# lucaspk512/vrdone

Measured on AMD Instinct MI355X. Metric: subject-object pairs/sec forward (2048 pairs x 256 frames x 512-d), higher is better.
Workload: dtype f16x3: f32 products as 3 scaled-f16 MFMA products (~22-bit), f32 accumulate; reference-grade: distance to a float64 run of the reference <= 1.4 x the reference's own float32 error (tests/golden/mask_vrd_f64.npz)

## Files before the change

### include/vrdone_hip.h

```cpp
#ifndef VRDONE_HIP_H
#define VRDONE_HIP_H

#include <stdint.h>

#ifdef __cplusplus
extern "C" {
#endif

#define VRD_ABI_VERSION 36

#define VRD_DETERMINISTIC 1
#define VRD_ERR_SCRATCH (-3)
int vrd_scratch_required(int64_t* floats);

enum vrd_act { VRD_ACT_NONE = 0, VRD_ACT_RELU = 1, VRD_ACT_GELU = 2 };

enum vrd_pair_format { VRD_PAIR_NONE = 0, VRD_PAIR_BF16 = 1, VRD_PAIR_F16 = 2 };
#define VRD_F16_ACT_EXP 4

enum vrd_kernel_id {
    VRD_K_GEMM = 0, VRD_K_LAYERNORM = 1, VRD_K_DWCONV_LN = 2, VRD_K_LOCAL_ATTN = 3,
    VRD_K_ATTN_SMALL = 4, VRD_K_ATTN_FLASH = 5, VRD_K_POOL = 6, VRD_K_MASK_HEAD = 7,
    VRD_K_TRANSPOSE = 8, VRD_K_POSTPROC = 9, VRD_K_GEMM_X3 = 10, VRD_K_GEMM_X3_DMA = 11, VRD_K_GEMM_X3_BIG = 12,
    VRD_K_BACKWARD = 13,
    VRD_K_COUNT = 14
};

int vrd_abi_version(void);
const char* vrd_last_error(void);

int vrd_f16_range_flag(void** flag);

int vrd_prof_enable(int on);
int vrd_prof_reset(void);
int vrd_prof_read(int kernel_id, double* ms, int64_t* launches, double* flops, double* bytes);
int vrd_prof_read_skipped(int kernel_id, double* flops_skipped);
int vrd_prof_select(unsigned long long family_mask);

int vrd_bct_to_btc(const float* src, int B, int C_total, int T, int c0, int count,
                   float* dst, int64_t ld_dst, int out_pair , int T_src, const int32_t* src_batch,
                   void* stream);
typedef struct {
    const float* const* src;
    const int32_t* lens;
    int32_t P, C_in, T, V, Cc, S, E;
    float* vis;
    float* clip;
    float* so_box;
    float* ent;
    int32_t pair_wide;
} vrd_pack_args;
int vrd_pack_pairs(const vrd_pack_args* a, void* stream);

typedef struct {
    const float* vis;
    const float* clip;
    const float* boxes;
    const int64_t* s_row;
    const int64_t* o_row;
    const int32_t* lens;
    int32_t P, T, V, Cc, stride;
    float w, h;
    float* out_vis;
    float* out_clip;
    float* out_so_box;
    float* out_ent;
    int32_t pair_wide;
    const float* seq_wh;
} vrd_gather_args;
int vrd_gather_pairs(const vrd_gather_args* a, void* stream);

typedef struct {
    const float* streams;
    const float* snippets;
    const int64_t* stream_row;
    const int32_t* lens;
    int32_t P, T, D, L, piece, reach;
    float* out;
} vrd_assemble_args;
int vrd_assemble_pairs(const vrd_assemble_args* a, void* stream);

int vrd_btc_to_bct(const float* src, int64_t ld_src, int B, int C, int T, float* dst, void* stream);

typedef struct {
    const float* A;  int64_t lda;
    const float* W;
    const float* bias;
    float* C;  int64_t ldc;
    int64_t M;  int32_t N;  int32_t Cin;  int32_t taps;  int32_t T;
    int32_t act;
    const uint8_t* row_mask;
    const float* scale;
    const float* res;  int64_t ldres;  int32_t res_masked;
    const float* res2;  int64_t ldres2;
    const uint16_t* W_split;
    int32_t a_pair_width;
    int32_t c_pair;
    const int32_t* row_blocks;
    const int32_t* row_blocks_active;
    int32_t row_block_seg_len;
    int32_t split_fmt;
    const float* w_scale;
    const float* a_scale;
    int32_t products;
} vrd_gemm_args;
int vrd_gemm(const vrd_gemm_args* a, void* stream);
int vrd_gemm_batch(const vrd_gemm_args* a, int count, void* stream);

int vrd_row_blocks(const uint8_t* mask, int64_t rows, int seg_len, int32_t* order, int32_t* n_active, void* stream);

typedef struct {
    const float* x;
    int64_t ldx;
    int64_t rows;
    int Cin, taps, T, N;
    const float* w;
    const float* bias;
    const uint8_t* row_mask;
    const float* gamma;
    const float* beta;
    int relu;
    float* y;
    int64_t ldy;
    int out_pair;
} vrd_conv_ln_args;
int vrd_conv_ln(const vrd_conv_ln_args* a, void* stream);

int vrd_layernorm(const float* x, int64_t ldx, float* y, int64_t ldy, int64_t rows, int C,
                  const float* gamma, const float* beta, int relu,
                  const float* post_add, int64_t ld_add, int add_period, int out_pair , void* stream);

#define VRD_MAX_SEGS 32
typedef struct {
    int32_t count;
    int32_t n[VRD_MAX_SEGS];
    int32_t T[VRD_MAX_SEGS];
    int64_t row[VRD_MAX_SEGS];
} vrd_row_segs;

typedef struct {
    const float* x;  int64_t ldx;
    const float* x_up;  int64_t ldx_up;
    int32_t B, Tin, C, ksize, stride, group_in;
    const uint8_t* mask_out;
    int32_t n_out;
    const float* w[3];
    const float* bias[3];
    const float* gamma[3];
    const float* beta[3];
    int32_t relu[3];
    float* y[3];
    int64_t ldy[3];
    int32_t out_pair[3];
    const float* pre_gamma;
    const float* pre_beta;
    const float* packed[3];
    const vrd_row_segs* segs;
} vrd_dwconv_ln_args;
int vrd_dwconv_ln(const vrd_dwconv_ln_args* a, void* stream);

int vrd_local_attn(const float* q, const float* k, const float* v, int64_t ld,
                   const uint8_t* mask, const float* rel_pe, int B, int T, int C, int n_head, int half_win,
                   float* out, int64_t ldo, int out_pair, void* stream);
int vrd_local_attn_segs(const float* q, const float* k, const float* v, int64_t ld,
                        const uint8_t* mask, const float* rel_pe, const vrd_row_segs* segs, int C, int n_head, int half_win,
                        float* out, int64_t ldo, int out_pair, void* stream);

int vrd_attention(const float* q, int64_t ldq, const float* k, const float* v, int64_t ldkv,
                  const uint8_t* kv_mask, int B, int Tq, int Tk, int n_head, int head_dim,
                  float* out, int64_t ldo, int algo, int out_pair, void* stream);

int vrd_attention_pair(const float* q, int64_t ldq, const float* k, const float* v, int64_t ldkv,
                       const uint8_t* kv_mask, const uint8_t* q_mask, int B, int Tq, int Tk, int n_head, int head_dim,
                       float* out, int64_t ldo, int out_pair, int pair_fmt, void* stream, int products);

int vrd_maxpool_mask(const float* x, int64_t ldx, int B, int Tin, int C, const uint8_t* mask_in,
                     float* y, int64_t ldy, uint8_t* mask_out, void* stream);

int vrd_mask_head(const float* emb, int64_t ld_emb, const float* feat, int64_t ld_feat,
                  const uint8_t* out_mask, int B, int Q, int T, int Dp, float fill,
                  float* seg, void* stream);

int vrd_postprocess(const float* logits, const float* masks, const int32_t* valid_len,
                    int P, int Q, int K1, int T, int topk,
                    float* top_score, int32_t* top_cat, int32_t* seg_first, int32_t* seg_last,
                    void* stream);

typedef struct {
    const float* cand;
    const float* s_score;
    const float* o_score;
    const int32_t* so_offset;
    const int32_t* so_start;
    const int32_t* so_end;
    const int32_t* video_pairs;
    int32_t n_videos, max_video_pairs, Q, k, feat_stride, pred_min_frames, n_max_pair;
    int32_t* out_count;
    int32_t* out_index;
    float* out_score;
} vrd_select_args;
int vrd_select_triplets(const vrd_select_args* a, void* stream);


int vrd_gemm_wgrad(const float* G, int64_t ldg, const float* X, int64_t ldx, const uint8_t* row_mask, int64_t M, int N, int Cin,
                   int taps, int T, float* dW, float* scratch, int64_t scratch_floats, void* stream, int flags);

int vrd_gemm_wgrad_x3(const float* G, int64_t ldg, const float* X, int64_t ldx, const uint8_t* row_mask, int64_t M, int N, int Cin,
                      int taps, int T, float* dW, float* dbias, float* scratch, int64_t scratch_floats, const float* g_scale,
                      void* stream, int flags);

#define VRD_ABSMAX_SCALE_FLOATS 516
int vrd_absmax_scale(const float* x, int64_t ldx, int64_t rows, int cols, float* scale, void* stream);

int vrd_colsum(const float* a, int64_t lda, const float* b, int64_t ldb, int b_cstride, int b_coffset, int b_rstride, int shift,
               int T, const uint8_t* row_mask, const float* row_scale, int64_t rows, int C, float* out, float* scratch,
               int64_t scratch_floats, void* stream, int flags);

int vrd_dwconv_wgrad(const float* dD, int64_t lddd, const float* x, int64_t ldx, int ksize, int stride, int group_in, int T,
                     const uint8_t* row_mask, int64_t rows, int C, float* dw, float* dbias, float* scratch, int64_t scratch_floats,
                     void* stream, int flags);

int vrd_rowcol_scale(const float* v, int64_t ldv, int64_t rows, int C, const float* col_scale, const float* row_scale,
                     const uint8_t* row_mask, const float* res, int64_t ldres, int res_masked, const float* res2, int64_t ldres2,
                     float* out, int64_t ldo, void* stream);

int vrd_activation(const float* x, int64_t ldx, const float* dy, int64_t lddy, int64_t rows, int C, int act, float* out, int64_t ldo,
            void* stream);

int vrd_layernorm_bwd(const float* x, int64_t ldx, const float* dy, int64_t lddy, int64_t rows, int C, const float* gamma,
                      const float* beta, int relu, float* dx, int64_t lddx, float* dgamma, float* dbeta, float* scratch,
                      int64_t scratch_floats, void* stream, int flags);

typedef struct {
    const float* dD[3];  int64_t lddd[3];
    const float* w[3];
    int32_t n_out, B, Tin, C, ksize, stride, group_in;
    const uint8_t* mask_out;
    float* dx;  int64_t lddx;
    float* dx_up;  int64_t lddx_up;
} vrd_dwconv_bwd_args;
int vrd_dwconv_bwd(const vrd_dwconv_bwd_args* a, void* stream);

int vrd_local_attn_bwd(const float* q, const float* k, const float* v, int64_t ld, const float* dO, int64_t lddo,
                       const uint8_t* mask, const float* rel_pe, int B, int T, int C, int n_head, int half_win,
                       float* dq, float* dk, float* dv,
                       int64_t ldd, float* scratch, void* stream);

int vrd_attn_bwd_probs(const float* q, int64_t ldq, const float* k, const float* v, int64_t ldkv, const float* dO, int64_t lddo,
                       const uint8_t* kv_mask, int B, int Tq, int Tk, int n_head, int head_dim, float* P, float* dS, void* stream);

int vrd_attn_bwd_softmax(float* P, float* dS, const uint8_t* kv_mask, int B, int Tq, int Tk, int n_head, void* stream);

int vrd_attention_bwd(const float* q, int64_t ldq, const float* k, const float* v, int64_t ldkv, const float* out, const float* dO,
                      int64_t ldo, const uint8_t* kv_mask, int B, int Tq, int Tk, int n_head, int head_dim, float* dq, float* dk,
                      float* dv, const float* lse , float* scratch,
                      const float* o_scale, const float* v_scale, void* stream);
int vrd_attention_rows(const float* q, int64_t ldq, const float* k, const float* v, int64_t ldkv, const uint8_t* kv_mask, int B, int Tq,
                       int Tk, int n_head, int head_dim, int fmt, float* out, int64_t ldo, float* lse, void* stream);

typedef struct {
    const float* A;  int64_t a_z0, a_z1, a_row, a_col;
    const float* B;  int64_t b_z0, b_z1, b_row, b_col;
    float* C;  int64_t c_z0, c_z1, c_row, c_col;
    int32_t Z0, Z1, M, N, K;
    float alpha;
    int32_t accumulate;
} vrd_bmm_args;
int vrd_bmm(const vrd_bmm_args* a, void* stream);

int vrd_maxpool_bwd(const float* x, int64_t ldx, const float* dy, int64_t lddy, int B, int Tin, int C, const uint8_t* mask_in, float* dx,
                    int64_t lddx, void* stream);

int vrd_assign(const float* cost, int64_t ld, const int32_t* first, const int32_t* count, int P, int Q, int32_t* query_of, void* stream);

int vrd_ema_update(float* const* ema, const float* const* model, const int64_t* numel, const int32_t* chunk_tensor,
                   const int32_t* chunk_index, int n_chunks, float decay, float one_minus_decay, void* stream);

typedef struct {
    const float* logits[4];
    const float* masks[4];
    int32_t n_layers, B, Q, K1, T, G;
    const uint8_t* out_valid;
    const int64_t* tgt_ids;
    const float* tgt_masks;
    const int32_t* owner;
    const int32_t* segs;
    float scale_range, alpha, gamma;
    float w_class, w_mask, w_dice;
} vrd_criterion_args;

typedef struct {
    float* logits[4];
    float* masks[4];
} vrd_criterion_grads;

int vrd_criterion_costs(const vrd_criterion_args* a, float* cost, void* stream);
int vrd_criterion_losses(const vrd_criterion_args* a, const int32_t* query_of, const float* class_weight, float num_masks, float* out,
                         void* stream);
int vrd_criterion_backward(const vrd_criterion_args* a, const int32_t* query_of, const float* class_weight, float num_masks,
                           const float* fwd_out, const float* gout, const vrd_criterion_grads* grads, void* stream);

int vrd_split_weight(const float* src, int R, int Q, int taps, int64_t sr, int64_t st, int64_t sq, uint16_t* out, int fmt, float* scale,
                     void* stream);

typedef struct {
    const float* src;
    uint16_t* out;
    int32_t R, Q, taps, fmt;
    int64_t sr, st, sq;
    float* scale;
} vrd_split_job;
int vrd_split_weights(const vrd_split_job* jobs, int n_jobs, const int32_t* chunk_job, const int32_t* chunk_index, int n_chunks,
// ... 7 lines not shown
```

### vrdone_amd/_hip.py

```python
import ctypes as C
import os

_HERE = os.path.dirname(os.path.abspath(__file__))
LIB_PATH = os.environ.get("VRDONE_HIP_LIB") or os.path.join(_HERE, "csrc", "libvrdone_hip.so")

ACT_NONE, ACT_RELU, ACT_GELU = 0, 1, 2
PAIR_NONE, PAIR_BF16, PAIR_F16 = 0, 1, 2
F16_ACT_EXP = 4
ABSMAX_SCALE_FLOATS = 516
(K_GEMM, K_LAYERNORM, K_DWCONV_LN, K_LOCAL_ATTN, K_ATTN_SMALL, K_ATTN_FLASH, K_POOL, K_MASK_HEAD,
 K_TRANSPOSE, K_POSTPROC, K_GEMM_X3, K_GEMM_X3_DMA, K_GEMM_X3_BIG, K_BACKWARD, K_COUNT) = range(15)
KERNEL_NAMES = ["gemm_f32_mfma", "layernorm", "dwconv_ln", "local_attn", "attn_small", "attn_flash",
                "maxpool_mask", "mask_head", "transpose", "postprocess", "gemm_x3_mfma", "gemm_x3_dma",
                "gemm_x3_big", "backward"]
assert len(KERNEL_NAMES) == K_COUNT

c_f32p = C.c_void_p
c_u8p = C.c_void_p
c_i32p = C.c_void_p


class CriterionArgs(C.Structure):
    _fields_ = [("logits", C.c_void_p * 4), ("masks", C.c_void_p * 4),
                ("n_layers", C.c_int32), ("B", C.c_int32), ("Q", C.c_int32), ("K1", C.c_int32), ("T", C.c_int32), ("G", C.c_int32),
                ("out_valid", C.c_void_p), ("tgt_ids", C.c_void_p), ("tgt_masks", C.c_void_p), ("owner", C.c_void_p),
                ("segs", C.c_void_p), ("scale_range", C.c_float), ("alpha", C.c_float), ("gamma", C.c_float),
                ("w_class", C.c_float), ("w_mask", C.c_float), ("w_dice", C.c_float)]


class CriterionGrads(C.Structure):
    _fields_ = [("logits", C.c_void_p * 4), ("masks", C.c_void_p * 4)]


class GemmArgs(C.Structure):
    _fields_ = [("A", c_f32p), ("lda", C.c_int64), ("W", c_f32p), ("bias", c_f32p),
                ("C", c_f32p), ("ldc", C.c_int64),
                ("M", C.c_int64), ("N", C.c_int32), ("Cin", C.c_int32), ("taps", C.c_int32), ("T", C.c_int32),
                ("act", C.c_int32), ("row_mask", c_u8p), ("scale", c_f32p),
                ("res", c_f32p), ("ldres", C.c_int64), ("res_masked", C.c_int32),
                ("res2", c_f32p), ("ldres2", C.c_int64), ("W_split", C.c_void_p),
                ("a_pair_width", C.c_int32), ("c_pair", C.c_int32),
                ("row_blocks", C.c_void_p), ("row_blocks_active", C.c_void_p), ("row_block_seg_len", C.c_int32),
                ("split_fmt", C.c_int32), ("w_scale", c_f32p), ("a_scale", c_f32p), ("products", C.c_int32)]


MAX_SEGS = 32


class RowSegs(C.Structure):
    _fields_ = [("count", C.c_int32), ("n", C.c_int32 * MAX_SEGS), ("T", C.c_int32 * MAX_SEGS), ("row", C.c_int64 * MAX_SEGS)]

    _made = {}

    @classmethod
    def of(cls, segs):
        key = tuple(segs)
        s = cls._made.get(key)
        if s is None:
            assert 1 <= len(segs) <= MAX_SEGS
            if len(cls._made) > 4096:
                cls._made.clear()
            s = cls._made[key] = cls()
            s.count = len(segs)
            for i, (row, n, T) in enumerate(segs):
                s.row[i], s.n[i], s.T[i] = row, n, T
        return s


class DwconvLnArgs(C.Structure):
    _fields_ = [("x", c_f32p), ("ldx", C.c_int64), ("x_up", c_f32p), ("ldx_up", C.c_int64),
                ("B", C.c_int32), ("Tin", C.c_int32), ("C", C.c_int32), ("ksize", C.c_int32),
                ("stride", C.c_int32), ("group_in", C.c_int32),
                ("mask_out", c_u8p), ("n_out", C.c_int32),
                ("w", c_f32p * 3), ("bias", c_f32p * 3), ("gamma", c_f32p * 3), ("beta", c_f32p * 3),
                ("relu", C.c_int32 * 3), ("y", c_f32p * 3), ("ldy", C.c_int64 * 3), ("out_pair", C.c_int32 * 3),
                ("pre_gamma", c_f32p), ("pre_beta", c_f32p), ("packed", c_f32p * 3), ("segs", C.POINTER(RowSegs))]


class ConvLnArgs(C.Structure):
    _fields_ = [("x", c_f32p), ("ldx", C.c_int64), ("rows", C.c_int64),
                ("Cin", C.c_int32), ("taps", C.c_int32), ("T", C.c_int32), ("N", C.c_int32),
                ("w", c_f32p), ("bias", c_f32p), ("row_mask", c_u8p), ("gamma", c_f32p), ("beta", c_f32p),
                ("relu", C.c_int32), ("y", c_f32p), ("ldy", C.c_int64), ("out_pair", C.c_int32)]


class PackArgs(C.Structure):
    _fields_ = [("src", C.c_void_p), ("lens", C.c_void_p),
                ("P", C.c_int32), ("C_in", C.c_int32), ("T", C.c_int32), ("V", C.c_int32), ("Cc", C.c_int32),
                ("S", C.c_int32), ("E", C.c_int32),
                ("vis", c_f32p), ("clip", c_f32p), ("so_box", c_f32p), ("ent", c_f32p), ("pair_wide", C.c_int32)]


class DwconvBwdArgs(C.Structure):
    _fields_ = [("dD", c_f32p * 3), ("lddd", C.c_int64 * 3), ("w", c_f32p * 3),
                ("n_out", C.c_int32), ("B", C.c_int32), ("Tin", C.c_int32), ("C", C.c_int32), ("ksize", C.c_int32),
                ("stride", C.c_int32), ("group_in", C.c_int32),
                ("mask_out", c_u8p), ("dx", c_f32p), ("lddx", C.c_int64), ("dx_up", c_f32p), ("lddx_up", C.c_int64)]


class BmmArgs(C.Structure):
    _fields_ = [("A", c_f32p), ("a_z0", C.c_int64), ("a_z1", C.c_int64), ("a_row", C.c_int64), ("a_col", C.c_int64),
                ("B", c_f32p), ("b_z0", C.c_int64), ("b_z1", C.c_int64), ("b_row", C.c_int64), ("b_col", C.c_int64),
                ("C", c_f32p), ("c_z0", C.c_int64), ("c_z1", C.c_int64), ("c_row", C.c_int64), ("c_col", C.c_int64),
                ("Z0", C.c_int32), ("Z1", C.c_int32), ("M", C.c_int32), ("N", C.c_int32), ("K", C.c_int32),
                ("alpha", C.c_float), ("accumulate", C.c_int32)]


class SplitJob(C.Structure):
    _fields_ = [("src", c_f32p), ("out", C.c_void_p), ("R", C.c_int32), ("Q", C.c_int32), ("taps", C.c_int32), ("fmt", C.c_int32),
                ("sr", C.c_int64), ("st", C.c_int64), ("sq", C.c_int64), ("scale", c_f32p)]


class GatherArgs(C.Structure):
    _fields_ = [("vis", c_f32p), ("clip", c_f32p), ("boxes", c_f32p), ("s_row", C.c_void_p), ("o_row", C.c_void_p),
                ("lens", C.c_void_p), ("P", C.c_int32), ("T", C.c_int32), ("V", C.c_int32), ("Cc", C.c_int32),
                ("stride", C.c_int32), ("w", C.c_float), ("h", C.c_float),
                ("out_vis", c_f32p), ("out_clip", c_f32p), ("out_so_box", c_f32p), ("out_ent", c_f32p),
                ("pair_wide", C.c_int32), ("seq_wh", c_f32p)]


class SelectArgs(C.Structure):
    _fields_ = [("cand", c_f32p), ("s_score", c_f32p), ("o_score", c_f32p), ("so_offset", c_i32p), ("so_start", c_i32p),
                ("so_end", c_i32p), ("video_pairs", c_i32p),
                ("n_videos", C.c_int32), ("max_video_pairs", C.c_int32), ("Q", C.c_int32), ("k", C.c_int32),
                ("feat_stride", C.c_int32), ("pred_min_frames", C.c_int32), ("n_max_pair", C.c_int32),
                ("out_count", c_i32p), ("out_index", c_i32p), ("out_score", c_f32p)]


class AssembleArgs(C.Structure):
    _fields_ = [("streams", c_f32p), ("snippets", c_f32p), ("stream_row", C.c_void_p), ("lens", C.c_void_p),
                ("P", C.c_int32), ("T", C.c_int32), ("D", C.c_int32), ("L", C.c_int32), ("piece", C.c_int32), ("reach", C.c_int32),
                ("out", c_f32p)]


_SIGNATURES = {
    "vrd_abi_version": (C.c_int, []),
    "vrd_last_error": (C.c_char_p, []),
    "vrd_f16_range_flag": (C.c_int, [C.POINTER(C.c_void_p)]),
    "vrd_prof_enable": (C.c_int, [C.c_int]),
    "vrd_prof_reset": (C.c_int, []),
    "vrd_prof_read": (C.c_int, [C.c_int, C.POINTER(C.c_double), C.POINTER(C.c_int64), C.POINTER(C.c_double),
                                C.POINTER(C.c_double)]),
    "vrd_prof_read_skipped": (C.c_int, [C.c_int, C.POINTER(C.c_double)]),
    "vrd_prof_select": (C.c_int, [C.c_uint64]),
    "vrd_bct_to_btc": (C.c_int, [c_f32p, C.c_int, C.c_int, C.c_int, C.c_int, C.c_int, c_f32p, C.c_int64, C.c_int, C.c_int, c_i32p,
                                 C.c_void_p]),
    "vrd_btc_to_bct": (C.c_int, [c_f32p, C.c_int64, C.c_int, C.c_int, C.c_int, c_f32p, C.c_void_p]),
    "vrd_pack_pairs": (C.c_int, [C.POINTER(PackArgs), C.c_void_p]),
    "vrd_gather_pairs": (C.c_int, [C.POINTER(GatherArgs), C.c_void_p]),
    "vrd_assemble_pairs": (C.c_int, [C.POINTER(AssembleArgs), C.c_void_p]),
    "vrd_split_weight": (C.c_int, [c_f32p, C.c_int, C.c_int, C.c_int, C.c_int64, C.c_int64, C.c_int64, C.c_void_p, C.c_int, c_f32p,
                                   C.c_void_p]),
    "vrd_split_weights": (C.c_int, [C.c_void_p, C.c_int, C.c_void_p, C.c_void_p, C.c_int, C.c_void_p]),
    "vrd_gemm": (C.c_int, [C.POINTER(GemmArgs), C.c_void_p]),
    "vrd_gemm_batch": (C.c_int, [C.POINTER(GemmArgs), C.c_int, C.c_void_p]),
    "vrd_row_blocks": (C.c_int, [c_u8p, C.c_int64, C.c_int, C.c_void_p, C.c_void_p, C.c_void_p]),
    "vrd_conv_ln": (C.c_int, [C.POINTER(ConvLnArgs), C.c_void_p]),
    "vrd_layernorm": (C.c_int, [c_f32p, C.c_int64, c_f32p, C.c_int64, C.c_int64, C.c_int, c_f32p, c_f32p, C.c_int,
                                c_f32p, C.c_int64, C.c_int, C.c_int, C.c_void_p]),
    "vrd_dwconv_ln": (C.c_int, [C.POINTER(DwconvLnArgs), C.c_void_p]),
    "vrd_local_attn": (C.c_int, [c_f32p, c_f32p, c_f32p, C.c_int64, c_u8p, c_f32p, C.c_int, C.c_int, C.c_int, C.c_int,
                                 C.c_int, c_f32p, C.c_int64, C.c_int, C.c_void_p]),
    "vrd_local_attn_segs": (C.c_int, [c_f32p, c_f32p, c_f32p, C.c_int64, c_u8p, c_f32p, C.POINTER(RowSegs), C.c_int, C.c_int,
                                      C.c_int, c_f32p, C.c_int64, C.c_int, C.c_void_p]),
    "vrd_attention": (C.c_int, [c_f32p, C.c_int64, c_f32p, c_f32p, C.c_int64, c_u8p, C.c_int, C.c_int, C.c_int,
                                C.c_int, C.c_int, c_f32p, C.c_int64, C.c_int, C.c_int, C.c_void_p]),
    "vrd_attention_pair": (C.c_int, [c_f32p, C.c_int64, c_f32p, c_f32p, C.c_int64, c_u8p, c_u8p, C.c_int, C.c_int, C.c_int,
                                     C.c_int, C.c_int, c_f32p, C.c_int64, C.c_int, C.c_int, C.c_void_p, C.c_int]),
    "vrd_maxpool_mask": (C.c_int, [c_f32p, C.c_int64, C.c_int, C.c_int, C.c_int, c_u8p, c_f32p, C.c_int64, c_u8p,
                                   C.c_void_p]),
    "vrd_mask_head": (C.c_int, [c_f32p, C.c_int64, c_f32p, C.c_int64, c_u8p, C.c_int, C.c_int, C.c_int, C.c_int,
                                C.c_float, c_f32p, C.c_void_p]),
    "vrd_postprocess": (C.c_int, [c_f32p, c_f32p, c_i32p, C.c_int, C.c_int, C.c_int, C.c_int, C.c_int, c_f32p, c_i32p,
                                  c_i32p, c_i32p, C.c_void_p]),
    "vrd_select_triplets": (C.c_int, [C.POINTER(SelectArgs), C.c_void_p]),
    "vrd_gemm_wgrad": (C.c_int, [c_f32p, C.c_int64, c_f32p, C.c_int64, c_u8p, C.c_int64, C.c_int, C.c_int, C.c_int, C.c_int,
                                 c_f32p, c_f32p, C.c_int64, C.c_void_p, C.c_int]),
    "vrd_gemm_wgrad_x3": (C.c_int, [c_f32p, C.c_int64, c_f32p, C.c_int64, c_u8p, C.c_int64, C.c_int, C.c_int, C.c_int, C.c_int,
                                    c_f32p, c_f32p, c_f32p, C.c_int64, c_f32p, C.c_void_p, C.c_int]),
    "vrd_scratch_required": (C.c_int, [C.POINTER(C.c_int64)]),
    "vrd_absmax_scale": (C.c_int, [c_f32p, C.c_int64, C.c_int64, C.c_int, c_f32p, C.c_void_p]),
    "vrd_dwconv_wgrad": (C.c_int, [c_f32p, C.c_int64, c_f32p, C.c_int64, C.c_int, C.c_int, C.c_int, C.c_int, c_u8p, C.c_int64,
                                   C.c_int, c_f32p, c_f32p, c_f32p, C.c_int64, C.c_void_p, C.c_int]),
    "vrd_colsum": (C.c_int, [c_f32p, C.c_int64, c_f32p, C.c_int64, C.c_int, C.c_int, C.c_int, C.c_int, C.c_int, c_u8p, c_f32p,
                             C.c_int64, C.c_int, c_f32p, c_f32p, C.c_int64, C.c_void_p, C.c_int]),
    "vrd_rowcol_scale": (C.c_int, [c_f32p, C.c_int64, C.c_int64, C.c_int, c_f32p, c_f32p, c_u8p, c_f32p, C.c_int64, C.c_int,
                                   c_f32p, C.c_int64, c_f32p, C.c_int64, C.c_void_p]),
    "vrd_activation": (C.c_int, [c_f32p, C.c_int64, c_f32p, C.c_int64, C.c_int64, C.c_int, C.c_int, c_f32p, C.c_int64, C.c_void_p]),
    "vrd_layernorm_bwd": (C.c_int, [c_f32p, C.c_int64, c_f32p, C.c_int64, C.c_int64, C.c_int, c_f32p, c_f32p, C.c_int, c_f32p,
                                    C.c_int64, c_f32p, c_f32p, c_f32p, C.c_int64, C.c_void_p, C.c_int]),
    "vrd_dwconv_bwd": (C.c_int, [C.POINTER(DwconvBwdArgs), C.c_void_p]),
    "vrd_local_attn_bwd": (C.c_int, [c_f32p, c_f32p, c_f32p, C.c_int64, c_f32p, C.c_int64, c_u8p, c_f32p, C.c_int, C.c_int,
                                     C.c_int, C.c_int, C.c_int, c_f32p, c_f32p, c_f32p, C.c_int64, c_f32p, C.c_void_p]),
    "vrd_attn_bwd_probs": (C.c_int, [c_f32p, C.c_int64, c_f32p, c_f32p, C.c_int64, c_f32p, C.c_int64, c_u8p, C.c_int, C.c_int,
                                     C.c_int, C.c_int, C.c_int, c_f32p, c_f32p, C.c_void_p]),
    "vrd_bmm": (C.c_int, [C.POINTER(BmmArgs), C.c_void_p]),
    "vrd_attention_bwd": (C.c_int, [c_f32p, C.c_int64, c_f32p, c_f32p, C.c_int64, c_f32p, c_f32p, C.c_int64, c_u8p, C.c_int, C.c_int,
                                    C.c_int, C.c_int, C.c_int, c_f32p, c_f32p, c_f32p, c_f32p, c_f32p, c_f32p, c_f32p, C.c_void_p]),
    "vrd_attention_rows": (C.c_int, [c_f32p, C.c_int64, c_f32p, c_f32p, C.c_int64, c_u8p, C.c_int, C.c_int, C.c_int, C.c_int, C.c_int,
                                     C.c_int, c_f32p, C.c_int64, c_f32p, C.c_void_p]),
    "vrd_assign": (C.c_int, [c_f32p, C.c_int64, c_i32p, c_i32p, C.c_int, C.c_int, c_i32p, C.c_void_p]),
    "vrd_ema_update": (C.c_int, [C.c_void_p, C.c_void_p, C.c_void_p, c_i32p, c_i32p, C.c_int, C.c_float, C.c_float, C.c_void_p]),
    "vrd_attn_bwd_softmax": (C.c_int, [c_f32p, c_f32p, c_u8p, C.c_int, C.c_int, C.c_int, C.c_int, C.c_void_p]),
    "vrd_criterion_costs": (C.c_int, [C.c_void_p, c_f32p, C.c_void_p]),
    "vrd_criterion_losses": (C.c_int, [C.c_void_p, c_i32p, c_f32p, C.c_float, c_f32p, C.c_void_p]),
    "vrd_criterion_backward": (C.c_int, [C.c_void_p, c_i32p, c_f32p, C.c_float, c_f32p, c_f32p, C.c_void_p, C.c_void_p]),
    "vrd_maxpool_bwd": (C.c_int, [c_f32p, C.c_int64, c_f32p, C.c_int64, C.c_int, C.c_int, C.c_int, c_u8p, c_f32p, C.c_int64,
                                  C.c_void_p]),
}

ABI_VERSION = 36

DETERMINISTIC = 1
ERR_SCRATCH = -3


class HipLibraryError(RuntimeError):
    pass


_FLAGS_DEFAULT = ("vrd_gemm_wgrad_x3", "vrd_colsum", "vrd_dwconv_wgrad", "vrd_layernorm_bwd")


def _flags_default(fn):
    n = len(fn.argtypes)

    def call(*args):
        return fn(*args, 0) if len(args) == n - 1 else fn(*args)
    call.__name__, call.argtypes, call.restype = fn.__name__, fn.argtypes, fn.restype
    return call


def _load():
    if not os.path.exists(LIB_PATH):
        raise HipLibraryError(
            f"{LIB_PATH} is missing: the HIP extension was not built "
            "(run `make -C vrdone_amd/csrc`); there is no CPU fallback for this path")
    import torch
    lib = C.CDLL(LIB_PATH)
    for name, (res, args) in _SIGNATURES.items():
        fn = getattr(lib, name)
        fn.restype = res
        fn.argtypes = args
    for name in _FLAGS_DEFAULT:
        setattr(lib, name, _flags_default(getattr(lib, name)))
    got = lib.vrd_abi_version()
    if got != ABI_VERSION:
        raise HipLibraryError(f"libvrdone_hip.so ABI {got} != expected {ABI_VERSION}: rebuild it")
    return lib


lib = _load()


def check(rc, what):
    if rc != 0:
        raise RuntimeError(f"{what} failed ({rc}): {lib.vrd_last_error().decode()}")


RANGE_TAGS = {1: "boundary tensors (bct_to_btc / pack_pairs / gather_pairs)", 2: "layernorm", 4: "dwconv_ln", 8: "gemm outputs",
              16: "f32 rows split inside a gemm", 32: "attention outputs", 64: "other"}


def prof_enable(on=True):
    check(lib.vrd_prof_enable(1 if on else 0), "vrd_prof_enable")


def prof_select(families=None):
    mask = (1 << 64) - 1 if families is None else sum(1 << KERNEL_NAMES.index(f) for f in families)
    check(lib.vrd_prof_select(mask), "vrd_prof_select")


def prof_reset():
    check(lib.vrd_prof_reset(), "vrd_prof_reset")


def prof_read():
    out = {}
    for kid, name in enumerate(KERNEL_NAMES):
        ms, n, fl, by, sk = C.c_double(), C.c_int64(), C.c_double(), C.c_double(), C.c_double()
        check(lib.vrd_prof_read(kid, C.byref(ms), C.byref(n), C.byref(fl), C.byref(by)), "vrd_prof_read")
        check(lib.vrd_prof_read_skipped(kid, C.byref(sk)), "vrd_prof_read_skipped")
        out[name] = {"ms": ms.value, "launches": n.value, "flops": fl.value, "bytes": by.value, "flops_skipped": sk.value}
    return out
```

### vrdone_amd/csrc/vrd_rowops.hip

```cpp
#include "vrd_common.h"
#include <cmath>

namespace {

constexpr float LN_EPS = 1e-5f;

__device__ __forceinline__ float4 ld4(const float* p) { return *reinterpret_cast<const float4*>(p); }
__device__ __forceinline__ void st4(float* p, float4 v) { *reinterpret_cast<float4*>(p) = v; }
__device__ __forceinline__ float4 f4add(float4 a, float4 b) { return make_float4(a.x + b.x, a.y + b.y, a.z + b.z, a.w + b.w); }

__global__ __launch_bounds__(256) void bct_to_btc_kernel(const float* __restrict__ src, int C_total, int T, int c0,
                                                         int count, float* __restrict__ dst, int64_t ld_dst, int pair, int T_src,
                                                         const int32_t* __restrict__ src_batch, unsigned* rflag) {
    __shared__ float tile[64][65];
    vrd::RangeTrack rt;
    const int b = blockIdx.z, ct = blockIdx.y * 64, tt = blockIdx.x * 64;
    const int tx = threadIdx.x & 63, ty = threadIdx.x >> 6;
    const float* s = src + ((int64_t)(src_batch ? src_batch[b] : b) * C_total + c0) * T_src;
    for (int c = ty; c < 64; c += 4)
        tile[c][tx] = (ct + c < count && tt + tx < T) ? s[(int64_t)(ct + c) * T_src + tt + tx] : 0.f;
    __syncthreads();
    for (int t = ty; t < 64; t += 4)
        if (tt + t < T && ct + tx < count) {
            float* row = dst + ((int64_t)b * T + tt + t) * ld_dst;
// ... 197 lines not shown
    for (int i = 0; i < NV; ++i) {
        v[i].x -= mean; v[i].y -= mean; v[i].z -= mean; v[i].w -= mean;
        ss += (v[i].x * v[i].x + v[i].y * v[i].y) + (v[i].z * v[i].z + v[i].w * v[i].w);
    }
    const float inv = 1.0f / sqrtf(vrd::wave_sum(ss) * inv_c + LN_EPS);
#pragma unroll
    for (int i = 0; i < NV; ++i) {
        const float4 g = ld4(gamma + lane_chan<NV, WIDE>(i, lane)), bb = ld4(beta + lane_chan<NV, WIDE>(i, lane));
        v[i].x = fmaf(v[i].x * inv, g.x, bb.x);
        v[i].y = fmaf(v[i].y * inv, g.y, bb.y);
        v[i].z = fmaf(v[i].z * inv, g.z, bb.z);
        v[i].w = fmaf(v[i].w * inv, g.w, bb.w);
        if (relu) {
            v[i].x = fmaxf(v[i].x, 0.f); v[i].y = fmaxf(v[i].y, 0.f);
            v[i].z = fmaxf(v[i].z, 0.f); v[i].w = fmaxf(v[i].w, 0.f);
        }
    }
}

template <int NV>
__global__ __launch_bounds__(256) void layernorm_kernel(const float* __restrict__ x, int64_t ldx, float* __restrict__ y,
                                                        int64_t ldy, int64_t rows, const float* __restrict__ gamma,
                                                        const float* __restrict__ beta, int relu,
                                                        const float* __restrict__ post_add, int64_t ld_add, int period,
                                                        int pair, unsigned* rflag) {
    vrd::RangeTrack rt;
    const int lane = threadIdx.x & 63;
    int64_t row = (int64_t)blockIdx.x * 4 + __builtin_amdgcn_readfirstlane(threadIdx.x >> 6);
    const int64_t stride = (int64_t)gridDim.x * 4;
    if (row >= rows) return;
    float4 v[NV], vn[NV];
#pragma unroll
    for (int i = 0; i < NV; ++i) v[i] = ld4(x + row * ldx + i * 256 + lane * 4);
    for (;;) {
        const int64_t nxt = row + stride;
        if (nxt < rows) {
#pragma unroll
            for (int i = 0; i < NV; ++i) vn[i] = ld4(x + nxt * ldx + i * 256 + lane * 4);
        }
        ln_rows<NV>(v, gamma, beta, lane, relu != 0);
        if (post_add) {
            const float* a = post_add + (row % period) * ld_add;
#pragma unroll
            for (int i = 0; i < NV; ++i) v[i] = f4add(v[i], ld4(a + i * 256 + lane * 4));
        }
#pragma unroll
        for (int i = 0; i < NV; ++i) {
            if (pair) vrd::store_pair4(y + row * ldy, i * 256 + lane * 4, 256 * NV, v[i], pair, &rt);
            else st4(y + row * ldy + i * 256 + lane * 4, v[i]);
        }
        if (nxt >= rows) break;
        row = nxt;
#pragma unroll
        for (int i = 0; i < NV; ++i) v[i] = vn[i];
    }
    rt.report(rflag, vrd::RANGE_LAYERNORM);
}

constexpr int CL_MAXK = 32;
template <int NV>
__global__ __launch_bounds__(256) void conv_ln_kernel(vrd_conv_ln_args p, unsigned* rflag) {
    vrd::RangeTrack rt;
    constexpr int N = 256 * NV;
    constexpr bool WIDE = NV == 2;
    extern __shared__ __attribute__((aligned(16))) float cl_lds[];
    const int K = p.Cin * p.taps;
    for (int idx = threadIdx.x; idx < N * K; idx += 256) {
        const int n = idx / K, rem = idx - n * K, ci = rem / p.taps, tap = rem - ci * p.taps;
        cl_lds[(tap * p.Cin + ci) * N + n] = p.w[idx];
    }
    for (int n = threadIdx.x; n < N; n += 256) cl_lds[K * N + n] = p.bias ? p.bias[n] : 0.f;
    __syncthreads();
    const int lane = threadIdx.x & 63;
    constexpr int RG = 4;
    int64_t grp = (int64_t)blockIdx.x * 4 + __builtin_amdgcn_readfirstlane(threadIdx.x >> 6);
    const int64_t stride = (int64_t)gridDim.x * 4;
    const int half = p.taps / 2;
    const int lrow = lane / p.Cin, lci = lane - lrow * p.Cin;
    auto load_in = [&](int64_t g) {
        const int64_t r = g * RG - half + lrow;
        float val = 0.f;
        if (lrow < RG + 2 * half && r >= 0 && r < p.rows) val = p.x[r * p.ldx + lci];
        return val;
    };
    float xin = grp * RG < p.rows ? load_in(grp) : 0.f;
    for (; grp * RG < p.rows; grp += stride) {
        const int64_t row0 = grp * RG;
        const float xcur = xin;
        if ((grp + stride) * RG < p.rows) xin = load_in(grp + stride);
        float4 v[RG][NV];
        int t[RG];
#pragma unroll
        for (int j = 0; j < RG; ++j) {
            t[j] = (int)((row0 + j) % p.T);
#pragma unroll
            for (int i = 0; i < NV; ++i) v[j][i] = *reinterpret_cast<const float4*>(cl_lds + K * N + lane_chan<NV, WIDE>(i, lane));
        }
        for (int tap = 0; tap < p.taps; ++tap) {
            for (int ci = 0; ci < p.Cin; ++ci) {
                const float* wk = cl_lds + (tap * p.Cin + ci) * N;
                float4 w[NV];
#pragma unroll
                for (int i = 0; i < NV; ++i) w[i] = *reinterpret_cast<const float4*>(wk + lane_chan<NV, WIDE>(i, lane));
#pragma unroll
                for (int j = 0; j < RG; ++j) {
                    const int tt = t[j] + tap - half;
                    const bool ok = tt >= 0 && tt < p.T && row0 + j < p.rows;
                    const float xl = __builtin_bit_cast(float, __builtin_amdgcn_readlane(__builtin_bit_cast(int, xcur), (j + tap) * p.Cin + ci));
                    const float xv = ok ? xl : 0.f;
#pragma unroll
                    for (int i = 0; i < NV; ++i) {
                        v[j][i].x = fmaf(w[i].x, xv, v[j][i].x); v[j][i].y = fmaf(w[i].y, xv, v[j][i].y);
                        v[j][i].z = fmaf(w[i].z, xv, v[j][i].z); v[j][i].w = fmaf(w[i].w, xv, v[j][i].w);
                    }
                }
            }
        }
#pragma unroll
        for (int j = 0; j < RG; ++j) {
            const int64_t row = row0 + j;
            if (row >= p.rows) break;
            if (p.row_mask) {
                const float mk = (float)vrd::uniform_load(p.row_mask + row);
#pragma unroll
                for (int i = 0; i < NV; ++i) v[j][i].x *= mk, v[j][i].y *= mk, v[j][i].z *= mk, v[j][i].w *= mk;
            }
            if (p.gamma) {
                ln_rows<NV, WIDE>(v[j], p.gamma, p.beta, lane, p.relu != 0);
            } else if (p.relu) {
#pragma unroll
                for (int i = 0; i < NV; ++i) {
                    v[j][i].x = fmaxf(v[j][i].x, 0.f); v[j][i].y = fmaxf(v[j][i].y, 0.f);
                    v[j][i].z = fmaxf(v[j][i].z, 0.f); v[j][i].w = fmaxf(v[j][i].w, 0.f);
                }
            }
            float* yr = p.y + row * p.ldy;
            if (WIDE && p.out_pair) {
                vrd::store_pair8(yr, lane * 8, v[j][0], v[j][NV - 1], p.out_pair, &rt);
            } else {
#pragma unroll
                for (int i = 0; i < NV; ++i) {
                    const int c = lane_chan<NV, WIDE>(i, lane);
                    if (p.out_pair) vrd::store_pair4(yr, c, N, v[j][i], p.out_pair, &rt);
                    else st4(yr + c, v[j][i]);
                }
            }
        }
    }
    rt.report(rflag, vrd::RANGE_LAYERNORM);
}

constexpr int DW_RW = 16;

template <int NV, int KS, int GIN>
__global__ __launch_bounds__(256) void dwconv_ln_kernel(vrd_dwconv_ln_args p, int Tout_u, int strips_per_seq, int strips_per_wave, int rw, unsigned* rflag,
                                                        vrd::SegTable sg) {
    vrd::RangeTrack rt;
    constexpr int C = 256 * NV, NT = GIN * KS, SETF = (NT + 3) * C;
    constexpr bool WIDE = NV == 2 && GIN == 1;
    extern __shared__ __attribute__((aligned(16))) float dw_lds[];
    const int lane = threadIdx.x & 63, wave = __builtin_amdgcn_readfirstlane(threadIdx.x >> 6);
    for (int o = 0; o < p.n_out; ++o) {
        float* const ls = dw_lds + o * SETF;
        if (p.packed[o]) {
            for (int idx = threadIdx.x * 4; idx < SETF; idx += 1024) st4(ls + idx, ld4(p.packed[o] + idx));
            continue;
        }
        for (int idx = threadIdx.x; idx < C * NT; idx += 256) ls[(idx % NT) * C + idx / NT] = p.w[o][idx];
        for (int c = threadIdx.x; c < C; c += 256) {
            ls[NT * C + c] = p.bias[o] ? p.bias[o][c] : 0.f;
            ls[(NT + 1) * C + c] = p.gamma[o] ? p.gamma[o][c] : 1.f;
            ls[(NT + 2) * C + c] = p.gamma[o] ? p.beta[o][c] : 0.f;
        }
    }
    const float* const pre = dw_lds + p.n_out * SETF;
    if (p.pre_gamma)
        for (int c = threadIdx.x; c < C; c += 256) {
            dw_lds[p.n_out * SETF + c] = p.pre_gamma[c];
            dw_lds[p.n_out * SETF + C + c] = p.pre_beta[c];
        }
    __syncthreads();
    const int nwg = gridDim.x, bid = blockIdx.x;
    const int xcd = bid & 7, qq = nwg >> 3, rem = nwg & 7;
    const int lid = (xcd < rem ? xcd * (qq + 1) : rem * (qq + 1) + (xcd - rem) * qq) + (bid >> 3);
    for (int si = 0; si < strips_per_wave; ++si) {
    const int64_t ws = ((int64_t)lid * 4 + wave) * strips_per_wave + si;
    int Tin, Tout, to0;
    int64_t xrow0, urow0, orow0;
    if (sg.count) {
        int g, b, strip;
        if (!vrd::seg_find(sg, ws, g, b, strip)) break;
        Tin = sg.T[g], Tout = Tin / p.stride, to0 = strip * rw;
        xrow0 = sg.row[g] + (int64_t)b * Tin;
        urow0 = sg.row[g] / 2 + (int64_t)b * (Tin / 2);
        orow0 = sg.row[g] / p.stride + (int64_t)b * Tout;
    } else {
        const int b = (int)(ws / strips_per_seq);
        if (b >= p.B) break;
        Tin = p.Tin, Tout = Tout_u, to0 = (int)(ws - (int64_t)b * strips_per_seq) * rw;
        xrow0 = (int64_t)b * Tin, urow0 = (int64_t)b * (Tin / 2), orow0 = (int64_t)b * Tout;
    }
    const int to1 = min(to0 + rw, Tout);

    struct Row {
        float4 v[NV][GIN];
    };
    auto load_row = [&](int ti) {
        Row r;
        const bool ok = ti >= 0 && ti < Tin;
#pragma unroll
        for (int i = 0; i < NV; ++i)
#pragma unroll
            for (int g = 0; g < GIN; ++g) {
                float4 v = make_float4(0.f, 0.f, 0.f, 0.f);
                if (ok) {
                    const int64_t coff = (int64_t)GIN * lane_chan<NV, WIDE>(i, lane) + 4 * g;
                    v = ld4(p.x + (xrow0 + ti) * p.ldx + coff);
                    if (p.x_up) v = f4add(v, ld4(p.x_up + (urow0 + (ti >> 1)) * p.ldx_up + coff));
                }
                r.v[i][g] = v;
            }
        if (GIN == 1 && p.pre_gamma && ok) {
            float4 t[NV];
#pragma unroll
            for (int i = 0; i < NV; ++i) t[i] = r.v[i][0];
            ln_rows<NV, WIDE>(t, pre, pre + C, lane, false);
#pragma unroll
            for (int i = 0; i < NV; ++i) r.v[i][0] = t[i];
        }
        return r;
    };
    if (p.mask_out) {
        const int64_t r0 = orow0 + to0;
        const bool mine = lane < to1 - to0 && p.mask_out[r0 + lane] != 0;
        if (!__any(mine)) {
#pragma unroll
            for (int o = 0; o < 3; ++o) {
                if (o >= p.n_out) break;
                const float* const lb = dw_lds + o * SETF + (NT + 2) * C;
                float4 val[NV];
#pragma unroll
                for (int i = 0; i < NV; ++i) {
                    val[i] = *reinterpret_cast<const float4*>(lb + lane_chan<NV, WIDE>(i, lane));
                    if (p.relu[o]) {
                        val[i].x = fmaxf(val[i].x, 0.f); val[i].y = fmaxf(val[i].y, 0.f);
                        val[i].z = fmaxf(val[i].z, 0.f); val[i].w = fmaxf(val[i].w, 0.f);
                    }
                }
                for (int to = to0; to < to1; ++to) {
                    const int64_t row = orow0 + to;
                    if (WIDE && p.out_pair[o]) {
                        vrd::store_pair8(p.y[o] + row * p.ldy[o], lane * 8, val[0], val[NV - 1], p.out_pair[o], &rt);
                    } else {
#pragma unroll
                        for (int i = 0; i < NV; ++i) {
                            const int c = lane_chan<NV, WIDE>(i, lane);
                            if (p.out_pair[o]) vrd::store_pair4(p.y[o] + row * p.ldy[o], c, 256 * NV, val[i], p.out_pair[o], &rt);
                            else st4(p.y[o] + row * p.ldy[o] + c, val[i]);
                        }
                    }
                }
            }
            continue;
        }
    }
    Row win[KS];
#pragma unroll
    for (int k = 0; k < KS; ++k) win[k] = load_row(p.stride * to0 + k - KS / 2);
    for (int to = to0; to < to1; ++to) {
        Row nxt[2];
        const int tn = p.stride * (to + 1) - KS / 2;
        const bool more = to + 1 < to1;
        if (KS == 1) {
            if (more) nxt[0] = load_row(tn);
        } else if (p.stride == 1) {
            if (more) nxt[0] = load_row(tn + 2);
        } else {
            if (more) {
                nxt[0] = load_row(tn + 1);
                nxt[1] = load_row(tn + 2);
            }
        }
        const int64_t row = orow0 + to;
        const float mk = p.mask_out ? (float)p.mask_out[row] : 1.f;
#pragma unroll
        for (int o = 0; o < 3; ++o) {
            if (o >= p.n_out) break;
            const float* const ls = dw_lds + o * SETF;
            float4 acc[NV];
#pragma unroll
            for (int i = 0; i < NV; ++i) {
                const int c = lane_chan<NV, WIDE>(i, lane);
                float4 r = *reinterpret_cast<const float4*>(ls + NT * C + c);
#pragma unroll
                for (int k = 0; k < KS; ++k) {
                    if (GIN == 1) {
                        const float4 w = *reinterpret_cast<const float4*>(ls + k * C + c);
                        const float4 v = win[k].v[i][0];
                        r.x += w.x * v.x; r.y += w.y * v.y; r.z += w.z * v.z; r.w += w.w * v.w;
                    } else {
                        const float4 w0 = *reinterpret_cast<const float4*>(ls + (0 * KS + k) * C + c);
                        const float4 w1 = *reinterpret_cast<const float4*>(ls + (1 * KS + k) * C + c);
                        const float4 v0 = win[k].v[i][0], v1 = win[k].v[i][GIN - 1];
                        r.x += w0.x * v0.x + w1.x * v0.y;
                        r.y += w0.y * v0.z + w1.y * v0.w;
                        r.z += w0.z * v1.x + w1.z * v1.y;
                        r.w += w0.w * v1.z + w1.w * v1.w;
                    }
                }
                acc[i] = make_float4(r.x * mk, r.y * mk, r.z * mk, r.w * mk);
            }
            if (p.gamma[o]) {
                ln_rows<NV, WIDE>(acc, ls + (NT + 1) * C, ls + (NT + 2) * C, lane, p.relu[o] != 0);
            } else if (p.relu[o]) {
#pragma unroll
                for (int i = 0; i < NV; ++i) {
                    acc[i].x = fmaxf(acc[i].x, 0.f); acc[i].y = fmaxf(acc[i].y, 0.f);
                    acc[i].z = fmaxf(acc[i].z, 0.f); acc[i].w = fmaxf(acc[i].w, 0.f);
                }
            }
            if (WIDE && p.out_pair[o]) {
                vrd::store_pair8(p.y[o] + row * p.ldy[o], lane * 8, acc[0], acc[NV - 1], p.out_pair[o], &rt);
            } else {
#pragma unroll
                for (int i = 0; i < NV; ++i) {
                    const int c = lane_chan<NV, WIDE>(i, lane);
                    if (p.out_pair[o]) vrd::store_pair4(p.y[o] + row * p.ldy[o], c, 256 * NV, acc[i], p.out_pair[o], &rt);
                    else st4(p.y[o] + row * p.ldy[o] + c, acc[i]);
                }
            }
        }
        if (more) {
            if (KS == 1) {
                win[0] = nxt[0];
            } else if (p.stride == 1) {
                win[0] = win[1];
                win[KS > 1 ? 1 : 0] = win[KS - 1];
                win[KS - 1] = nxt[0];
            } else {
                win[0] = win[KS - 1];
                win[KS > 1 ? 1 : 0] = nxt[0];
                win[KS - 1] = nxt[1];
            }
        }
    }
    }
    rt.report(rflag, vrd::RANGE_DWCONV_LN);
}

__global__ __launch_bounds__(256) void maxpool_mask_kernel(const float* __restrict__ x, int64_t ldx, int B, int Tin, int C,
                                                           const uint8_t* __restrict__ mask_in, float* __restrict__ y,
                                                           int64_t ldy, uint8_t* __restrict__ mask_out) {
    const int c4 = C / 4;
    const int64_t idx = (int64_t)blockIdx.x * 256 + threadIdx.x;
    const int Tout = Tin / 2;
    if (idx >= (int64_t)B * Tout * c4) return;
    const int c = (int)(idx % c4) * 4;
    const int64_t row = idx / c4;
    const int b = (int)(row / Tout), to = (int)(row - (int64_t)b * Tout);
    const float* base = x + ((int64_t)b * Tin + 2 * to) * ldx + c;
    float4 m = ld4(base);
    const float4 r = ld4(base + ldx);
    m.x = fmaxf(m.x, r.x); m.y = fmaxf(m.y, r.y); m.z = fmaxf(m.z, r.z); m.w = fmaxf(m.w, r.w);
    if (to > 0) {
        const float4 l = ld4(base - ldx);
        m.x = fmaxf(m.x, l.x); m.y = fmaxf(m.y, l.y); m.z = fmaxf(m.z, l.z); m.w = fmaxf(m.w, l.w);
    }
    const uint8_t mk = mask_in[(int64_t)b * Tin + 2 * to];
    const float f = (float)mk;
    st4(y + row * ldy + c, make_float4(m.x * f, m.y * f, m.z * f, m.w * f));
    if (c == 0 && mask_out) mask_out[row] = mk;
}

constexpr int MH_D = 256, MH_TT = 32, MH_QMAX = 16;

__global__ __launch_bounds__(256) void mask_head_kernel(const float* __restrict__ emb, int64_t ld_emb,
                                                        const float* __restrict__ feat, int64_t ld_feat,
                                                        const uint8_t* __restrict__ out_mask, int Q, int T, float fill,
                                                        float* __restrict__ seg) {
    __shared__ float fs[MH_TT][MH_D + 1];
    __shared__ float es[MH_QMAX][MH_D];
    const int b = blockIdx.y, t0 = blockIdx.x * MH_TT, tid = threadIdx.x;
    for (int i = tid; i < MH_TT * (MH_D / 4); i += 256) {
        const int r = i / (MH_D / 4), c = (i % (MH_D / 4)) * 4;
        float4 v = make_float4(0.f, 0.f, 0.f, 0.f);
        if (t0 + r < T) v = ld4(feat + ((int64_t)b * T + t0 + r) * ld_feat + c);
        fs[r][c] = v.x; fs[r][c + 1] = v.y; fs[r][c + 2] = v.z; fs[r][c + 3] = v.w;
    }
    for (int i = tid; i < Q * (MH_D / 4); i += 256) {
        const int r = i / (MH_D / 4), c = (i % (MH_D / 4)) * 4;
        st4(&es[r][c], ld4(emb + ((int64_t)b * Q + r) * ld_emb + c));
    }
    __syncthreads();
    const int tt = tid & 31, qg = tid >> 5;
    if (t0 + tt >= T) return;
    const bool on = out_mask[(int64_t)b * T + t0 + tt] != 0;
    for (int q = qg; q < Q; q += 8) {
        float s = 0.f;
#pragma unroll 8
        for (int c = 0; c < MH_D; ++c) s = fmaf(es[q][c], fs[tt][c], s);
        seg[((int64_t)b * Q + q) * T + t0 + tt] = on ? s : fill;
    }
}

inline bool aligned16(const void* ptr) { return (reinterpret_cast<uintptr_t>(ptr) & 15u) == 0; }

constexpr int RB_THREADS = 1024;
__global__ __launch_bounds__(RB_THREADS) void row_blocks_kernel(const uint8_t* __restrict__ mask, int nblocks, int seg_len, int S,
                                                                int32_t* __restrict__ order, int32_t* __restrict__ n_active) {
    __shared__ int counts[RB_THREADS];
    const int tid = threadIdx.x;
    const int per = (nblocks + RB_THREADS - 1) / RB_THREADS;
    const int b0 = min(tid * per, nblocks), b1 = min(b0 + per, nblocks);
    auto active = [&](int b) {
        const uint4* q = reinterpret_cast<const uint4*>(mask + (int64_t)b * 32);
        const uint4 lo = q[0], hi = q[1];
        return ((lo.x | lo.y | lo.z | lo.w | hi.x | hi.y | hi.z | hi.w) != 0u) ? 1 : 0;
    };
    int mine = 0;
    for (int b = b0; b < b1; ++b) mine += active(b);
    counts[tid] = mine;
    __syncthreads();
    for (int d = 1; d < RB_THREADS; d <<= 1) {
        const int v = tid >= d ? counts[tid - d] : 0;
        __syncthreads();
        counts[tid] += v;
        __syncthreads();
    }
    const int total = counts[RB_THREADS - 1];
    auto start = [&](int s) { return min(s * seg_len, nblocks); };
    auto first = [&](int s) { return (int)(((int64_t)total * start(s)) / nblocks); };
    auto pads_before = [&](int s) { return start(s) - first(s); };
    int a = counts[tid] - mine;
    int i = b0 - a;
    int sa = 0, sp = 0;
    for (int b = b0; b < b1; ++b) {
        if (active(b)) {
            while (sa + 1 < S && first(sa + 1) <= a) ++sa;
            order[start(sa) + (a - first(sa))] = b;
            ++a;
        } else {
            while (sp + 1 < S && pads_before(sp + 1) <= i) ++sp;
            order[start(sp) + (first(sp + 1) - first(sp)) + (i - pads_before(sp))] = b;
            ++i;
        }
    }
    if (tid < S) n_active[tid] = first(tid + 1) - first(tid);
}

}

extern "C" {

int vrd_bct_to_btc(const float* src, int B, int C_total, int T, int c0, int count, float* dst, int64_t ld_dst,
                   int out_pair, int T_src, const int32_t* src_batch, void* stream) {
    VRD_CHECK_ARG(src && dst, "vrd_bct_to_btc: null pointer");
    if (T_src == 0) T_src = T;
    VRD_CHECK_ARG(T_src >= T, "vrd_bct_to_btc: T_src (%d) < T (%d)", T_src, T);
    VRD_CHECK_ARG(B > 0 && T > 0 && count > 0 && c0 >= 0 && c0 + count <= C_total && ld_dst >= count,
                  "vrd_bct_to_btc: bad slab c0=%d count=%d C=%d ld=%lld", c0, count, C_total, (long long)ld_dst);
    VRD_CHECK_ARG(B <= 65535, "vrd_bct_to_btc: B too large for one launch (%d)", B);
    hipStream_t s = static_cast<hipStream_t>(stream);
    vrd::ProfScope prof(VRD_K_TRANSPOSE, s, 0.0, 8.0 * B * (double)count * T);
    dim3 grid((T + 63) / 64, (count + 63) / 64, B);
    VRD_CHECK_ARG(!out_pair || (count % 32 == 0 && ld_dst % 4 == 0 && aligned16(dst)), "vrd_bct_to_btc: pair rows need count %% 32 == 0");
    const bool vec = T % 4 == 0 && T_src % 4 == 0 && count % 4 == 0 && ld_dst % 4 == 0 && aligned16(dst) && aligned16(src);
    if (vec) hipLaunchKernelGGL(bct_to_btc_vec_kernel, grid, dim3(256), 0, s, src, C_total, T, c0, count, dst, ld_dst, out_pair, T_src, src_batch, out_pair == VRD_PAIR_F16 ? vrd::range_flag() : nullptr);
    else hipLaunchKernelGGL(bct_to_btc_kernel, grid, dim3(256), 0, s, src, C_total, T, c0, count, dst, ld_dst, out_pair, T_src, src_batch, out_pair == VRD_PAIR_F16 ? vrd::range_flag() : nullptr);
    VRD_LAUNCH_CHECK();
    return 0;
}

int vrd_pack_pairs(const vrd_pack_args* a, void* stream) {
    VRD_CHECK_ARG(a && a->src && a->lens && a->vis && a->so_box && a->ent, "vrd_pack_pairs: null pointer");
    VRD_CHECK_ARG(a->P > 0 && a->T > 0 && a->V > 0 && a->S > 0 && a->E > 0 && a->Cc >= 0, "vrd_pack_pairs: bad sizes");
    VRD_CHECK_ARG(a->C_in == 2 * a->V + 2 * a->Cc + a->S + 2 * a->E, "vrd_pack_pairs: C_in %d does not match the slab widths", a->C_in);
    VRD_CHECK_ARG(a->Cc == 0 || a->clip, "vrd_pack_pairs: clip buffer missing");
    VRD_CHECK_ARG(!a->pair_wide || (a->V % 32 == 0 && a->Cc % 32 == 0), "vrd_pack_pairs: pair rows need widths %% 32 == 0");
    hipStream_t s = static_cast<hipStream_t>(stream);
    const int64_t rows = (int64_t)a->P * a->T;
    vrd::ProfScope prof(VRD_K_TRANSPOSE, s, 0.0, 8.0 * (double)rows * a->C_in);
    hipLaunchKernelGGL(pack_pairs_kernel, dim3((unsigned)((rows + 3) / 4)), dim3(256), 0, s, *a, a->pair_wide == VRD_PAIR_F16 ? vrd::range_flag() : nullptr);
    VRD_LAUNCH_CHECK();
    return 0;
}

int vrd_gather_pairs(const vrd_gather_args* a, void* stream) {
    VRD_CHECK_ARG(a && a->vis && a->boxes && a->s_row && a->o_row && a->lens && a->out_so_box && a->out_ent,
                  "vrd_gather_pairs: null pointer");
    VRD_CHECK_ARG(a->P > 0 && a->T > 0 && a->V > 0 && a->Cc >= 0 && a->stride >= 1 && a->w > 0.f && a->h > 0.f, "vrd_gather_pairs: bad sizes");
    VRD_CHECK_ARG(a->Cc == 0 || !a->out_vis || (a->clip && a->out_clip), "vrd_gather_pairs: clip buffers missing");
    VRD_CHECK_ARG(!a->pair_wide || (a->V % 32 == 0 && a->Cc % 32 == 0), "vrd_gather_pairs: pair rows need widths %% 32 == 0");
    VRD_CHECK_ARG(aligned16(a->boxes), "vrd_gather_pairs: boxes must be 16-byte aligned");
    hipStream_t s = static_cast<hipStream_t>(stream);
    const int64_t rows = (int64_t)a->P * a->T;
    vrd::ProfScope prof(VRD_K_TRANSPOSE, s, 0.0, 8.0 * (double)rows * ((a->out_vis ? 2 * a->V + 2 * a->Cc : 0) + 21));
    hipLaunchKernelGGL(gather_pairs_kernel, dim3((unsigned)((rows + 3) / 4)), dim3(256), 0, s, *a, a->pair_wide == VRD_PAIR_F16 ? vrd::range_flag() : nullptr);
    VRD_LAUNCH_CHECK();
    return 0;
}

int vrd_assemble_pairs(const vrd_assemble_args* a, void* stream) {
    VRD_CHECK_ARG(a && a->streams && a->snippets && a->stream_row && a->lens && a->out, "vrd_assemble_pairs: null pointer");
    VRD_CHECK_ARG(a->P > 0 && a->T > 0 && a->D > 0 && a->D % 4 == 0, "vrd_assemble_pairs: bad sizes");
    VRD_CHECK_ARG(a->reach >= 0 && a->piece >= 2 * a->reach && a->piece >= 1 && a->L > a->piece && a->T >= a->L,
                  "vrd_assemble_pairs: pieces of %d frames in buffers of %d (T = %d) cannot cover a reach of %d", a->piece, a->L, a->T, a->reach);
    VRD_CHECK_ARG(aligned16(a->streams) && aligned16(a->snippets) && aligned16(a->out), "vrd_assemble_pairs: rows must be 16-byte aligned");
    hipStream_t s = static_cast<hipStream_t>(stream);
    const int64_t rows = 2 * (int64_t)a->P * a->T;
    VRD_CHECK_ARG((rows + 3) / 4 < ((int64_t)1 << 31), "vrd_assemble_pairs: grid too large");
    vrd::ProfScope prof(VRD_K_TRANSPOSE, s, 0.0, 8.0 * (double)rows * a->D);
    hipLaunchKernelGGL(assemble_pairs_kernel, dim3((unsigned)((rows + 3) / 4)), dim3(256), 0, s, *a);
    VRD_LAUNCH_CHECK();
    return 0;
}

int vrd_row_blocks(const uint8_t* mask, int64_t rows, int seg_len, int32_t* order, int32_t* n_active, void* stream) {
    VRD_CHECK_ARG(mask && order && n_active, "vrd_row_blocks: null pointer");
    VRD_CHECK_ARG(rows > 0 && rows % 32 == 0 && rows / 32 < (1 << 30), "vrd_row_blocks: rows %lld must be a positive multiple of 32", (long long)rows);
    const int nblocks = (int)(rows / 32);
    VRD_CHECK_ARG(seg_len >= 1 && (nblocks + seg_len - 1) / seg_len <= 64, "vrd_row_blocks: segment length %d gives more than 64 segments", seg_len);
    VRD_CHECK_ARG(aligned16(mask), "vrd_row_blocks: mask must be 16-byte aligned");
    hipStream_t s = static_cast<hipStream_t>(stream);
    vrd::ProfScope prof(VRD_K_TRANSPOSE, s, 0.0, (double)rows + 4.0 * nblocks);
    hipLaunchKernelGGL(row_blocks_kernel, dim3(1), dim3(RB_THREADS), 0, s, mask, nblocks, seg_len, (nblocks + seg_len - 1) / seg_len, order, n_active);
    VRD_LAUNCH_CHECK();
    return 0;
}

int vrd_btc_to_bct(const float* src, int64_t ld_src, int B, int C, int T, float* dst, void* stream) {
    VRD_CHECK_ARG(src && dst, "vrd_btc_to_bct: null pointer");
    VRD_CHECK_ARG(B > 0 && B <= 65535 && T > 0 && C > 0 && ld_src >= C, "vrd_btc_to_bct: bad shape");
    hipStream_t s = static_cast<hipStream_t>(stream);
    vrd::ProfScope prof(VRD_K_TRANSPOSE, s, 0.0, 8.0 * B * (double)C * T);
    dim3 grid((T + 63) / 64, (C + 63) / 64, B);
    hipLaunchKernelGGL(btc_to_bct_kernel, grid, dim3(256), 0, s, src, ld_src, C, T, dst);
    VRD_LAUNCH_CHECK();
    return 0;
}

int vrd_layernorm(const float* x, int64_t ldx, float* y, int64_t ldy, int64_t rows, int C, const float* gamma,
                  const float* beta, int relu, const float* post_add, int64_t ld_add, int add_period, int out_pair,
                  void* stream) {
    VRD_CHECK_ARG(x && y && gamma && beta, "vrd_layernorm: null pointer");
    VRD_CHECK_ARG(C == 256 || C == 512, "vrd_layernorm: C must be 256 or 512 (got %d)", C);
    VRD_CHECK_ARG(ldx >= C && ldy >= C && ldx % 4 == 0 && ldy % 4 == 0 && aligned16(x) && aligned16(y) &&
                      aligned16(gamma) && aligned16(beta),
                  "vrd_layernorm: rows must be 16-byte aligned");
    VRD_CHECK_ARG(!post_add || (add_period > 0 && ld_add % 4 == 0 && aligned16(post_add)), "vrd_layernorm: bad post_add");
    if (rows <= 0) return 0;
    hipStream_t s = static_cast<hipStream_t>(stream);
    vrd::ProfScope prof(VRD_K_LAYERNORM, s, 0.0, 8.0 * (double)rows * C);
    unsigned* const rflag = out_pair == VRD_PAIR_F16 ? vrd::range_flag() : nullptr;
    static const int64_t max_blocks = [] { const char* e = getenv("VRD_LN_BLOCKS"); return e ? atoll(e) : 8192; }();
    const int64_t want = (rows + 3) / 4;
    dim3 grid((unsigned)(max_blocks > 0 && want > max_blocks ? max_blocks : want));
    if (C == 256)
        hipLaunchKernelGGL(layernorm_kernel<1>, grid, dim3(256), 0, s, x, ldx, y, ldy, rows, gamma, beta, relu, post_add, ld_add, add_period, out_pair, rflag);
    else
        hipLaunchKernelGGL(layernorm_kernel<2>, grid, dim3(256), 0, s, x, ldx, y, ldy, rows, gamma, beta, relu, post_add, ld_add, add_period, out_pair, rflag);
    VRD_LAUNCH_CHECK();
    return 0;
}

int vrd_conv_ln(const vrd_conv_ln_args* a, void* stream) {
    VRD_CHECK_ARG(a && a->x && a->w && a->y, "vrd_conv_ln: null pointer");
    VRD_CHECK_ARG(a->N == 256 || a->N == 512, "vrd_conv_ln: N must be 256 or 512 (got %d)", a->N);
    VRD_CHECK_ARG((a->taps == 1 || a->taps == 3) && a->Cin > 0 && a->Cin * a->taps <= CL_MAXK && (4 + a->taps - 1) * a->Cin <= 64,
                  "vrd_conv_ln: taps in {1, 3}, taps * Cin <= %d and (3 + taps) * Cin <= 64 (got %d x %d)", CL_MAXK, a->taps, a->Cin);
    VRD_CHECK_ARG(a->rows >= 0 && a->T > 0 && a->rows % a->T == 0 && a->ldx >= a->Cin, "vrd_conv_ln: bad rows / T / ldx");
    VRD_CHECK_ARG((a->gamma == nullptr) == (a->beta == nullptr), "vrd_conv_ln: gamma and beta go together");
    VRD_CHECK_ARG(a->ldy >= a->N && a->ldy % 4 == 0 && aligned16(a->y) && aligned16(a->gamma) && aligned16(a->beta),
                  "vrd_conv_ln: output rows and LayerNorm parameters must be 16-byte aligned");
    VRD_CHECK_ARG(!a->out_pair || (a->ldy % 32 == 0 && (a->out_pair == VRD_PAIR_BF16 || a->out_pair == VRD_PAIR_F16)),
                  "vrd_conv_ln: pair output needs rows that start on a 128-byte block");
    if (a->rows == 0) return 0;
    hipStream_t s = static_cast<hipStream_t>(stream);
    const int K = a->Cin * a->taps;
    vrd::ProfScope prof(VRD_K_LAYERNORM, s, 2.0 * (double)a->rows * a->N * K, 4.0 * (double)a->rows * (a->N + a->Cin));
    unsigned* const rflag = a->out_pair == VRD_PAIR_F16 ? vrd::range_flag() : nullptr;
    const size_t lds = (size_t)(K + 1) * a->N * sizeof(float);
    const int64_t want = (a->rows + 15) / 16;
    dim3 grid((unsigned)(want > 4096 ? 4096 : want));
    if (a->N == 256) {
        if (lds > 48 * 1024)
            if (int rc = vrd::reserve_lds(reinterpret_cast<const void*>(conv_ln_kernel<1>), lds, "vrd_conv_ln")) return rc;
        hipLaunchKernelGGL(conv_ln_kernel<1>, grid, dim3(256), lds, s, *a, rflag);
    } else {
        if (lds > 48 * 1024)
            if (int rc = vrd::reserve_lds(reinterpret_cast<const void*>(conv_ln_kernel<2>), lds, "vrd_conv_ln")) return rc;
        hipLaunchKernelGGL(conv_ln_kernel<2>, grid, dim3(256), lds, s, *a, rflag);
    }
    VRD_LAUNCH_CHECK();
    return 0;
}

int vrd_dwconv_ln(const vrd_dwconv_ln_args* a, void* stream) {
    VRD_CHECK_ARG(a && a->x, "vrd_dwconv_ln: null args");
    VRD_CHECK_ARG(a->C == 256 || a->C == 512, "vrd_dwconv_ln: C must be 256 or 512 (got %d)", a->C);
    VRD_CHECK_ARG(a->ksize == 1 || a->ksize == 3, "vrd_dwconv_ln: ksize must be 1 or 3");
    VRD_CHECK_ARG(a->stride == 1 || a->stride == 2, "vrd_dwconv_ln: stride must be 1 or 2");
    VRD_CHECK_ARG(a->group_in == 1 || (a->group_in == 2 && a->C == 256 && a->ksize == 3),
                  "vrd_dwconv_ln: group_in=2 is only built for C=256, ksize=3");
    VRD_CHECK_ARG(a->segs || (a->B > 0 && a->Tin > 0 && a->Tin % a->stride == 0), "vrd_dwconv_ln: Tin %% stride != 0");
    VRD_CHECK_ARG(a->n_out >= 1 && a->n_out <= 3, "vrd_dwconv_ln: n_out must be 1..3");
    VRD_CHECK_ARG((a->pre_gamma == nullptr) == (a->pre_beta == nullptr) && (!a->pre_gamma || (a->group_in == 1 && !a->x_up)),
                  "vrd_dwconv_ln: input LayerNorm needs gamma and beta, group_in == 1 and no x_up");
    VRD_CHECK_ARG(a->ldx >= (int64_t)a->C * a->group_in && a->ldx % 4 == 0 && aligned16(a->x), "vrd_dwconv_ln: bad x layout");
    VRD_CHECK_ARG(!a->x_up || (a->Tin % 2 == 0 && a->ldx_up % 4 == 0 && aligned16(a->x_up)), "vrd_dwconv_ln: bad x_up layout");
    for (int o = 0; o < a->n_out; ++o) {
        VRD_CHECK_ARG((a->w[o] || a->packed[o]) && a->y[o] && aligned16(a->w[o]) && aligned16(a->packed[o]) && aligned16(a->y[o]) &&
                          a->ldy[o] % 4 == 0 && a->ldy[o] >= a->C,
                      "vrd_dwconv_ln: bad output set %d", o);
        VRD_CHECK_ARG((a->gamma[o] == nullptr) == (a->beta[o] == nullptr), "vrd_dwconv_ln: gamma/beta mismatch");
    }
    vrd::SegTable sg;
    sg.count = 0;
    int64_t rows_in = (int64_t)a->B * a->Tin;
    int Tmax = a->Tin;
    if (a->segs) {
        const int even = (a->x_up || a->stride == 2) ? 2 : 1;
        VRD_CHECK_ARG(vrd::seg_table(sg, a->segs, even, 16) >= 0, "vrd_dwconv_ln: bad row groups (1..%d groups, T %% %d == 0)", VRD_MAX_SEGS, even);
        rows_in = 0, Tmax = 0;
        for (int g = 0; g < sg.count; ++g) {
            VRD_CHECK_ARG(sg.row[g] % even == 0, "vrd_dwconv_ln: a group's first row must be even with stride 2 / x_up");
            rows_in += (int64_t)sg.n[g] * sg.T[g];
            Tmax = sg.T[g] > Tmax ? sg.T[g] : Tmax;
        }
    }
    const int Tout = Tmax / a->stride;
    const int64_t rows = rows_in / a->stride;
    hipStream_t s = static_cast<hipStream_t>(stream);
    vrd::ProfScope prof(VRD_K_DWCONV_LN, s, 0.0,
                        4.0 * ((double)rows_in * a->C * a->group_in * (a->x_up ? 1.5 : 1.0) + (double)rows * a->C * a->n_out));
    const size_t lds = ((size_t)a->n_out * (a->group_in * a->ksize + 3) + (a->pre_gamma ? 2 : 0)) * a->C * sizeof(float);
    static const int rw_env = [] { const char* e = getenv("VRD_DW_RW"); return e ? atoi(e) : 0; }();
    int rw = DW_RW;
    {
        const int64_t wgs_per_cu = lds ? (int64_t)(160 * 1024 / lds) : 8;
        const int64_t resident = 256 * (wgs_per_cu < 1 ? 1 : wgs_per_cu > 4 ? 4 : wgs_per_cu) * 4;
        auto strips_at = [&](int r) -> int64_t {
            return a->segs ? vrd::seg_table(sg, a->segs, a->stride, r) : (int64_t)a->B * ((Tout + r - 1) / r);
        };
        if (strips_at(DW_RW) < 6 * resident) {
            double best = 1e30;
            for (int r = 8; r <= 32; ++r) {
                const int64_t n = strips_at(r);
                const double cost = (double)((n + resident - 1) / resident) * (r + 3);
                if (cost < best - 1e-9) best = cost, rw = r;
            }
        }
        if (rw_env >= 1 && rw_env <= 64) rw = rw_env;
    }
    const int strips = (Tout + rw - 1) / rw;
    static const int spw_env = [] { const char* e = getenv("VRD_DW_SPW"); return e ? atoi(e) : 0; }();
    const int64_t total_strips = a->segs ? vrd::seg_table(sg, a->segs, a->stride, rw) : (int64_t)a->B * strips;
    const int spw = spw_env > 0 ? spw_env : 1;
    dim3 grid((unsigned)((total_strips + 4 * spw - 1) / (4 * spw))), block(256);
    bool any_f16 = false;
    for (int o = 0; o < a->n_out; ++o) any_f16 |= a->out_pair[o] == VRD_PAIR_F16;
    unsigned* const rflag = any_f16 ? vrd::range_flag() : nullptr;
#define VRD_DW(NV, KS, GIN) hipLaunchKernelGGL((dwconv_ln_kernel<NV, KS, GIN>), grid, block, lds, s, *a, Tout, strips, spw, rw, rflag, sg)
    if (a->group_in == 2) VRD_DW(1, 3, 2);
    else if (a->C == 256 && a->ksize == 3) VRD_DW(1, 3, 1);
    else if (a->C == 256) VRD_DW(1, 1, 1);
    else if (a->ksize == 3) VRD_DW(2, 3, 1);
    else VRD_DW(2, 1, 1);
#undef VRD_DW
    VRD_LAUNCH_CHECK();
    return 0;
}

int vrd_maxpool_mask(const float* x, int64_t ldx, int B, int Tin, int C, const uint8_t* mask_in, float* y, int64_t ldy,
                     uint8_t* mask_out, void* stream) {
    VRD_CHECK_ARG(x && y && mask_in, "vrd_maxpool_mask: null pointer");
    VRD_CHECK_ARG(B > 0 && Tin > 0 && Tin % 2 == 0 && C % 4 == 0, "vrd_maxpool_mask: Tin must be even, C %% 4 == 0");
    VRD_CHECK_ARG(ldx % 4 == 0 && ldy % 4 == 0 && ldx >= C && ldy >= C && aligned16(x) && aligned16(y), "vrd_maxpool_mask: bad layout");
    hipStream_t s = static_cast<hipStream_t>(stream);
    const int64_t n = (int64_t)B * (Tin / 2) * (C / 4);
    vrd::ProfScope prof(VRD_K_POOL, s, 0.0, 4.0 * (double)B * Tin * C * 1.5);
    hipLaunchKernelGGL(maxpool_mask_kernel, dim3((unsigned)((n + 255) / 256)), dim3(256), 0, s, x, ldx, B, Tin, C, mask_in, y, ldy, mask_out);
    VRD_LAUNCH_CHECK();
    return 0;
}

int vrd_mask_head(const float* emb, int64_t ld_emb, const float* feat, int64_t ld_feat, const uint8_t* out_mask, int B,
                  int Q, int T, int Dp, float fill, float* seg, void* stream) {
    VRD_CHECK_ARG(emb && feat && out_mask && seg, "vrd_mask_head: null pointer");
    VRD_CHECK_ARG(Dp == MH_D, "vrd_mask_head: mask dim must be %d (got %d)", MH_D, Dp);
    VRD_CHECK_ARG(Q >= 1 && Q <= MH_QMAX, "vrd_mask_head: num queries must be 1..%d (got %d)", MH_QMAX, Q);
    VRD_CHECK_ARG(B > 0 && B <= 65535 && T > 0, "vrd_mask_head: bad B/T");
    VRD_CHECK_ARG(ld_emb % 4 == 0 && ld_feat % 4 == 0 && aligned16(emb) && aligned16(feat), "vrd_mask_head: bad layout");
    hipStream_t s = static_cast<hipStream_t>(stream);
    vrd::ProfScope prof(VRD_K_MASK_HEAD, s, 2.0 * B * (double)Q * T * Dp, 4.0 * B * ((double)T * Dp + (double)Q * Dp + (double)Q * T));
    hipLaunchKernelGGL(mask_head_kernel, dim3((T + MH_TT - 1) / MH_TT, B), dim3(256), 0, s, emb, ld_emb, feat, ld_feat, out_mask, Q, T, fill, seg);
    VRD_LAUNCH_CHECK();
    return 0;
}

}
```

### vrdone_amd/csrc/vrd_runtime.hip

```cpp
#include "vrd_common.h"
#include <atomic>
#include <mutex>
#include <vector>
#include <utility>
#include <cstring>

namespace vrd {

static thread_local char g_err[512] = "";
static std::mutex g_mu;
static bool g_prof_on = false;
static unsigned long long g_prof_mask = ~0ull;

struct ProfRec {
    int id;
    hipEvent_t e0, e1;
    double flops, bytes;
};
static std::vector<ProfRec> g_recs;
static std::vector<hipEvent_t> g_free_events;
static double g_ms[VRD_K_COUNT], g_flops[VRD_K_COUNT], g_bytes[VRD_K_COUNT];
static int64_t g_launches[VRD_K_COUNT];
static double g_skipped[VRD_K_COUNT];
double take_big_skipped_flops();
double take_f32_skipped_flops();

void set_error(const char* fmt, ...) {
    va_list ap;
    va_start(ap, fmt);
    vsnprintf(g_err, sizeof(g_err), fmt, ap);
    va_end(ap);
}

int reserve_lds(const void* kernel, size_t bytes, const char* what) {
    int dev = 0;
    if (hipGetDevice(&dev) != hipSuccess) dev = 0;
    std::lock_guard<std::mutex> lk(g_mu);
    static std::vector<std::pair<const void*, int>> done;
    for (const auto& d : done)
        if (d.first == kernel && d.second == dev) return 0;
    hipError_t e = hipFuncSetAttribute(kernel, hipFuncAttributeMaxDynamicSharedMemorySize, (int)bytes);
    if (e != hipSuccess) {
        set_error("%s: cannot reserve %zu B of LDS on device %d: %s", what, bytes, dev, hipGetErrorString(e));
        return -2;
    }
    done.emplace_back(kernel, dev);
    return 0;
}

int device_cu_count() {
    int dev = 0;
    if (hipGetDevice(&dev) != hipSuccess) dev = 0;
    std::lock_guard<std::mutex> lk(g_mu);
    static std::vector<int> cus;
    if (dev >= (int)cus.size()) cus.resize(dev + 1, 0);
    if (cus[dev] == 0) {
        int n = 0;
        if (hipDeviceGetAttribute(&n, hipDeviceAttributeMultiprocessorCount, dev) != hipSuccess || n <= 0) n = 256;
        cus[dev] = n;
    }
    return cus[dev];
}

unsigned* range_flag() {
    constexpr int MAX_DEV = 64;
    static std::atomic<unsigned*> flags[MAX_DEV];
    static std::atomic<bool> failed[MAX_DEV];
    int dev = 0;
    if (hipGetDevice(&dev) != hipSuccess) dev = 0;
    if (dev < 0 || dev >= MAX_DEV) return nullptr;
    if (unsigned* q = flags[dev].load(std::memory_order_acquire)) return q;
    if (failed[dev].load(std::memory_order_relaxed)) return nullptr;
    std::lock_guard<std::mutex> lk(g_mu);
    if (unsigned* q = flags[dev].load(std::memory_order_acquire)) return q;
    unsigned* q = nullptr;
    if (hipMalloc(&q, 64) != hipSuccess) {
        failed[dev].store(true);
        return nullptr;
    }
    if (hipMemset(q, 0, 64) != hipSuccess) {
        (void)hipFree(q);
        failed[dev].store(true);
        return nullptr;
    }
    flags[dev].store(q, std::memory_order_release);
    return q;
}

static hipEvent_t get_event() {
    if (!g_free_events.empty()) {
        hipEvent_t e = g_free_events.back();
        g_free_events.pop_back();
        return e;
    }
    hipEvent_t e;
    if (hipEventCreate(&e) != hipSuccess) return nullptr;
    return e;
}

ProfScope::ProfScope(int kernel_id, hipStream_t s, double flops, double bytes)
    : id(kernel_id), stream(s), slot(nullptr) {
    if (!g_prof_on || !((g_prof_mask >> kernel_id) & 1ull)) return;
    std::lock_guard<std::mutex> lk(g_mu);
    ProfRec r;
    r.id = kernel_id;
    r.e0 = get_event();
    r.e1 = get_event();
    r.flops = flops;
    r.bytes = bytes;
    if (!r.e0 || !r.e1) return;
    (void)hipEventRecord(r.e0, s);
    g_recs.push_back(r);
    slot = reinterpret_cast<void*>(g_recs.size());
}

ProfScope::~ProfScope() {
    if (!slot) return;
    std::lock_guard<std::mutex> lk(g_mu);
    size_t idx = reinterpret_cast<size_t>(slot) - 1;
    if (idx < g_recs.size()) (void)hipEventRecord(g_recs[idx].e1, stream);
}

static void drain() {
    for (auto& r : g_recs) {
        float ms = 0.f;
        if (hipEventSynchronize(r.e1) == hipSuccess && hipEventElapsedTime(&ms, r.e0, r.e1) == hipSuccess) {
            g_ms[r.id] += ms;
            g_flops[r.id] += r.flops;
            g_bytes[r.id] += r.bytes;
            g_launches[r.id] += 1;
        }
        g_free_events.push_back(r.e0);
        g_free_events.push_back(r.e1);
    }
    g_recs.clear();
    g_skipped[VRD_K_GEMM_X3_BIG] += take_big_skipped_flops();
    g_skipped[VRD_K_GEMM] += take_f32_skipped_flops();
}

}

extern "C" {

int vrd_abi_version(void) { return VRD_ABI_VERSION; }
const char* vrd_last_error(void) { return vrd::g_err; }

int vrd_f16_range_flag(void** flag) {
    VRD_CHECK_ARG(flag, "vrd_f16_range_flag: null pointer");
    *flag = vrd::range_flag();
    if (!*flag) {
        vrd::set_error("vrd_f16_range_flag: cannot allocate the flag word");
        return -2;
    }
    return 0;
}

int vrd_prof_enable(int on) {
    std::lock_guard<std::mutex> lk(vrd::g_mu);
    vrd::g_prof_on = on != 0;
    return 0;
}

int vrd_prof_select(unsigned long long family_mask) {
    std::lock_guard<std::mutex> lk(vrd::g_mu);
    vrd::g_prof_mask = family_mask;
    return 0;
}

int vrd_prof_reset(void) {
    std::lock_guard<std::mutex> lk(vrd::g_mu);
    vrd::drain();
    memset(vrd::g_ms, 0, sizeof(vrd::g_ms));
    memset(vrd::g_flops, 0, sizeof(vrd::g_flops));
    memset(vrd::g_bytes, 0, sizeof(vrd::g_bytes));
    memset(vrd::g_launches, 0, sizeof(vrd::g_launches));
    memset(vrd::g_skipped, 0, sizeof(vrd::g_skipped));
    return 0;
}

int vrd_prof_read_skipped(int kernel_id, double* flops_skipped) {
    VRD_CHECK_ARG(kernel_id >= 0 && kernel_id < VRD_K_COUNT && flops_skipped, "vrd_prof_read_skipped: bad arguments");
    std::lock_guard<std::mutex> lk(vrd::g_mu);
    vrd::drain();
    *flops_skipped = vrd::g_skipped[kernel_id];
    return 0;
}

int vrd_prof_read(int kernel_id, double* ms, int64_t* launches, double* flops, double* bytes) {
    VRD_CHECK_ARG(kernel_id >= 0 && kernel_id < VRD_K_COUNT, "vrd_prof_read: bad kernel id %d", kernel_id);
    std::lock_guard<std::mutex> lk(vrd::g_mu);
    vrd::drain();
    if (ms) *ms = vrd::g_ms[kernel_id];
    if (launches) *launches = vrd::g_launches[kernel_id];
    if (flops) *flops = vrd::g_flops[kernel_id];
    if (bytes) *bytes = vrd::g_bytes[kernel_id];
    return 0;
}

}
```

### vrdone_amd/models/backbones.py

```python
import torch
from torch import nn

from .blocks import ConvMLP, LayerNorm, MaskedConv1D, TransformerBlock, _from_cl, _mask2d, _ops, get_sinusoid_encoding
from .local_transformer import MaskedConvTransformerDecoderLayer


class MaskConvTransformerBackbone(nn.Module):
    def __init__(self, n_visual, n_bbox_entity, n_bbox_so, n_embd, n_head, n_embd_ks, fuse_ks, n_fuse_head,
                 fuse_path_drop, fuse_qx_stride, fuse_kv_stride, max_len, arch=(2, 2, 3), mha_win_size=[-1] * 4,
                 scale_factor=2, with_ln=False, attn_pdrop=0.0, proj_pdrop=0.0, path_pdrop=0.0, use_abs_pe=False,
                 use_rel_pe=False, use_local=True):
        super().__init__()
        assert len(arch) == 3 and len(mha_win_size) == 1 + arch[-1]
        assert with_ln, "built for embd_with_ln=True"
        assert scale_factor == 2 and n_embd_ks == 3
        self.n_visual, self.n_bbox_entity, self.n_bbox_so = n_visual, n_bbox_entity, n_bbox_so
        self.n_clip = 0
        self.arch, self.mha_win_size, self.max_len = arch, mha_win_size, max_len
        self.relu = nn.ReLU(inplace=True)
        self.scale_factor, self.use_abs_pe, self.use_rel_pe = scale_factor, use_abs_pe, use_rel_pe

        if use_abs_pe:
            self.register_buffer("pos_embd", get_sinusoid_encoding(max_len, n_embd) / (n_embd ** 0.5), persistent=False)
        self.visual_embd, self.visual_embd_norm = self._embedding(n_visual, n_embd, n_embd_ks, arch[0])
        self.bbox_entity_embd = MaskedConv1D(n_bbox_entity, n_embd, n_embd_ks, stride=1, padding=n_embd_ks // 2)
        self.bbox_entity_norm = LayerNorm(n_embd)
        self.visual_bbox_fuse = ConvMLP(n_embd * 2, n_embd, n_embd, kernel_size=fuse_ks, num_layers=2)

        self.stem = nn.ModuleList()
        self.s_attn = nn.ModuleList()
        self.o_attn = nn.ModuleList()
        for _ in range(arch[1]):
            self.stem.append(TransformerBlock(n_embd, n_head, n_ds_strides=(1, 1), attn_pdrop=attn_pdrop,
                                              proj_pdrop=proj_pdrop, path_pdrop=path_pdrop,
                                              mha_win_size=mha_win_size[0], use_rel_pe=use_rel_pe))
            for mutual in (self.s_attn, self.o_attn):
                mutual.append(MaskedConvTransformerDecoderLayer(
                    n_embd=n_embd, n_head=n_fuse_head, path_pdrop=fuse_path_drop, n_qx_stride=fuse_qx_stride,
                    n_kv_stride=fuse_kv_stride, with_ffn=False, use_local=use_local,
                    win_size=mha_win_size[0] if use_local else None))
        self.s_fuse_norm = LayerNorm(n_embd)
        self.o_fuse_norm = LayerNorm(n_embd)
        self.so_fuse = ConvMLP(n_embd * 2, n_embd, n_embd, kernel_size=fuse_ks, num_layers=2)
        self.bbox_so_embd = MaskedConv1D(n_bbox_so, n_embd, n_embd_ks, stride=1, padding=n_embd_ks // 2)
        self.so_visual_bbox_fuse = ConvMLP(n_embd * 2, n_embd, n_embd, kernel_size=fuse_ks, num_layers=2)

        self.branch = nn.ModuleList(
            TransformerBlock(n_embd, n_head, n_ds_strides=(scale_factor, scale_factor), attn_pdrop=attn_pdrop,
                             proj_pdrop=proj_pdrop, path_pdrop=path_pdrop, mha_win_size=mha_win_size[1 + i],
                             use_rel_pe=use_rel_pe)
            for i in range(arch[2]))
        self._zero_biases()

    @staticmethod
    def _embedding(n_in, n_embd, ks, depth):
        convs, norms = nn.ModuleList(), nn.ModuleList()
        for i in range(depth):
            convs.append(MaskedConv1D(n_in if i == 0 else n_embd, n_embd, ks, stride=1, padding=ks // 2, bias=False))
            norms.append(LayerNorm(n_embd))
        return convs, norms

    def _zero_biases(self):
        for m in self.modules():
            if isinstance(m, (nn.Linear, nn.Conv1d)) and m.bias is not None:
                nn.init.zeros_(m.bias)

    def in_channels(self):
        return 2 * self.n_visual + 2 * self.n_clip + self.n_bbox_so + 2 * self.n_bbox_entity

    def _unpack(self, x, frames=None, index=None):
        ops = _ops()
        B, _, T = x.shape
        if index is not None:
            B = index.numel()
        if frames is not None:
            T = frames
        V, Cc, S, E = self.n_visual, self.n_clip, self.n_bbox_so, self.n_bbox_entity
        pair = ops.pair_mode()

        def stacked(c0, width, as_pair):
            h = torch.empty(2, B, T, width, device=x.device, dtype=torch.float32)
            ops.bct_to_btc(x, c0, width, h[0], pair=as_pair, frames=frames, index=index)
            ops.bct_to_btc(x, c0 + width, width, h[1], pair=as_pair, frames=frames, index=index)
            h = h.view(2 * B, T, width)
            return ops.Pair(h, width) if as_pair else h

        o0 = 2 * V + 2 * Cc
        so_box = torch.empty(B, T, S, device=x.device, dtype=torch.float32)
        ops.bct_to_btc(x, o0, S, so_box, frames=frames, index=index)
        return (stacked(0, V, pair), stacked(2 * V, Cc, pair) if Cc else None, so_box, stacked(o0 + S, E, False))

    @staticmethod
    def _embed(h, convs, norms, mask2, out, post_add=None):
        ops = _ops()
        last = len(convs) - 1
        if last == 0 and post_add is None and ops.conv_ln_ok(h, convs[0].conv.weight, convs[0].conv.bias, norms[0].weight, norms[0].bias):
            c, nm = convs[0].conv, norms[0]
            return ops.conv_ln(h, c.weight, c.bias, row_mask=mask2, gamma=nm.weight.reshape(-1), beta=nm.bias.reshape(-1), relu=True,
                               out=out, pair=ops.pair_mode())
        for i, (conv, norm) in enumerate(zip(convs, norms)):
            h = ops.conv_gemm(h, conv.conv.weight, conv.conv.bias, row_mask=mask2)
            h = norm.cl(h, relu=True, out=out if i == last else None, pair=ops.pair_mode(), post_add=post_add if i == last else None)
        return h

    def cl(self, x, mask):
        assert x.shape[1] == self.in_channels(), f"expected {self.in_channels()} input channels, got {x.shape[1]}"
        return self.cl_parts(*self._unpack(x.contiguous()), mask)

    def cl_parts(self, vis, clip, so_box, ent, mask):
        return self.pair_stage(self.entity_stage(vis, clip, ent, torch.cat([mask, mask], dim=0)), so_box, mask)

    def entity_reach(self):
        win = self.mha_win_size[0]
        if self.use_abs_pe:
            return None
        if win <= 1 or any(c.kernel_size[0] != 1 for c in self.visual_bbox_fuse.layers):
            return None
        return self.arch[0] + 1 + win // 2

    def _position_rows(self, mask2):
        n, T = mask2.shape
        pe = self.pos_embd
        if self.training:
            assert T <= self.max_len, "Reached max length."
        elif T >= self.max_len:
            pe = torch.nn.functional.interpolate(pe, T, mode='linear', align_corners=False)
        rows = pe[0, :, :T].t()
        return (rows[None] * mask2[..., None].to(rows.dtype)).reshape(n * T, -1).contiguous()

    def entity_stage(self, vis, clip, ent, mask2):
        ops = _ops()
        n, T = mask2.shape
        Cc = self.n_clip
        D = self.s_fuse_norm.num_channels
        new = lambda *shape: torch.empty(*shape, device=mask2.device, dtype=torch.float32)

        pair = ops.pair_mode()
        cat = (lambda t: ops.Pair(t, D)) if pair else (lambda t: t)

        fuse_in = new(n, T, 2 * D)
        pe = self._position_rows(mask2) if self.use_abs_pe else None
        if Cc:
            vc = new(n, T, 2 * D)
            a = self._embed(vis, self.visual_embd, self.visual_embd_norm, mask2, vc[..., :D])
            b = self._embed(clip, self.clip_embd, self.clip_embd_norm, mask2, vc[..., D:])
            a = self.visual_clip_fuse.cl(cat(ops.join(vc, (a, b))), row_mask=mask2, out=fuse_in[..., :D], out_pair=pair, res=pe)
        else:
            a = self._embed(vis, self.visual_embd, self.visual_embd_norm, mask2, fuse_in[..., :D], post_add=pe)
        b = self._embed(ent, [self.bbox_entity_embd], [self.bbox_entity_norm], mask2, fuse_in[..., D:])
        so = self.visual_bbox_fuse.cl(cat(ops.join(fuse_in, (a, b))), row_mask=mask2)
        so, _ = self.stem[0].cl(so, mask2)
        return so

    def pair_stage(self, so, so_box, mask):
        ops = _ops()
        B, T = mask.shape
        D = self.s_fuse_norm.num_channels
        dev = mask.device
        mask2 = torch.cat([mask, mask], dim=0)
        new = lambda *shape: torch.empty(*shape, device=dev, dtype=torch.float32)
        pair = ops.pair_mode()
        cat = (lambda t: ops.Pair(t, D)) if pair else (lambda t: t)

        for i, (s_attn, o_attn) in enumerate(zip(self.s_attn, self.o_attn)):
            if i:
                so, _ = self.stem[i].cl(so, mask2)
            s, o = so[:B], so[B:]
            nxt = new(2 * B, T, D)
            s2, _ = s_attn.cl(s, o, mask, mask, stream_add=s, out=nxt[:B])
            o2, _ = o_attn.cl(o, s, mask, mask, stream_add=o, out=nxt[B:])
            so = ops.join(nxt, (s2, o2), dim=0)

        so_in = new(B, T, 2 * D)
        a = self.s_fuse_norm.cl(so[:B], out=so_in[..., :D], pair=pair)
        b = self.o_fuse_norm.cl(so[B:], out=so_in[..., D:], pair=pair)
        pair_box = new(B, T, 2 * D)
        a = self.so_fuse.cl(cat(ops.join(so_in, (a, b))), row_mask=mask, out=pair_box[..., :D], out_pair=pair)
        conv = self.bbox_so_embd.conv
        if ops.conv_ln_ok(so_box, conv.weight, conv.bias):
            b = ops.conv_ln(so_box, conv.weight, conv.bias, row_mask=mask, out=pair_box[..., D:], pair=pair)
        else:
            b = ops.conv_gemm(so_box, conv.weight, conv.bias, row_mask=mask, out=pair_box[..., D:], out_pair=pair)
        e = self.so_visual_bbox_fuse.cl(cat(ops.join(pair_box, (a, b))), row_mask=mask)

        feats, masks = [e], [mask]
        for blk in self.branch:
            e, mask = blk.cl(e, mask)
            feats.append(e)
            masks.append(mask)
        return feats, masks

    def forward(self, x, mask):
        feats, masks = self.cl(x, _mask2d(mask))
        return tuple(_from_cl(f) for f in feats), tuple(m[:, None, :] for m in masks)


class MaskConvTransformerBackboneWithCLIP(MaskConvTransformerBackbone):

    def __init__(self, n_visual, n_clip, n_bbox_entity, n_bbox_so, n_embd, n_head, n_embd_ks, fuse_ks, n_fuse_head,
                 fuse_path_drop, fuse_qx_stride, fuse_kv_stride, max_len, arch=(2, 2, 3), mha_win_size=[-1] * 4,
                 scale_factor=2, with_ln=False, attn_pdrop=0.0, proj_pdrop=0.0, path_pdrop=0.0, use_abs_pe=False,
                 use_rel_pe=False, use_local=True):
        super().__init__(n_visual=n_visual, n_bbox_entity=n_bbox_entity, n_bbox_so=n_bbox_so, n_embd=n_embd,
                         n_head=n_head, n_embd_ks=n_embd_ks, fuse_ks=fuse_ks, n_fuse_head=n_fuse_head,
                         fuse_path_drop=fuse_path_drop, fuse_qx_stride=fuse_qx_stride, fuse_kv_stride=fuse_kv_stride,
                         max_len=max_len, arch=arch, mha_win_size=mha_win_size, scale_factor=scale_factor,
                         with_ln=with_ln, attn_pdrop=attn_pdrop, proj_pdrop=proj_pdrop, path_pdrop=path_pdrop,
                         use_abs_pe=use_abs_pe, use_rel_pe=use_rel_pe, use_local=use_local)
        self.n_clip = n_clip
        self.clip_embd, self.clip_embd_norm = self._embedding(n_clip, n_embd, n_embd_ks, arch[0])
        self.visual_clip_fuse = ConvMLP(n_embd * 2, n_embd, n_embd, kernel_size=fuse_ks, num_layers=2)
        self._zero_biases()
```

### vrdone_amd/models/blocks.py

```python
import math

import torch
from torch import nn

from .transformer import _get_activation_fn


def _ops():
    from .. import ops
    return ops


def _mask2d(mask):
    return mask.reshape(mask.shape[0], mask.shape[-1]).contiguous()


def _from_cl(x_cl):
    return _ops().btc_to_bct(x_cl)


def _to_cl(x):
    return _ops().to_channels_last(x)


class MaskedConv1D(nn.Module):

    def __init__(self, in_channels, out_channels, kernel_size, stride=1, padding=0, dilation=1, groups=1,
                 bias=True, padding_mode='zeros'):
        super().__init__()
        assert kernel_size % 2 == 1 and kernel_size // 2 == padding
        self.stride = stride
        self.conv = nn.Conv1d(in_channels, out_channels, kernel_size, stride, padding, dilation, groups, bias,
                              padding_mode)
        if bias:
            nn.init.zeros_(self.conv.bias)

    def cl(self, x, mask, out=None):
        ops = _ops()
        conv = self.conv
        assert x.shape[1] % self.stride == 0
        m_out = mask if self.stride == 1 else mask[:, ::self.stride].contiguous()
        if conv.groups == 1:
            assert self.stride == 1, "dense strided conv is not on the path"
            y = ops.conv_gemm(x, conv.weight, conv.bias, row_mask=m_out, out=out)
        else:
            assert conv.groups == conv.out_channels, "only depthwise / 2-in-per-group convs are on the path"
            y, = ops.dwconv_ln(x, [dict(weight=conv.weight, bias=conv.bias, out=out)], mask_out=m_out,
                               stride=self.stride)
        return y, m_out

    def forward(self, x, mask, downsample=True):
        assert downsample or self.stride == 1
        y, m = self.cl(_to_cl(x), _mask2d(mask))
        return _from_cl(y), m[:, None, :]


class LayerNorm(nn.Module):

    def __init__(self, num_channels, eps=1e-5, affine=True, device=None, dtype=None):
        super().__init__()
        assert affine and eps == 1e-5, "the fused kernels implement the affine, eps=1e-5 form used on the path"
        self.num_channels, self.eps, self.affine = num_channels, eps, affine
        kw = {'device': device, 'dtype': dtype}
        self.weight = nn.Parameter(torch.ones(1, num_channels, 1, **kw))
        self.bias = nn.Parameter(torch.zeros(1, num_channels, 1, **kw))

    def cl(self, x, relu=False, post_add=None, out=None, pair=False):
        return _ops().layernorm(x, self.weight, self.bias, relu=relu, post_add=post_add, out=out, pair=pair)

    def forward(self, x):
        assert x.dim() == 3 and x.shape[1] == self.num_channels
        return _from_cl(self.cl(_to_cl(x)))


def get_sinusoid_encoding(n_position, d_hid):
    import numpy as np
    pos = np.arange(n_position, dtype=np.float64)[:, None]
    j = np.arange(d_hid)[None, :]
    angle = pos / np.power(10000.0, 2 * (j // 2) / d_hid)
    return torch.tensor(np.where(j % 2 == 0, np.sin(angle), np.cos(angle)), dtype=torch.float32).unsqueeze(0).transpose(1, 2)


class ConvMLP(nn.Module):

    def __init__(self, input_dim, hidden_dim, output_dim, num_layers, kernel_size=1, act_layer='gelu', drop=0.0,
                 with_bias=True):
        super().__init__()
        assert kernel_size == 1 and act_layer == 'gelu' and drop == 0.0
        self.num_layers = num_layers
        dims = [input_dim] + [hidden_dim] * (num_layers - 1) + [output_dim]
        self.layers = nn.ModuleList(nn.Conv1d(a, b, 1, bias=with_bias) for a, b in zip(dims[:-1], dims[1:]))
        for layer in self.layers:
            if layer.bias is not None:
                nn.init.zeros_(layer.bias)

    def cl(self, x, row_mask=None, out=None, out_pair=False, res=None):
        ops = _ops()
        last = self.num_layers - 1
        for i, layer in enumerate(self.layers):
            if i < last:
                x = ops.conv_gemm(x, layer.weight, layer.bias, act=ops.ACT_GELU, out_pair=ops.pair_mode(), skip_rows=row_mask)
            else:
                x = ops.conv_gemm(x, layer.weight, layer.bias, row_mask=row_mask, out=out, out_pair=out_pair, res=res)
        return x

    def forward(self, x):
        return _from_cl(self.cl(_to_cl(x)))


class _FactorPool:
    POOL = 4096

    def __init__(self):
        self.pools = {}

    def reset(self):
        self.pools.clear()

    def take(self, n, keep_prob, device):
        capturing = torch.cuda.is_current_stream_capturing()
        key = (device, keep_prob)
        ent = self.pools.get(key)
        if ent is None or ent[2] != capturing or ent[1] + n > ent[0].numel():
            size = max(self.POOL, n)
            ent = self.pools[key] = [torch.floor(keep_prob + torch.rand(size, device=device)) / keep_prob, 0, capturing]
        out = ent[0][ent[1]:ent[1] + n]
        ent[1] += n
        return out


_factor_pool = _FactorPool()


class AffineDropPath(nn.Module):

    def __init__(self, num_dim, drop_prob=0.0, init_scale_value=1e-4):
        super().__init__()
        self.scale = nn.Parameter(init_scale_value * torch.ones(1, num_dim, 1))
        self.drop_prob = drop_prob
        self.keep = None

    def row_factors(self, n_samples, rows_per_sample, device):
        if not self.training or self.drop_prob == 0.0 or not torch.is_grad_enabled():
            return None
        keep_prob = 1.0 - self.drop_prob
        if self.keep is not None:
            assert self.keep.numel() >= n_samples
            factors = self.keep[:n_samples].to(device=device, dtype=torch.float32) / keep_prob
        else:
            factors = _factor_pool.take(n_samples, keep_prob, torch.device(device))
        return factors[:, None].expand(n_samples, rows_per_sample).contiguous().view(-1)

    def forward(self, x):
        y = x * self.scale
        rf = self.row_factors(x.shape[0], 1, x.device)
        return y if rf is None else y * rf.view(-1, 1, 1)


class Scale(nn.Module):

    def __init__(self, init_value=1.0):
        super().__init__()
        self.scale = nn.Parameter(torch.tensor(init_value, dtype=torch.float32))

    def forward(self, x):
        return x * self.scale


class _ConvAttention(nn.Module):

    def _build(self, n_embd, n_head, q_kernel, kv_kernel, stride):
        assert n_embd % n_head == 0
        self.n_embd, self.n_head = n_embd, n_head
        self.n_channels = n_embd // n_head
        self.scale = 1.0 / math.sqrt(self.n_channels)
        for name, ks in (("query", q_kernel), ("key", kv_kernel), ("value", kv_kernel)):
            setattr(self, f"{name}_conv", MaskedConv1D(n_embd, n_embd, ks, stride=stride, padding=ks // 2,
                                                        groups=n_embd, bias=False))
            setattr(self, f"{name}_norm", LayerNorm(n_embd))
        self.key = nn.Conv1d(n_embd, n_embd, 1)
        self.query = nn.Conv1d(n_embd, n_embd, 1)
        self.value = nn.Conv1d(n_embd, n_embd, 1)
        self.attn_drop, self.proj_drop = nn.Dropout(0.0), nn.Dropout(0.0)
        self.proj = nn.Conv1d(n_embd, n_embd, 1)

    def _branch_set(self, name):
        conv, norm = getattr(self, f"{name}_conv"), getattr(self, f"{name}_norm")
        return dict(weight=conv.conv.weight, gamma=norm.weight, beta=norm.bias, pair=_ops().pair_mode())

    def _groups(self, q_in, k_in, v_in, q_mask, kv_mask, pre_ln=None, pre_ln_on="qkv"):
        specs = [("query", q_in, q_mask, "q"), ("key", k_in, kv_mask, "k"), ("value", v_in, kv_mask, "v")]
        groups = []
        for name, x, m, tag in specs:
            ks = getattr(self, f"{name}_conv").conv.kernel_size
            use_ln = pre_ln is not None and tag in pre_ln_on
            for g in groups:
                if g[0] is x and g[1] is m and g[2] == use_ln and g[3] == ks:
                    g[4].append(name)
                    break
            else:
                groups.append((x, m, use_ln, ks, [name]))
        return groups

    def _prep(self, q_in, k_in, v_in, q_mask, kv_mask, stride=1, pre_ln=None, pre_ln_on="qkv"):
        ops = _ops()
        outs = {}
        for x, m, use_ln, _, names in self._groups(q_in, k_in, v_in, q_mask, kv_mask, pre_ln, pre_ln_on):
            res = ops.dwconv_ln(x, [self._branch_set(n) for n in names], mask_out=m, stride=stride,
                                pre_ln=pre_ln if use_ln else None)
            outs.update(zip(names, res))
        return outs["query"], outs["key"], outs["value"]

    def _project(self, q, k, v, out_pair=False, q_mask=None, kv_mask=None):
        ops = _ops()
        return tuple(ops.conv_gemm_batch([
            ((q, self.query.weight, self.query.bias), dict(out_pair=out_pair, skip_rows=q_mask)),
            ((k, self.key.weight, self.key.bias), dict(out_pair=out_pair, skip_rows=kv_mask)),
            ((v, self.value.weight, self.value.bias), dict(out_pair=out_pair, skip_rows=kv_mask))]))


def make_rel_pe(n_embd, n_head, window_size):
    rel_pe = nn.Parameter(torch.zeros(1, 1, n_head, window_size))
    nn.init.trunc_normal_(rel_pe, std=(2.0 / n_embd) ** 0.5)
    return rel_pe


class LocalMaskedMHCA(_ConvAttention):

    def __init__(self, n_embd, n_head, window_size, n_qx_stride=1, n_kv_stride=1, attn_pdrop=0.0, proj_pdrop=0.0,
                 use_rel_pe=False):
        super().__init__()
        assert window_size > 1 and window_size % 2 == 1
        assert n_qx_stride == n_kv_stride and n_kv_stride in (1, 2)
        assert attn_pdrop == 0.0 and proj_pdrop == 0.0
        self.window_size, self.window_overlap = window_size, window_size // 2
        self.use_rel_pe = use_rel_pe
        self.n_qx_stride, self.n_kv_stride = n_qx_stride, n_kv_stride
        ks = n_kv_stride + 1 if n_kv_stride > 1 else 3
        self._build(n_embd, n_head, ks, ks, n_kv_stride)
        self.rel_pe = make_rel_pe(n_embd, n_head, window_size) if use_rel_pe else None

    def cl(self, x, mask, mask_out=None, pre_ln=None, **epilogue):
        ops = _ops()
        s = self.n_kv_stride
        if mask_out is None:
            mask_out = mask if s == 1 else mask[:, ::s].contiguous()
        q, k, v = self._prep(x, x, x, mask_out, mask_out, stride=s, pre_ln=pre_ln)
        q, k, v = self._project(q, k, v, q_mask=mask_out, kv_mask=mask_out)
        att = ops.local_attention(q, k, v, mask_out, self.n_head, self.window_overlap, pair=ops.pair_mode(),
                                  rel_pe=self.rel_pe)
        return ops.conv_gemm(att, self.proj.weight, self.proj.bias, row_mask=mask_out, **epilogue), mask_out

    def forward(self, x, mask):
        assert (x.shape[-1] // self.n_kv_stride) % (2 * self.window_overlap) == 0
        y, m = self.cl(_to_cl(x), _mask2d(mask))
        return _from_cl(y), m[:, None, :]


class MaskedMHCA(_ConvAttention):

    def __init__(self, n_embd, n_head, n_qx_stride=1, n_kv_stride=1, attn_pdrop=0.0, proj_pdrop=0.0):
        super().__init__()
        assert n_qx_stride == n_kv_stride and n_kv_stride in (1, 2), "built for equal query / key-value strides 1 or 2"
        assert attn_pdrop == 0.0 and proj_pdrop == 0.0
        self.n_qx_stride, self.n_kv_stride = n_qx_stride, n_kv_stride
        ks = n_kv_stride + 1 if n_kv_stride > 1 else 3
        self._build(n_embd, n_head, ks, ks, n_kv_stride)

    def cl(self, x, mask, mask_out=None, pre_ln=None, **epilogue):
        ops = _ops()
        s = self.n_kv_stride
        if mask_out is None:
            mask_out = mask if s == 1 else mask[:, ::s].contiguous()
        q, k, v = self._prep(x, x, x, mask_out, mask_out, stride=s, pre_ln=pre_ln)
        qkv_pair = ops.flash_pair_ok(self.n_head, self.n_embd, q.shape[1])
        q, k, v = self._project(q, k, v, out_pair=qkv_pair, q_mask=mask_out, kv_mask=mask_out)
        att = ops.attention(q, k, v, mask_out, self.n_head, pair=ops.pair_mode(), q_mask=mask_out)
        return ops.conv_gemm(att, self.proj.weight, self.proj.bias, row_mask=mask_out, **epilogue), mask_out

    def forward(self, x, mask):
        y, m = self.cl(_to_cl(x), _mask2d(mask))
        return _from_cl(y), m[:, None, :]


class MaskedMHA(nn.Module):

    def __init__(self, n_embd, n_head, attn_pdrop=0.0, proj_pdrop=0.0):
        super().__init__()
        assert n_embd % n_head == 0 and attn_pdrop == 0.0 and proj_pdrop == 0.0
        self.n_embd, self.n_head = n_embd, n_head
        self.n_channels = n_embd // n_head
        self.scale = 1.0 / math.sqrt(self.n_channels)
        self.key = nn.Conv1d(n_embd, n_embd, 1)
        self.query = nn.Conv1d(n_embd, n_embd, 1)
        self.value = nn.Conv1d(n_embd, n_embd, 1)
        self.attn_drop, self.proj_drop = nn.Dropout(0.0), nn.Dropout(0.0)
        self.proj = nn.Conv1d(n_embd, n_embd, 1)

    def cl_qkv(self, q_in, k_in, v_in, q_mask, kv_mask, **epilogue):
        ops = _ops()
        q = ops.conv_gemm(q_in, self.query.weight, self.query.bias)
        k = ops.conv_gemm(k_in, self.key.weight, self.key.bias)
        v = ops.conv_gemm(v_in, self.value.weight, self.value.bias)
        att = ops.attention(q, k, v, kv_mask, self.n_head)
        return ops.conv_gemm(att, self.proj.weight, self.proj.bias, row_mask=q_mask, **epilogue), q_mask

    def forward(self, x, mask):
        m = _mask2d(mask)
        xc = _to_cl(x)
        y, _ = self.cl_qkv(xc, xc, xc, m, m)
        return _from_cl(y), mask


class TransformerBlock(nn.Module):

    def __init__(self, n_embd, n_head, n_ds_strides=(1, 1), n_out=None, n_hidden=None, act_layer=nn.GELU,
                 attn_pdrop=0.0, proj_pdrop=0.0, path_pdrop=0.0, mha_win_size=-1, use_rel_pe=False):
        super().__init__()
        assert len(n_ds_strides) == 2 and act_layer is nn.GELU
        self.ln1 = LayerNorm(n_embd)
        self.ln2 = LayerNorm(n_embd)
        if mha_win_size > 1:
            self.attn = LocalMaskedMHCA(n_embd, n_head, window_size=mha_win_size, n_qx_stride=n_ds_strides[0],
                                        n_kv_stride=n_ds_strides[1], attn_pdrop=attn_pdrop, proj_pdrop=proj_pdrop,
                                        use_rel_pe=use_rel_pe)
        else:
            self.attn = MaskedMHCA(n_embd, n_head, n_qx_stride=n_ds_strides[0], n_kv_stride=n_ds_strides[1],
                                   attn_pdrop=attn_pdrop, proj_pdrop=proj_pdrop)
        s = n_ds_strides[0]
        self.pool_skip = nn.MaxPool1d(s + 1, stride=s, padding=(s + 1) // 2) if s > 1 else nn.Identity()
        n_hidden = n_hidden or 4 * n_embd
        n_out = n_out or n_embd
        assert n_out == n_embd
        self.mlp = nn.Sequential(nn.Conv1d(n_embd, n_hidden, 1), act_layer(), nn.Dropout(proj_pdrop, inplace=True),
                                 nn.Conv1d(n_hidden, n_out, 1), nn.Dropout(proj_pdrop, inplace=True))
        if path_pdrop > 0.0:
            self.drop_path_attn = AffineDropPath(n_embd, drop_prob=path_pdrop)
            self.drop_path_mlp = AffineDropPath(n_out, drop_prob=path_pdrop)
        else:
            self.drop_path_attn = nn.Identity()
            self.drop_path_mlp = nn.Identity()

    @staticmethod
    def _scale(dp):
        return dp.scale if isinstance(dp, AffineDropPath) else None

    @staticmethod
    def _drop(dp, mask):
        return dp.row_factors(mask.shape[0], mask.shape[1], mask.device) if isinstance(dp, AffineDropPath) else None

    def cl(self, x, mask, out=None):
        ops = _ops()
        if self.attn.n_kv_stride > 1:
            skip, m_out = ops.maxpool_mask(x, mask)
        else:
            skip, m_out = x, mask
        y, _ = self.attn.cl(x, mask, m_out, pre_ln=(self.ln1.weight, self.ln1.bias),
                            scale=self._scale(self.drop_path_attn), row_scale=self._drop(self.drop_path_attn, m_out),
                            res=skip, res_masked=True)
        h = self.ln2.cl(y, pair=ops.pair_mode())
        h = ops.conv_gemm(h, self.mlp[0].weight, self.mlp[0].bias, act=ops.ACT_GELU, out_pair=ops.pair_mode(), skip_rows=m_out)
        y = ops.conv_gemm(h, self.mlp[3].weight, self.mlp[3].bias, row_mask=m_out, scale=self._scale(self.drop_path_mlp),
# ... 8 lines not shown
```

### vrdone_amd/models/fpns.py

```python
from torch import nn

from .blocks import LayerNorm, MaskedConv1D, _from_cl, _mask2d, _ops, _to_cl


class FPN1D_Fuse(nn.Module):
    def __init__(self, in_channels, out_channel, scale_factor=2.0, start_level=0, end_level=-1, with_ln=True,
                 norm_first=False):
        super().__init__()
        assert isinstance(in_channels, (list, tuple))
        assert with_ln and norm_first and start_level == 0 and int(scale_factor) == 2, \
            "built for the shipped configs: fpn_with_ln, fpn_norm_first, start level 0, scale factor 2"
        self.in_channels, self.out_channel, self.scale_factor = in_channels, out_channel, scale_factor
        self.start_level = start_level
        self.end_level = len(in_channels) if end_level == -1 else end_level
        assert self.start_level < self.end_level <= len(in_channels)

        self.input_norms = nn.ModuleList()
        self.lateral_convs = nn.ModuleList()
        self.fpn_convs = nn.ModuleList()
        self.lateral_norms = nn.ModuleList()
        self.fpn_norms = nn.ModuleList()
        for i in range(self.start_level, self.end_level):
            top = i == self.end_level - 1
            self.input_norms.append(LayerNorm(in_channels[i]))
            self.lateral_convs.append(None if top else MaskedConv1D(in_channels[i], out_channel, 1, bias=False))
            self.lateral_norms.append(None if top else LayerNorm(out_channel))
            self.fpn_convs.append(MaskedConv1D(in_channels[i] if top else out_channel, out_channel, 3, padding=1,
                                               bias=False, groups=out_channel))
            self.fpn_norms.append(LayerNorm(out_channel))
        self.mask_features = MaskedConv1D(out_channel, out_channel, 3, padding=1, groups=out_channel)

    def cl(self, feats, masks):
        ops = _ops()
        y = None
        for l in range(len(self.lateral_convs) - 1, -1, -1):
            x = self.input_norms[l].cl(feats[l], pair=ops.pair_mode() and self.lateral_convs[l] is not None)
            fpn = dict(weight=self.fpn_convs[l].conv.weight, gamma=self.fpn_norms[l].weight, beta=self.fpn_norms[l].bias)
            if self.lateral_convs[l] is None:
                y, = ops.dwconv_ln(x, [fpn], mask_out=masks[l])
            else:
                c = ops.conv_gemm(x, self.lateral_convs[l].conv.weight, None, row_mask=masks[l])
                c = self.lateral_norms[l].cl(c)
                y, = ops.dwconv_ln(c, [fpn], mask_out=masks[l], x_up=y)
        mf = self.mask_features.conv
        out, = ops.dwconv_ln(y, [dict(weight=mf.weight, bias=mf.bias)], mask_out=masks[0])
        return out, masks[0]

    def forward(self, inputs, fpn_masks):
        assert len(inputs) == len(self.in_channels) == len(fpn_masks)
        out, m = self.cl([_to_cl(x) for x in inputs], [_mask2d(m) for m in fpn_masks])
        return _from_cl(out), m[:, None, :]
```

### vrdone_amd/models/local_transformer.py

```python
from typing import Optional

import torch
from torch import nn, Tensor

from .blocks import (make_rel_pe, AffineDropPath, LayerNorm, MaskedMHA, _ConvAttention, _from_cl, _mask2d, _ops,
                     _to_cl)
from .transformer import _get_clones


class MaskedMHA_QKV(MaskedMHA):

    def forward(self, q, k, v, _qx_mask, _kv_mask, _attn_mask=None):
        assert _attn_mask is None
        y, _ = self.cl_qkv(_to_cl(q), _to_cl(k), _to_cl(v), _mask2d(_qx_mask), _mask2d(_kv_mask))
        return _from_cl(y), _qx_mask


def _qkv_kernel(stride):
    return stride + 1 if (stride > 1 or stride == 0) else 3


class MaskedMHCA_QKV(_ConvAttention):
    _half_win = None

    def __init__(self, n_embd, n_head, n_qx_stride=0, n_kv_stride=1, attn_pdrop=0.0, proj_pdrop=0.0):
        super().__init__()
        assert n_qx_stride in (0, 1) and n_kv_stride in (0, 1) and attn_pdrop == 0.0 and proj_pdrop == 0.0
        self.n_qx_stride, self.n_kv_stride = n_qx_stride, n_kv_stride
        self._build(n_embd, n_head, _qkv_kernel(n_qx_stride), _qkv_kernel(n_kv_stride), 1)

    def cl_qkv(self, q_in, k_in, v_in, q_mask, kv_mask, pre_ln=None, pre_ln_on="", **epilogue):
        ops = _ops()
        q, k, v = self._prep(q_in, k_in, v_in, q_mask, kv_mask, pre_ln=pre_ln, pre_ln_on=pre_ln_on)
        qkv_pair = self._half_win is None and ops.flash_pair_ok(self.n_head, self.n_embd, q.shape[1])
        q, k, v = self._project(q, k, v, out_pair=qkv_pair, q_mask=q_mask, kv_mask=kv_mask)
        if self._half_win is None:
            att = ops.attention(q, k, v, kv_mask, self.n_head, pair=ops.pair_mode(), q_mask=q_mask)
        else:
            assert q.shape[1] == k.shape[1]
            att = ops.local_attention(q, k, v, kv_mask, self.n_head, self._half_win, pair=ops.pair_mode(),
                                      rel_pe=getattr(self, "rel_pe", None))
        return ops.conv_gemm(att, self.proj.weight, self.proj.bias, row_mask=q_mask, **epilogue), q_mask

    def forward(self, q, k, v, _qx_mask, _kv_mask, _attn_mask=None):
        assert _attn_mask is None
        qc = _to_cl(q)
        kc = qc if k is q else _to_cl(k)
        vc = kc if v is k else (qc if v is q else _to_cl(v))
        qm = _mask2d(_qx_mask)
        km = qm if _kv_mask is _qx_mask else _mask2d(_kv_mask)
        y, _ = self.cl_qkv(qc, kc, vc, qm, km)
        return _from_cl(y), _qx_mask


class LocalMaskedMHCA_QKV(MaskedMHCA_QKV):

    def __init__(self, n_embd, n_head, window_size, n_qx_stride=0, n_kv_stride=1, attn_pdrop=0.0, proj_pdrop=0.0,
                 use_rel_pe=False):
        super().__init__(n_embd, n_head, n_qx_stride, n_kv_stride, attn_pdrop, proj_pdrop)
        assert window_size > 1 and window_size % 2 == 1
        self.window_size, self.window_overlap = window_size, window_size // 2
        self.use_rel_pe = use_rel_pe
        self._half_win = self.window_overlap
        self.rel_pe = make_rel_pe(n_embd, n_head, window_size) if use_rel_pe else None


class MaskedConvTransformerDecoderLayer(nn.Module):

    def __init__(self, n_embd, n_head, n_hidden=None, act_layer=nn.GELU, attn_pdrop=0.0, proj_pdrop=0.0,
                 path_pdrop=0.0, n_qx_stride=0, n_kv_stride=1, with_ffn=True, use_local=False, win_size=None,
                 use_rel_pe=False):
        super().__init__()
        assert n_qx_stride >= 0 and n_kv_stride >= 0 and act_layer is nn.GELU
        self.with_ffn = with_ffn
        self.ln1 = LayerNorm(n_embd)
        self.ln2 = LayerNorm(n_embd)
        if use_local:
            assert win_size is not None and n_qx_stride != 0 and n_kv_stride != 0, \
                "local decoder layers are built for the conv (stride 1) form only"
            self.self_attn = LocalMaskedMHCA_QKV(n_embd, n_head, window_size=win_size, n_qx_stride=n_qx_stride,
                                                 n_kv_stride=n_kv_stride, use_rel_pe=use_rel_pe)
            self.multihead_attn = LocalMaskedMHCA_QKV(n_embd, n_head, window_size=win_size, n_qx_stride=n_qx_stride,
                                                      n_kv_stride=n_kv_stride, use_rel_pe=use_rel_pe)
        else:
            if n_qx_stride == 0:
                self.self_attn = MaskedMHA_QKV(n_embd, n_head)
            else:
                self.self_attn = MaskedMHCA_QKV(n_embd, n_head, n_qx_stride=n_qx_stride, n_kv_stride=n_qx_stride)
            if n_kv_stride == 0:
                assert n_qx_stride == 0
                self.multihead_attn = MaskedMHA_QKV(n_embd, n_head)
            else:
                self.multihead_attn = MaskedMHCA_QKV(n_embd, n_head, n_qx_stride=n_qx_stride, n_kv_stride=n_kv_stride)
        if path_pdrop > 0.0:
            self.drop_path_attn1 = AffineDropPath(n_embd, drop_prob=path_pdrop)
            self.drop_path_attn2 = AffineDropPath(n_embd, drop_prob=path_pdrop)
        else:
            self.drop_path_attn1 = nn.Identity()
            self.drop_path_attn2 = nn.Identity()
        if with_ffn:
            self.ln3 = LayerNorm(n_embd)
            n_hidden = n_hidden or 4 * n_embd
            self.mlp = nn.Sequential(nn.Conv1d(n_embd, n_hidden, 1), act_layer(), nn.Dropout(proj_pdrop, inplace=True),
                                     nn.Conv1d(n_hidden, n_embd, 1), nn.Dropout(proj_pdrop, inplace=True))
            self.drop_path_mlp = AffineDropPath(n_embd, drop_prob=path_pdrop) if path_pdrop > 0.0 else nn.Identity()

    @staticmethod
    def _scale(dp):
        return dp.scale if isinstance(dp, AffineDropPath) else None

    @staticmethod
    def _drop(dp, tgt):
        return dp.row_factors(tgt.shape[0], tgt.shape[1], tgt.device) if isinstance(dp, AffineDropPath) else None

    def cl(self, tgt, memory, tgt_mask, memory_mask, query_pos=None, stream_add=None, out=None):
        ops = _ops()
        fuse1 = query_pos is None and isinstance(self.self_attn, MaskedMHCA_QKV)
        fuse2 = query_pos is None and isinstance(self.multihead_attn, MaskedMHCA_QKV)
        last = not self.with_ffn
        if fuse1:
            tgt, _ = self.self_attn.cl_qkv(tgt, tgt, tgt, tgt_mask, tgt_mask, pre_ln=(self.ln1.weight, self.ln1.bias),
                                           pre_ln_on="qk", scale=self._scale(self.drop_path_attn1),
                                           row_scale=self._drop(self.drop_path_attn1, tgt), res=tgt, res_masked=True)
        else:
            t2 = self.ln1.cl(tgt, post_add=query_pos)
            tgt, _ = self.self_attn.cl_qkv(t2, t2, tgt, tgt_mask, tgt_mask, scale=self._scale(self.drop_path_attn1),
                                           row_scale=self._drop(self.drop_path_attn1, tgt), res=tgt, res_masked=True)
        kw = dict(scale=self._scale(self.drop_path_attn2), row_scale=self._drop(self.drop_path_attn2, tgt), res=tgt,
                  res_masked=True, res2=stream_add if last else None, out=out if last else None)
        if fuse2:
            tgt, _ = self.multihead_attn.cl_qkv(tgt, memory, memory, tgt_mask, memory_mask,
                                                pre_ln=(self.ln2.weight, self.ln2.bias), pre_ln_on="q", **kw)
        else:
            t2 = self.ln2.cl(tgt, post_add=query_pos)
            tgt, _ = self.multihead_attn.cl_qkv(t2, memory, memory, tgt_mask, memory_mask, **kw)
        if self.with_ffn:
            assert stream_add is None
            t2 = self.ln3.cl(tgt)
            h = ops.conv_gemm(t2, self.mlp[0].weight, self.mlp[0].bias, act=ops.ACT_GELU)
            tgt = ops.conv_gemm(h, self.mlp[3].weight, self.mlp[3].bias, row_mask=tgt_mask, scale=self._scale(self.drop_path_mlp),
                                row_scale=self._drop(self.drop_path_mlp, tgt), res=tgt, out=out)
        return tgt, tgt_mask

    def forward(self, tgt, memory, tgt_mask: Optional[Tensor] = None, memory_mask: Optional[Tensor] = None,
                pos: Optional[Tensor] = None, query_pos: Optional[Tensor] = None, cross_first: bool = False,
                attn_mask: Optional[Tensor] = None):
        assert pos is None and not cross_first and attn_mask is None, "only the call form used on the path is built"
        qp = None
        if query_pos is not None:
            qp = query_pos[0].t().contiguous()
        tm = _mask2d(tgt_mask)
        mm = tm if memory_mask is tgt_mask else _mask2d(memory_mask)
        y, _ = self.cl(_to_cl(tgt), _to_cl(memory), tm, mm, query_pos=qp)
        return _from_cl(y), tgt_mask


class MaskedConvTransformerDecoder(nn.Module):

    def __init__(self, n_embd, n_head, n_hidden, attn_pdrop=0.0, proj_pdrop=0.0, path_pdrop=0.1, n_qx_stride=0,
                 n_kv_stride=1, num_layers=4, norm=None, return_intermediate=False, use_local=False, win_size=None,
                 use_rel_pe=False):
        super().__init__()
        layer = MaskedConvTransformerDecoderLayer(n_embd, n_head, n_hidden, attn_pdrop=attn_pdrop,
                                                  proj_pdrop=proj_pdrop, path_pdrop=path_pdrop,
                                                  n_qx_stride=n_qx_stride, n_kv_stride=n_kv_stride,
                                                  use_local=use_local, win_size=win_size, use_rel_pe=use_rel_pe)
        self.layers = _get_clones(layer, num_layers)
        self.num_layers = num_layers
        self.norm = norm
        self.return_intermediate = return_intermediate

    def cl(self, tgt, memory, memory_mask, query_pos, all_layers):
        outs = []
        for i, layer in enumerate(self.layers):
            tgt, _ = layer.cl(tgt, memory, None, memory_mask, query_pos=query_pos)
            if all_layers or i == self.num_layers - 1:
                outs.append(self.norm.cl(tgt))
        return outs


class MaskedConvTransformerDecoderOnly(nn.Module):

    def __init__(self, n_embd, n_head, n_hidden, attn_pdrop=0.0, proj_pdrop=0.0, path_pdrop=0.1, n_qx_stride=0,
                 n_kv_stride=1, num_layers=4, return_intermediate=False, use_local=False, win_size=None,
                 use_rel_pe=False):
        super().__init__()
        self.decoder = MaskedConvTransformerDecoder(n_embd, n_head, n_hidden, attn_pdrop=attn_pdrop,
                                                    proj_pdrop=proj_pdrop, path_pdrop=path_pdrop,
                                                    n_qx_stride=n_qx_stride, n_kv_stride=n_kv_stride,
                                                    num_layers=num_layers, norm=LayerNorm(n_embd),
                                                    return_intermediate=return_intermediate, use_local=use_local,
                                                    win_size=win_size, use_rel_pe=use_rel_pe)
        self.n_embd, self.n_head = n_embd, n_head
        for m in self.modules():
            if isinstance(m, (nn.Linear, nn.Conv1d)) and m.bias is not None:
                nn.init.zeros_(m.bias)

    def cl(self, src, src_mask, query_embed, all_layers):
        B = src.shape[0]
        tgt = torch.zeros(B, query_embed.shape[0], query_embed.shape[1], device=src.device, dtype=torch.float32)
        return self.decoder.cl(tgt, src, src_mask, query_embed, all_layers)
```

### vrdone_amd/models/ragged.py

```python
import torch

from .blocks import _ConvAttention, _ops


_MAX_SEGS = 32


class Layout:

    def __init__(self, buckets):
        self.segs, self.flat, off = [], [], 0
        self._tails = {}
        for n, T, flat in buckets:
            self.segs.append((off, n, T))
            self.flat.append(bool(flat))
            off += n * T
        assert self.flat == sorted(self.flat, reverse=True), "buckets that take the flat k = 3 convs come first"
        self.rows = off
        self.rows_flat = sum(n * T for (_, n, T), f in zip(self.segs, self.flat) if f)

    def twice(self):
        return self.segs + [(self.rows + off, n, T) for off, n, T in self.segs]

    def tail_rows(self, halves, device):
        key = (halves, str(device))
        if key not in self._tails:
            idx = [torch.arange(h * self.rows + off + T - 1, h * self.rows + off + n * T, T, dtype=torch.int64, device=device)
                   for h in range(halves) for (off, n, T), f in zip(self.segs, self.flat) if f]
            self._tails[key] = (torch.cat(idx) if len(idx) > 1 else idx[0]) if idx else None
        return self._tails[key]


def _part(x, off, n, T):
    if x is None:
        return None
    ops = _ops()
    if isinstance(x, ops.Pair):
        return ops.Pair(_part(x.t, off, n, T), x.width, x.fmt)
    return x[0, off:off + n * T].unflatten(0, (n, T))


def _mpart(m, off, n, T):
    return None if m is None else m[0, off:off + n * T].view(n, T)


def _merged(segs):
    if len(segs) > 1 and all(T == segs[0][2] for _, _, T in segs):
        return [(segs[0][0], sum(n for _, n, _ in segs), segs[0][2])]
    return segs


def _raw(x):
    return x.t if isinstance(x, _ops().Pair) else x


def _zero_rows(x, rows):
    _raw(x)[0].index_fill_(0, rows, 0.0)


def _dwconv_rows(x, sets, mask_out, segs, *, stride=1, x_up=None, pre_ln=None):
    ops = _ops()
    Cout = sets[0]["weight"].shape[0]
    rows_out = sum(n * (T // stride) for _, n, T in segs)
    bufs = [torch.empty(1, rows_out, Cout, device=x.device, dtype=torch.float32) for _ in sets]
    segs = _merged(segs)
    if len(segs) == 1:
        off, n, T = segs[0]
        oo, To = off // stride, T // stride
        ops.dwconv_ln(_part(x, off, n, T), [dict(st, out=_part(b, oo, n, To)) for st, b in zip(sets, bufs)],
                      mask_out=_mpart(mask_out, oo, n, To), stride=stride, x_up=_part(x_up, off // 2, n, T // 2), pre_ln=pre_ln)
    else:
        for g0 in range(0, len(segs), _MAX_SEGS):
            part = segs[g0:g0 + _MAX_SEGS]
            r0, r1 = part[0][0], part[-1][0] + part[-1][1] * part[-1][2]
            rel = [(off - r0, n, T) for off, n, T in part]
            ops.dwconv_ln(x[:, r0:r1], [dict(st, out=b[:, r0 // stride:r1 // stride]) for st, b in zip(sets, bufs)],
                          mask_out=None if mask_out is None else mask_out[:, r0 // stride:r1 // stride], stride=stride,
                          x_up=None if x_up is None else x_up[:, r0 // 2:r1 // 2], pre_ln=pre_ln, segs=rel)
    return [ops.Pair(b, Cout) if ops._fmt(st.get("pair")) else b for st, b in zip(sets, bufs)]


def _attention_rows(q, k, v, kv_mask, q_mask, n_head, qsegs, ksegs, *, half_win=None, rel_pe=None, pair=False, plain=False):
    ops = _ops()
    Cc = q.shape[-1]
    out = torch.empty(1, sum(n * T for _, n, T in qsegs), Cc, device=_raw(q).device, dtype=torch.float32)
    r = None
    if len(qsegs) > 1 and len(_merged(qsegs)) == 1 and len(_merged(ksegs)) == 1:
        qsegs, ksegs = _merged(qsegs), _merged(ksegs)
    if half_win is not None and 1 < len(qsegs) <= _MAX_SEGS:
        assert list(qsegs) == list(ksegs)
        r = ops.local_attention(q, k, v, kv_mask, n_head, half_win, pair=pair, rel_pe=rel_pe, out=out, segs=list(qsegs))
        return ops.Pair(out, Cc, r.fmt) if isinstance(r, ops.Pair) else out
    dev = _raw(q).device
    lanes = _lanes(dev) if half_win is None and len(qsegs) > 2 else None
    if lanes:
        main = torch.cuda.current_stream(dev)
        ready = torch.cuda.Event()
        ready.record(main)
        for lane in lanes:
            lane.wait_event(ready)
    for i, ((qo, n, Tq), (ko, nk, Tk)) in enumerate(zip(qsegs, ksegs)):
        assert n == nk
        o = _part(out, qo, n, Tq)
        if lanes and i % (len(lanes) + 1):
            with torch.cuda.stream(lanes[i % (len(lanes) + 1) - 1]):
                r = _attention_one(q, k, v, kv_mask, q_mask, n_head, (qo, n, Tq), (ko, nk, Tk), o, pair, plain)
            continue
        if half_win is not None:
            assert Tq == Tk
            r = ops.local_attention(_part(q, qo, n, Tq), _part(k, ko, n, Tk), _part(v, ko, n, Tk), _mpart(kv_mask, ko, n, Tk),
                                    n_head, half_win, pair=pair, rel_pe=rel_pe, out=o)
        elif plain:
            r = ops.attention(_part(q, qo, n, Tq), _part(k, ko, n, Tk), _part(v, ko, n, Tk), _mpart(kv_mask, ko, n, Tk), n_head, out=o)
        else:
            r = ops.attention(_part(q, qo, n, Tq), _part(k, ko, n, Tk), _part(v, ko, n, Tk), _mpart(kv_mask, ko, n, Tk), n_head,
                              pair=pair, q_mask=_mpart(q_mask, qo, n, Tq), out=o)
    if lanes:
        for lane in lanes:
            main.wait_stream(lane)
    return ops.Pair(out, Cc, r.fmt) if isinstance(r, ops.Pair) else out


def _attention_one(q, k, v, kv_mask, q_mask, n_head, qseg, kseg, o, pair, plain):
    ops = _ops()
    (qo, n, Tq), (ko, _, Tk) = qseg, kseg
    if plain:
        return ops.attention(_part(q, qo, n, Tq), _part(k, ko, n, Tk), _part(v, ko, n, Tk), _mpart(kv_mask, ko, n, Tk), n_head, out=o)
    return ops.attention(_part(q, qo, n, Tq), _part(k, ko, n, Tk), _part(v, ko, n, Tk), _mpart(kv_mask, ko, n, Tk), n_head,
                         pair=pair, q_mask=_mpart(q_mask, qo, n, Tq), out=o)


ATTN_LANES = int(__import__("os").environ.get("VRDONE_ROWS_ATTN_STREAMS", "2"))
_side_streams = {}


def _lanes(dev):
    if ATTN_LANES <= 1 or torch.cuda.is_current_stream_capturing():
        return None
    key = (dev.index if dev.index is not None else torch.cuda.current_device(), ATTN_LANES)
    if key not in _side_streams:
        _side_streams[key] = [torch.cuda.Stream(device=dev) for _ in range(ATTN_LANES - 1)]
    return _side_streams[key]


def _attn_rows(mod, q_in, k_in, v_in, q_mask, kv_mask, qsegs, ksegs, *, stride=1, pre_ln=None, pre_ln_on="", **epilogue):
    ops = _ops()
    if stride > 1:
        qsegs_o = ksegs_o = [(off // stride, n, T // stride) for off, n, T in qsegs]
    else:
        qsegs_o, ksegs_o = qsegs, ksegs
    if isinstance(mod, _ConvAttention):
        outs = {}
        for x, m, use_ln, _, names in mod._groups(q_in, k_in, v_in, q_mask, kv_mask, pre_ln, pre_ln_on):
            res = _dwconv_rows(x, [mod._branch_set(nm) for nm in names], m, qsegs if x is q_in else ksegs, stride=stride,
                               pre_ln=pre_ln if use_ln else None)
            outs.update(zip(names, res))
        q, k, v = outs["query"], outs["key"], outs["value"]
        half_win = getattr(mod, "_half_win", None)
        if half_win is None and hasattr(mod, "window_overlap"):
            half_win = mod.window_overlap
        qkv_pair = half_win is None and ops.flash_pair_ok(mod.n_head, mod.n_embd, min(T for _, _, T in qsegs_o))
        q, k, v = mod._project(q, k, v, out_pair=qkv_pair, q_mask=q_mask, kv_mask=kv_mask)
        att = _attention_rows(q, k, v, kv_mask, q_mask, mod.n_head, qsegs_o, ksegs_o, half_win=half_win,
                              rel_pe=getattr(mod, "rel_pe", None), pair=ops.pair_mode())
    else:
        q = ops.conv_gemm(q_in, mod.query.weight, mod.query.bias)
        k = ops.conv_gemm(k_in, mod.key.weight, mod.key.bias)
        v = ops.conv_gemm(v_in, mod.value.weight, mod.value.bias)
        att = _attention_rows(q, k, v, kv_mask, None, mod.n_head, qsegs_o, ksegs_o, plain=True)
    return ops.conv_gemm(att, mod.proj.weight, mod.proj.bias, row_mask=q_mask, **epilogue)


def _block(blk, x, mask, segs, out=None):
    ops = _ops()
    s = blk.attn.n_kv_stride
    if s > 1:
        assert s == 2
        rows_o = sum(n * (T // 2) for _, n, T in segs)
        skip = torch.empty(1, rows_o, x.shape[-1], device=x.device, dtype=torch.float32)
        m_out = torch.empty(1, rows_o, device=x.device, dtype=torch.bool)
        for off, n, T in segs:
            ops.maxpool_mask(_part(x, off, n, T), _mpart(mask, off, n, T), out=(_part(skip, off // 2, n, T // 2), _mpart(m_out, off // 2, n, T // 2)))
        segs_o = [(off // 2, n, T // 2) for off, n, T in segs]
    else:
        skip, m_out, segs_o = x, mask, segs
    y = _attn_rows(blk.attn, x, x, x, m_out, m_out, segs, segs, stride=s, pre_ln=(blk.ln1.weight, blk.ln1.bias), pre_ln_on="qkv",
                   scale=blk._scale(blk.drop_path_attn), res=skip, res_masked=True)
    h = blk.ln2.cl(y, pair=ops.pair_mode())
    h = ops.conv_gemm(h, blk.mlp[0].weight, blk.mlp[0].bias, act=ops.ACT_GELU, out_pair=ops.pair_mode(), skip_rows=m_out)
    y = ops.conv_gemm(h, blk.mlp[3].weight, blk.mlp[3].bias, row_mask=m_out, scale=blk._scale(blk.drop_path_mlp), res=y, out=out)
    return y, m_out, segs_o


def _decoder_layer(layer, tgt, memory, tgt_mask, memory_mask, qsegs, ksegs, *, query_pos=None, stream_add=None, out=None):
    ops = _ops()
    from .local_transformer import MaskedMHCA_QKV
    fuse1 = query_pos is None and isinstance(layer.self_attn, MaskedMHCA_QKV)
    fuse2 = query_pos is None and isinstance(layer.multihead_attn, MaskedMHCA_QKV)
    last = not layer.with_ffn
    kw1 = dict(scale=layer._scale(layer.drop_path_attn1), res=tgt, res_masked=True)
    if fuse1:
        tgt = _attn_rows(layer.self_attn, tgt, tgt, tgt, tgt_mask, tgt_mask, qsegs, qsegs, pre_ln=(layer.ln1.weight, layer.ln1.bias),
                         pre_ln_on="qk", **kw1)
    else:
        t2 = layer.ln1.cl(tgt, post_add=query_pos)
        tgt = _attn_rows(layer.self_attn, t2, t2, tgt, tgt_mask, tgt_mask, qsegs, qsegs, **kw1)
    kw = dict(scale=layer._scale(layer.drop_path_attn2), res=tgt, res_masked=True, res2=stream_add if last else None,
              out=out if last else None)
    if fuse2:
        tgt = _attn_rows(layer.multihead_attn, tgt, memory, memory, tgt_mask, memory_mask, qsegs, ksegs,
                         pre_ln=(layer.ln2.weight, layer.ln2.bias), pre_ln_on="q", **kw)
    else:
        t2 = layer.ln2.cl(tgt, post_add=query_pos)
        tgt = _attn_rows(layer.multihead_attn, t2, memory, memory, tgt_mask, memory_mask, qsegs, ksegs, **kw)
    if layer.with_ffn:
        assert stream_add is None
        t2 = layer.ln3.cl(tgt)
        h = ops.conv_gemm(t2, layer.mlp[0].weight, layer.mlp[0].bias, act=ops.ACT_GELU)
        tgt = ops.conv_gemm(h, layer.mlp[3].weight, layer.mlp[3].bias, row_mask=tgt_mask, scale=layer._scale(layer.drop_path_mlp),
                            res=tgt, out=out)
    return tgt


def _rows_of(x, sl):
    ops = _ops()
    return ops.Pair(x.t[:, sl], x.width, x.fmt) if isinstance(x, ops.Pair) else x[:, sl]


def _conv3_rows(h, conv, row_mask, lay, halves, tails, out=None, out_pair=False, norm=None):
    ops = _ops()
    assert conv.kernel_size[0] == 3
    N = conv.weight.shape[0]
    if out is None:
        out = torch.empty(1, halves * lay.rows, N, device=_raw(h).device, dtype=torch.float32)
    if tails is not None:
        _zero_rows(h, tails)
    small = ops.conv_ln_ok(h, conv.weight, conv.bias, *((norm.weight, norm.bias) if norm is not None else ()))
    assert small or norm is None

    def one(x, m, o):
        if small:
            ops.conv_ln(x, conv.weight, conv.bias, row_mask=m, out=o, pair=out_pair, relu=norm is not None,
                        gamma=None if norm is None else norm.weight.reshape(-1), beta=None if norm is None else norm.bias.reshape(-1))
        else:
            ops.conv_gemm(x, conv.weight, conv.bias, row_mask=m, out=o, out_pair=out_pair)
    for hf in range(halves):
        base = hf * lay.rows
        if lay.rows_flat:
            sl = slice(base, base + lay.rows_flat)
            one(_rows_of(h, sl), row_mask[:, sl], out[:, sl])
        for (off, n, T), flat in zip(lay.segs, lay.flat):
            if not flat:
                one(_part(h, base + off, n, T), _mpart(row_mask, base + off, n, T), _part(out, base + off, n, T))
    return ops.Pair(out, N) if out_pair else out


def _embed(h, convs, norms, mask2, out, lay, tails2):
    ops = _ops()
    last = len(convs) - 1
    if last == 0 and ops.conv_ln_ok(h, convs[0].conv.weight, convs[0].conv.bias, norms[0].weight, norms[0].bias):
        return _conv3_rows(h, convs[0].conv, mask2, lay, 2, tails2, out=out, out_pair=bool(ops.pair_mode()), norm=norms[0])
    for i, (conv, norm) in enumerate(zip(convs, norms)):
        h = _conv3_rows(h, conv.conv, mask2, lay, 2, tails2)
        h = norm.cl(h, relu=True, out=out if i == last else None, pair=ops.pair_mode())
    return h


def unpack_rows(bb, x, plan, lay):
    ops = _ops()
    R = lay.rows
    V, Cc, S, E = bb.n_visual, bb.n_clip, bb.n_bbox_so, bb.n_bbox_entity
    pair = ops.pair_mode()
    new = lambda rows, width: torch.empty(1, rows, width, device=x.device, dtype=torch.float32)

    def stacked(c0, width, as_pair):
        h = new(2 * R, width)
        for (off, n, T), bucket in zip(lay.segs, plan):
            t2, idx = bucket[0], bucket[1]
            ops.bct_to_btc(x, c0, width, _part(h, off, n, T), pair=as_pair, frames=t2, index=idx)
            ops.bct_to_btc(x, c0 + width, width, _part(h, R + off, n, T), pair=as_pair, frames=t2, index=idx)
        return ops.Pair(h, width) if as_pair else h

    o0 = 2 * V + 2 * Cc
    so_box = new(R, S)
    for (off, n, T), bucket in zip(lay.segs, plan):
        ops.bct_to_btc(x, o0, S, _part(so_box, off, n, T), frames=bucket[0], index=bucket[1])
    return stacked(0, V, pair), (stacked(2 * V, Cc, pair) if Cc else None), so_box, stacked(o0 + S, E, False)


def entity_rows(bb, vis, clip, ent, mask2, lay):
    ops = _ops()
    assert not bb.use_abs_pe, "absolute position rows are laid out per padded length: such models run bucket by bucket"
    dev = mask2.device
    R = lay.rows
    D = bb.s_fuse_norm.num_channels
    pair = ops.pair_mode()
    new = lambda rows, width: torch.empty(1, rows, width, device=dev, dtype=torch.float32)
    cat = (lambda t: ops.Pair(t, D)) if pair else (lambda t: t)
    tails2 = lay.tail_rows(2, dev)
    fuse_in = new(2 * R, 2 * D)
    if bb.n_clip:
        vc = new(2 * R, 2 * D)
        _embed(vis, bb.visual_embd, bb.visual_embd_norm, mask2, vc[..., :D], lay, tails2)
        _embed(clip, bb.clip_embd, bb.clip_embd_norm, mask2, vc[..., D:], lay, tails2)
        bb.visual_clip_fuse.cl(cat(vc), row_mask=mask2, out=fuse_in[..., :D], out_pair=pair)
    else:
        _embed(vis, bb.visual_embd, bb.visual_embd_norm, mask2, fuse_in[..., :D], lay, tails2)
    _embed(ent, [bb.bbox_entity_embd], [bb.bbox_entity_norm], mask2, fuse_in[..., D:], lay, tails2)
    so = bb.visual_bbox_fuse.cl(cat(fuse_in), row_mask=mask2)
    so, _, _ = _block(bb.stem[0], so, mask2, lay.twice())
    return so


def pair_rows(bb, so, so_box, mask, lay):
    ops = _ops()
    dev = mask.device
    R = lay.rows
    D = bb.s_fuse_norm.num_channels
    pair = ops.pair_mode()
    segs, segs2 = lay.segs, lay.twice()
    new = lambda rows, width: torch.empty(1, rows, width, device=dev, dtype=torch.float32)
    cat = (lambda t: ops.Pair(t, D)) if pair else (lambda t: t)
    mask2 = torch.cat([mask, mask], dim=1)
    for i, (s_attn, o_attn) in enumerate(zip(bb.s_attn, bb.o_attn)):
        if i:
            so, _, _ = _block(bb.stem[i], so, mask2, segs2)
        s, o = so[:, :R], so[:, R:]
        nxt = new(2 * R, D)
        _decoder_layer(s_attn, s, o, mask, mask, segs, segs, stream_add=s, out=nxt[:, :R])
        _decoder_layer(o_attn, o, s, mask, mask, segs, segs, stream_add=o, out=nxt[:, R:])
        so = nxt
    so_in = new(R, 2 * D)
    bb.s_fuse_norm.cl(so[:, :R], out=so_in[..., :D], pair=pair)
    bb.o_fuse_norm.cl(so[:, R:], out=so_in[..., D:], pair=pair)
    pair_box = new(R, 2 * D)
    bb.so_fuse.cl(cat(so_in), row_mask=mask, out=pair_box[..., :D], out_pair=pair)
    _conv3_rows(so_box, bb.bbox_so_embd.conv, mask, lay, 1, lay.tail_rows(1, dev), out=pair_box[..., D:], out_pair=pair)
    e = bb.so_visual_bbox_fuse.cl(cat(pair_box), row_mask=mask)

    feats, masks, lays = [e], [mask], [segs]
    for blk in bb.branch:
        e, mask, segs = _block(blk, e, mask, segs)
        feats.append(e)
        masks.append(mask)
        lays.append(segs)
    return feats, masks, lays


def backbone_rows(bb, x, plan, lay, mask):
    vis, clip, so_box, ent = unpack_rows(bb, x, plan, lay)
    so = entity_rows(bb, vis, clip, ent, torch.cat([mask, mask], dim=1), lay)
    return pair_rows(bb, so, so_box, mask, lay)


def neck_rows(neck, feats, masks, lays):
    ops = _ops()
    y = None
    for l in range(len(neck.lateral_convs) - 1, -1, -1):
        x = neck.input_norms[l].cl(feats[l], pair=ops.pair_mode() and neck.lateral_convs[l] is not None)
        fpn = dict(weight=neck.fpn_convs[l].conv.weight, gamma=neck.fpn_norms[l].weight, beta=neck.fpn_norms[l].bias)
        if neck.lateral_convs[l] is None:
            y, = _dwconv_rows(x, [fpn], masks[l], lays[l])
        else:
            c = ops.conv_gemm(x, neck.lateral_convs[l].conv.weight, None, row_mask=masks[l])
            c = neck.lateral_norms[l].cl(c)
            y, = _dwconv_rows(c, [fpn], masks[l], lays[l], x_up=y)
    mf = neck.mask_features.conv
    out, = _dwconv_rows(y, [dict(weight=mf.weight, bias=mf.bias)], masks[0], lays[0])
    return out


def predictor_rows(pred, x, mask_features, mask, output_mask, ksegs, segs0, with_aux, fill=-10.0):
    ops = _ops()
    if with_aux is None:
        with_aux = pred.aux_loss
    src = pred.input_norm.cl(x, pair=ops.pair_mode() and pred.input_proj is not None)
    if pred.input_proj is not None:
        src = ops.conv_gemm(src, pred.input_proj.weight, pred.input_proj.bias, row_mask=mask)
    qe = pred.query_embed.weight
    Q, Cq = qe.shape
    B = sum(n for _, n, _ in ksegs)
    qsegs, p = [], 0
    for _, n, _ in ksegs:
        qsegs.append((p * Q, n, Q))
        p += n
    dec = pred.transformer.decoder
    tgt = torch.zeros(1, B * Q, Cq, device=_raw(src).device, dtype=torch.float32)
    hs = []
    all_layers = with_aux and pred.aux_loss
    for i, layer in enumerate(dec.layers):
        tgt = _decoder_layer(layer, tgt, src, None, mask, qsegs, ksegs, query_pos=qe)
        if all_layers or i == dec.num_layers - 1:
            hs.append(dec.norm.cl(tgt))
    heads = []
    for h in hs:
        h3 = h.view(B, Q, Cq)
        logits = ops.conv_gemm(h3, pred.class_embed.weight, pred.class_embed.bias)
        emb = pred.mask_embed.cl(h3)
        segs_out, p = [], 0
        for off, n, T in segs0:
            segs_out.append(ops.mask_head(emb[p:p + n], _part(mask_features, off, n, T), _mpart(output_mask, off, n, T), fill))
            p += n
        heads.append((logits, segs_out))
    return heads


def heads_rows(model, feats, masks, lays, with_aux):
    mask_features = neck_rows(model.neck, feats, masks, lays)
    return predictor_rows(model.predictor, feats[-1], mask_features, masks[-1], masks[0], lays[-1], lays[0], with_aux)


def filler_buckets(rows, t_max):
    need = (-rows) % 256
    if need == 0 or rows % 8 or rows < 65536:
        return []
    odd = need % 32
    first = 32 + odd if odd else 0
    if first > t_max or t_max < 32:
        return []
    if need < first:
        need += 256
    out = [(1, first)] if first else []
    if need - first:
        out.insert(0, ((need - first) // 32, 32))
    return out


def with_filler(buckets, make, t_max):
    fill = filler_buckets(sum(b[2] * b[0] for b in buckets), t_max)
    at = sum(1 for b in buckets if b[-1])
    return list(buckets[:at]) + [make(n, T) for n, T in fill] + list(buckets[at:]), set(range(at, at + len(fill)))


def mask_vrd_rows(model, x, masks2d, plan, with_aux, out=None):
    B, T = masks2d.shape
    dev = x.device
    plan, filler = with_filler(plan, lambda n, t: (t, plan[0][1][:1].repeat(n), n, True), T)
    lay = Layout([(n, t2, flat) for t2, _, n, flat in plan])
    idx64 = [b[1].long() for b in plan]
    mask = torch.cat([masks2d[i64, :b[0]].reshape(-1) if j not in filler else torch.zeros(b[2] * b[0], dtype=torch.bool, device=dev)
                      for j, (b, i64) in enumerate(zip(plan, idx64))]).view(1, lay.rows)
    heads = heads_rows(model, *backbone_rows(model.backbone, x, plan, lay, mask), with_aux)
    fill = -10.0
    if out is None:
        Q, K1 = heads[-1][0].shape[1:]
        new = lambda: {"pred_logits": torch.empty(B, Q, K1, device=dev), "pred_masks": torch.full((B, Q, T), fill, device=dev)}
        out = new()
        if len(heads) > 1:
            out["aux_outputs"] = [new() for _ in heads[:-1]]
    for dst, (logits, segs) in zip(out.get("aux_outputs", []) + [out], heads):
        p = 0
        for j, (b, i64, seg) in enumerate(zip(plan, idx64, segs)):
            if j not in filler:
                dst["pred_logits"][i64] = logits[p:p + b[2]]
                dst["pred_masks"][i64, :, :b[0]] = seg
            p += b[2]
    return out
```

### vrdone_amd/ops.py

```python
import ctypes as C
import os

import torch

from . import _hip
from ._hip import ACT_GELU, ACT_NONE, ACT_RELU, lib


_raw_stream = getattr(torch._C, "_cuda_getCurrentRawStream", None)


def _stream():
    if _raw_stream is not None:
        return C.c_void_p(_raw_stream(torch.cuda.current_device()))
    return C.c_void_p(torch.cuda.current_stream().cuda_stream)


def _rows(t):
    if not t.is_cuda:
        raise RuntimeError("vrdone_amd ops need HIP tensors (no CPU path exists for the hot path)")
    if t.dtype != torch.float32:
        raise TypeError(f"expected float32, got {t.dtype}")
    if t.stride(-1) != 1:
        raise ValueError("channels-last operand must have unit stride along channels")
# ... 540 lines not shown
    pa, rows, cols, lda = _rows(x)
    assert cols == Cin, f"input has {cols} channels, weight expects {Cin}"
    T = x.shape[-2]
    if out is None:
        out = torch.empty(*x.shape[:-1], N, device=x.device, dtype=torch.float32)
    pc, rows_c, cols_c, ldc = _rows(out)
    assert rows_c == rows and cols_c == N
    a = _hip.GemmArgs()
    if _dgrad:
        assert (Cin * k) % 32 == 0 and not a_width
        wt = split_conv_weight_dgrad(weight, _bfmt)
        a.W = wt.data_ptr()
        wt.set_args(a)
        if wt.fmt == _hip.PAIR_F16:
            assert _a_scale is not None
            a.a_scale = _a_scale.data_ptr()
    else:
        a.W = _param_ptr(packed_conv_weight(weight), x, "conv weight")
    a.A, a.lda, a.bias = pa, lda, _param_ptr(bias, x, "conv bias")
    a.C, a.ldc = pc, ldc
    a.M, a.N, a.Cin, a.taps, a.T = rows, N, Cin, k, T
    a.act = act
    a.row_mask = _mask_ptr(row_mask, rows)
    a.scale = _param_ptr(scale, x, "drop-path scale")
    if a_width:
        assert pair_fmt() and x_fmt == pair_fmt() and Cin % 32 == 0, "pair input needs the split-precision mode it was made in and Cin % 32 == 0"
    w_fmt = pair_fmt() if _split_fmt is None else _split_fmt
    if _dgrad:
        w_fmt = a.split_fmt
    assert not (a_width and w_fmt != x_fmt) and not (out_pair and w_fmt != pair_fmt())
    if not _dgrad and w_fmt and (Cin * k) % 32 == 0:
        split_conv_weight(weight, w_fmt).set_args(a)
        if w_fmt == _hip.PAIR_F16 and _split_fmt is None:
            a.products = products()
    a.a_pair_width = a_width
    a.c_pair = _fmt(out_pair)
    if skip_rows is None:
        skip_rows = row_mask
    f32_kernel = not a_width and not _dgrad and not (w_fmt and (Cin * k) % 32 == 0)
    if _skip_padding and skip_rows is not None and (a_width or f32_kernel) and rows >= SKIP_MIN_ROWS and skip_rows.numel() == rows:
        blocks = row_blocks(skip_rows)
        if blocks is not None:
            a.row_blocks, a.row_blocks_active = blocks[0].data_ptr(), blocks[1].data_ptr()
            a.row_block_seg_len = blocks[2]
    if res is not None:
        pr, rr, rc, ldr = _rows(res)
        assert rr == rows and rc == N
        a.res, a.ldres, a.res_masked = pr, ldr, 1 if res_masked else 0
    if res2 is not None:
        pr, rr, rc, ldr = _rows(res2)
        assert rr == rows and rc == N
        a.res2, a.ldres2 = pr, ldr
    if _launch is not None:
        _launch.append(a)
    else:
        _hip.check(lib.vrd_gemm(C.byref(a), _stream()), "vrd_gemm")
    return Pair(out, N, a.c_pair) if a.c_pair else out


def conv_gemm_batch(calls):
    assert 1 <= len(calls) <= 4
    if torch.is_grad_enabled():
        return [conv_gemm(*args, **kwargs) for args, kwargs in calls]
    collected, results = [], []
    for args, kwargs in calls:
        results.append(conv_gemm(*args, _launch=collected, **kwargs))
    arr = (_hip.GemmArgs * len(collected))(*collected)
    _hip.check(lib.vrd_gemm_batch(arr, len(collected), _stream()), "vrd_gemm_batch")
    return results


def layernorm(x, gamma, beta, *, relu=False, post_add=None, out=None, pair=False):
    if recording(x, gamma, beta, post_add):
        from . import autograd
        assert not pair
        return autograd.layernorm(x, gamma, beta, relu=relu, post_add=post_add)
    px, rows, cols, ldx = _rows(x)
    if out is None:
        out = torch.empty(*x.shape, device=x.device, dtype=torch.float32)
    py, rows_y, cols_y, ldy = _rows(out)
    assert rows_y == rows and cols_y == cols
    pa, lda, period = None, 0, 0
    if post_add is not None:
        pa, period, ca, lda = _rows(post_add)
        assert ca == cols
    assert gamma.numel() == cols and beta.numel() == cols
    _hip.check(lib.vrd_layernorm(px, ldx, py, ldy, rows, cols, _param_ptr(gamma, x, "LayerNorm weight"),
                                 _param_ptr(beta, x, "LayerNorm bias"), 1 if relu else 0,
                                 pa, lda, period, _fmt(pair), _stream()), "vrd_layernorm")
    return Pair(out, cols) if _fmt(pair) else out


CONV_LN_MAXK = 32
_conv_ln_on = os.environ.get("VRDONE_CONV_LN", "1") != "0"


def conv_ln_ok(x, weight, *tensors):
    N, Cin, k = weight.shape
    return (_conv_ln_on and not isinstance(x, Pair) and k in (1, 3) and Cin * k <= CONV_LN_MAXK and (3 + k) * Cin <= 64 and N in (256, 512) and
            not recording(x, weight, *tensors))


def conv_ln(x, weight, bias, *, row_mask=None, gamma=None, beta=None, relu=False, out=None, pair=False):
    N, Cin, k = weight.shape
    px, rows, cols, ldx = _rows(x)
    assert cols == Cin and weight.is_contiguous()
    if out is None:
        out = torch.empty(*x.shape[:-1], N, device=x.device, dtype=torch.float32)
    py, rows_y, cols_y, ldy = _rows(out)
    assert rows_y == rows and cols_y == N
    a = _hip.ConvLnArgs()
    a.x, a.ldx, a.rows = px, ldx, rows
    a.Cin, a.taps, a.T, a.N = Cin, k, x.shape[-2], N
    a.w, a.bias = _param_ptr(weight, x, "conv weight"), _param_ptr(bias, x, "conv bias")
    a.row_mask = _mask_ptr(row_mask, rows)
    a.gamma, a.beta = _param_ptr(gamma, x, "LayerNorm weight"), _param_ptr(beta, x, "LayerNorm bias")
    a.relu = 1 if relu else 0
    a.y, a.ldy, a.out_pair = py, ldy, _fmt(pair)
    _hip.check(lib.vrd_conv_ln(C.byref(a), _stream()), "vrd_conv_ln")
    return Pair(out, N) if a.out_pair else out


_CONST_ROWS = {}


def _const_row(n, fill, device):
    key = (n, float(fill), str(device))
    t = _CONST_ROWS.get(key)
    if t is None:
        t = _CONST_ROWS[key] = torch.full((n,), fill, device=device, dtype=torch.float32)
    return t


def _dwconv_block(w, bias, gamma, beta):
    parts = (w, bias, gamma, beta)
    key = tuple((t.data_ptr(), t._version) if t is not None else None for t in parts)
    hit = getattr(w, "_vrd_dw_block", None)
    capturing = _capturing()
    if hit is not None and hit[0] == key and not capturing:
        return hit[1]
    Cout, g, k = w.shape
    one = lambda t, fill: _const_row(Cout, fill, w.device) if t is None else t.detach().float().reshape(-1)
    val = torch.cat([w.detach().float().permute(1, 2, 0).reshape(-1), one(bias, 0.0), one(gamma, 1.0), one(beta, 0.0)]).contiguous()
    if capturing:
        return _keep_for_capture(val)
    w._vrd_dw_block = (key, val)
    return val


def dwconv_ln(x, sets, *, mask_out=None, stride=1, x_up=None, pre_ln=None, segs=None):
    if recording(x, x_up, *(t for st in sets for t in (st["weight"], st.get("bias"), st.get("gamma"), st.get("beta"))),
                 *(pre_ln or ())):
        from . import autograd
        return autograd.dwconv_ln(x, sets, mask_out=mask_out, stride=stride, x_up=x_up, pre_ln=pre_ln)
    B, Tin, Cx = x.shape
    w0 = sets[0]["weight"]
    Cout, g, k = w0.shape
    px, rows, cols, ldx = _rows(x)
    assert cols == Cout * g
    Tout = Tin // stride
    a = _hip.DwconvLnArgs()
    seg_table = None
    if segs is not None:
        assert B == 1 and sum(n * T for _, n, T in segs) == Tin
        seg_table = _hip.RowSegs.of(segs)
        a.segs = C.pointer(seg_table)
    a.x, a.ldx = px, ldx
    if x_up is not None:
        pu, ru, cu, ldu = _rows(x_up)
        assert cu == cols and ru * 2 == rows
        a.x_up, a.ldx_up = pu, ldu
    a.B, a.Tin, a.C, a.ksize, a.stride, a.group_in = B, Tin, Cout, k, stride, g
    if pre_ln is not None:
        assert g == 1 and x_up is None
        a.pre_gamma, a.pre_beta = _param_ptr(pre_ln[0], x, "LayerNorm weight"), _param_ptr(pre_ln[1], x, "LayerNorm bias")
    a.mask_out = _mask_ptr(mask_out, B * Tout)
    a.n_out = len(sets)
    outs = []
    for i, s in enumerate(sets):
        assert tuple(s["weight"].shape) == (Cout, g, k) and s["weight"].is_contiguous()
        o = s.get("out")
        if o is None:
            o = torch.empty(B, Tout, Cout, device=x.device, dtype=torch.float32)
        po, ro, co, ldo = _rows(o)
        assert ro == B * Tout and co == Cout
        a.w[i], a.bias[i] = _param_ptr(s["weight"], x, "depthwise weight"), _param_ptr(s.get("bias"), x, "depthwise bias")
        a.gamma[i], a.beta[i] = (_param_ptr(s.get("gamma"), x, "LayerNorm weight"),
                                 _param_ptr(s.get("beta"), x, "LayerNorm bias"))
        a.packed[i] = _dwconv_block(s["weight"], s.get("bias"), s.get("gamma"), s.get("beta")).data_ptr()
        a.relu[i] = 1 if s.get("relu") else 0
        a.y[i], a.ldy[i] = po, ldo
        a.out_pair[i] = _fmt(s.get("pair"))
        outs.append(Pair(o, Cout) if _fmt(s.get("pair")) else o)
    _hip.check(lib.vrd_dwconv_ln(C.byref(a), _stream()), "vrd_dwconv_ln")
    return outs


def _rel_pe_ptr(rel_pe, like, n_head, half_win):
    if rel_pe is None:
        return None
    assert rel_pe.numel() == n_head * (2 * half_win + 1) and rel_pe.dtype == torch.float32 and rel_pe.is_contiguous()
    assert rel_pe.device == like.device
    return rel_pe.data_ptr()


def local_attention(q, k, v, mask, n_head, half_win, pair=False, rel_pe=None, out=None, segs=None):
    if recording(q, k, v, rel_pe):
        from . import autograd
        return autograd.LocalAttention.apply(q, k, v, mask, n_head, half_win, rel_pe)
    B, T, Cc = q.shape
    rel = _rel_pe_ptr(rel_pe, q, n_head, half_win)
    pq, rows, cols, ld = _rows(q)
    pk, _, _, ldk = _rows(k)
    pv, _, _, ldv = _rows(v)
    assert ld == ldk == ldv
    if out is None:
        out = torch.empty(B, T, Cc, device=q.device, dtype=torch.float32)
    assert out.shape == (B, T, Cc) and out.is_contiguous()
    if segs is not None:
        assert B == 1 and sum(n * t for _, n, t in segs) == T
        table = _hip.RowSegs.of(segs)
        _hip.check(lib.vrd_local_attn_segs(pq, pk, pv, ld, _mask_ptr(mask, rows), rel, C.byref(table), Cc, n_head, half_win,
                                           out.data_ptr(), Cc, _fmt(pair), _stream()), "vrd_local_attn_segs")
        return Pair(out, Cc) if _fmt(pair) else out
    _hip.check(lib.vrd_local_attn(pq, pk, pv, ld, _mask_ptr(mask, rows), rel, B, T, Cc, n_head, half_win,
                                  out.data_ptr(), Cc, _fmt(pair), _stream()), "vrd_local_attn")
    return Pair(out, Cc) if _fmt(pair) else out


def attention(q, k, v, kv_mask, n_head, algo=0, pair=False, q_mask=None, out=None):
    if not isinstance(q, Pair) and recording(q, k, v):
        from . import autograd
        return autograd.Attention.apply(q, k, v, kv_mask, n_head)
    if isinstance(q, Pair):
        assert isinstance(k, Pair) and isinstance(v, Pair) and q.width == k.width == v.width == q.shape[-1]
        assert q.fmt == k.fmt == v.fmt
        fmt = q.fmt
        q, k, v = q.t, k.t, v.t
        B, Tq, Cc = q.shape
        Tk = k.shape[1]
        pq, _, _, ldq = _rows(q)
        pk, rows_k, _, ldk = _rows(k)
        pv, _, _, ldv = _rows(v)
        assert ldk == ldv
        if out is None:
            out = torch.empty(B, Tq, Cc, device=q.device, dtype=torch.float32)
        assert out.shape == (B, Tq, Cc) and out.is_contiguous()
        _hip.check(lib.vrd_attention_pair(pq, ldq, pk, pv, ldk, _mask_ptr(kv_mask, rows_k), _mask_ptr(q_mask, B * Tq), B, Tq, Tk, n_head,
                                          Cc // n_head, out.data_ptr(), Cc, fmt if pair else 0, fmt, _stream(),
                                          products() if fmt == _hip.PAIR_F16 else 0),
                   "vrd_attention_pair")
        return Pair(out, Cc, fmt) if pair else out
    B, Tq, Cc = q.shape
    Tk = k.shape[1]
    pq, _, _, ldq = _rows(q)
    pk, rows_k, _, ldk = _rows(k)
    pv, _, _, ldv = _rows(v)
    assert ldk == ldv
    if out is None:
        out = torch.empty(B, Tq, Cc, device=q.device, dtype=torch.float32)
    assert out.shape == (B, Tq, Cc) and out.is_contiguous()
    hd = Cc // n_head
    flash = algo == 2 or (algo == 0 and hd in (64, 128))
    pair = bool(pair and flash and pair_fmt())
    _hip.check(lib.vrd_attention(pq, ldq, pk, pv, ldk, _mask_ptr(kv_mask, rows_k), B, Tq, Tk, n_head, hd,
                                 out.data_ptr(), Cc, algo, _fmt(pair), _stream()), "vrd_attention")
    return Pair(out, Cc) if pair else out


def maxpool_mask(x, mask_in, out=None):
    if recording(x):
        from . import autograd
        return autograd.MaxPoolMask.apply(x, mask_in)
    B, T, Cc = x.shape
    px, rows, cols, ldx = _rows(x)
    if out is None:
        y = torch.empty(B, T // 2, Cc, device=x.device, dtype=torch.float32)
        m_out = torch.empty(B, T // 2, device=x.device, dtype=torch.bool)
    else:
        y, m_out = out
        assert y.shape == (B, T // 2, Cc) and y.is_contiguous() and m_out.shape == (B, T // 2) and m_out.is_contiguous()
        assert m_out.dtype == torch.bool
    _hip.check(lib.vrd_maxpool_mask(px, ldx, B, T, Cc, _mask_ptr(mask_in, rows), y.data_ptr(), Cc, m_out.data_ptr(),
                                    _stream()), "vrd_maxpool_mask")
    return y, m_out


def mask_head(emb, feat, out_mask, fill=-10.0):
    if recording(emb, feat):
        from . import autograd
        return autograd.MaskHead.apply(emb, feat, out_mask, fill)
    B, Q, Dp = emb.shape
    T = feat.shape[1]
    pe, _, _, lde = _rows(emb)
    pf, rows_f, _, ldf = _rows(feat)
    seg = torch.empty(B, Q, T, device=emb.device, dtype=torch.float32)
    _hip.check(lib.vrd_mask_head(pe, lde, pf, ldf, _mask_ptr(out_mask, rows_f), B, Q, T, Dp, fill, seg.data_ptr(),
                                 _stream()), "vrd_mask_head")
    return seg


def assign_tables(sizes, dev):
    first, at = [], 0
    for n in sizes:
        first.append(at)
        at += n
    return torch.tensor(first, dtype=torch.int32, device=dev), torch.tensor(sizes, dtype=torch.int32, device=dev)


def assign(cost, sizes, tables=None):
    assert cost.is_cuda and cost.dtype == torch.float32 and cost.dim() == 2 and cost.stride(1) == 1
    G, Q = cost.shape
    assert sum(sizes) == G and max(sizes) <= Q <= 16
    first_d, count_d = tables if tables is not None else assign_tables(sizes, cost.device)
    out = torch.full((G,), -1, dtype=torch.int32, device=cost.device)
    _hip.check(lib.vrd_assign(cost.data_ptr(), cost.stride(0), first_d.data_ptr(), count_d.data_ptr(), len(sizes), Q,
                              out.data_ptr(), _stream()), "vrd_assign")
    return out


def postprocess(logits, masks, valid_len, topk):
    P, Q, K1 = logits.shape
    T = masks.shape[-1]
    assert logits.is_contiguous() and masks.is_contiguous() and valid_len.dtype == torch.int32
    dev = logits.device
    ts = torch.empty(P, Q, topk, device=dev, dtype=torch.float32)
    tc = torch.empty(P, Q, topk, device=dev, dtype=torch.int32)
    sf = torch.empty(P, Q, device=dev, dtype=torch.int32)
    sl = torch.empty(P, Q, device=dev, dtype=torch.int32)
    _hip.check(lib.vrd_postprocess(logits.data_ptr(), masks.data_ptr(), valid_len.data_ptr(), P, Q, K1, T, topk,
                                   ts.data_ptr(), tc.data_ptr(), sf.data_ptr(), sl.data_ptr(), _stream()),
               "vrd_postprocess")
    return ts, tc, sf, sl


def select_triplets(cand, s_score, o_score, so_offset, so_start, so_end, video_pairs, feat_stride, pred_min_frames, n_max_pair,
                    max_video_pairs):
    P, Q, W = cand.shape
    k = (W - 2) // 2
    n_videos = video_pairs.shape[0] - 1
    assert cand.is_contiguous() and cand.dtype == torch.float32 and W == 2 * k + 2 and n_videos >= 1
    for t in (s_score, o_score):
        assert t.dtype == torch.float32 and t.shape == (P,) and t.is_contiguous()
# ... 16 lines not shown
```

Baseline: 15800.

## Merge subject/object dwconv_ln launches into one multi-set kernel with mixed input LayerNorm

Extends the depthwise-conv+LayerNorm kernel to up to six output sets, with a per-set flag choosing whether the set reads the input-LayerNormed row or the raw row. The subject/object decoder layers now prepare the self- and cross-attention Q/K/V convs of both streams in shared launches, each input row read once. The FPN lateral LayerNorm is also folded into the dwconv with an x_up add. The aim is fewer launches and less re-reading of the same activations. In exchange, wider workgroups (6 or 8 waves) need more LDS and extra registers to hold the normalized and raw rows, which can lower occupancy.

```diff
diff --git a/include/vrdone_hip.h b/include/vrdone_hip.h
--- a/include/vrdone_hip.h
+++ b/include/vrdone_hip.h
@@ -138,26 +138,29 @@
     int64_t row[VRD_MAX_SEGS];
 } vrd_row_segs;
 
+#define VRD_DWCONV_MAX_SETS 6
 typedef struct {
     const float* x;  int64_t ldx;
     const float* x_up;  int64_t ldx_up;
     int32_t B, Tin, C, ksize, stride, group_in;
     const uint8_t* mask_out;
     int32_t n_out;
-    const float* w[3];
-    const float* bias[3];
-    const float* gamma[3];
-    const float* beta[3];
-    int32_t relu[3];
-    float* y[3];
-    int64_t ldy[3];
-    int32_t out_pair[3];
+    const float* w[VRD_DWCONV_MAX_SETS];
+    const float* bias[VRD_DWCONV_MAX_SETS];
+    const float* gamma[VRD_DWCONV_MAX_SETS];
+    const float* beta[VRD_DWCONV_MAX_SETS];
+    int32_t relu[VRD_DWCONV_MAX_SETS];
+    float* y[VRD_DWCONV_MAX_SETS];
+    int64_t ldy[VRD_DWCONV_MAX_SETS];
+    int32_t out_pair[VRD_DWCONV_MAX_SETS];
     const float* pre_gamma;
     const float* pre_beta;
-    const float* packed[3];
+    int32_t pre_ln_set[VRD_DWCONV_MAX_SETS];
+    const float* packed[VRD_DWCONV_MAX_SETS];
     const vrd_row_segs* segs;
 } vrd_dwconv_ln_args;
 int vrd_dwconv_ln(const vrd_dwconv_ln_args* a, void* stream);
+int vrd_dwconv_max_sets(void);
 
 int vrd_local_attn(const float* q, const float* k, const float* v, int64_t ld,
                    const uint8_t* mask, const float* rel_pe, int B, int T, int C, int n_head, int half_win,
diff --git a/vrdone_amd/_hip.py b/vrdone_amd/_hip.py
--- a/vrdone_amd/_hip.py
+++ b/vrdone_amd/_hip.py
@@ -67,14 +67,19 @@
         return s
 
 
+DWCONV_MAX_SETS = 6
+
+
 class DwconvLnArgs(C.Structure):
     _fields_ = [("x", c_f32p), ("ldx", C.c_int64), ("x_up", c_f32p), ("ldx_up", C.c_int64),
                 ("B", C.c_int32), ("Tin", C.c_int32), ("C", C.c_int32), ("ksize", C.c_int32),
                 ("stride", C.c_int32), ("group_in", C.c_int32),
                 ("mask_out", c_u8p), ("n_out", C.c_int32),
-                ("w", c_f32p * 3), ("bias", c_f32p * 3), ("gamma", c_f32p * 3), ("beta", c_f32p * 3),
-                ("relu", C.c_int32 * 3), ("y", c_f32p * 3), ("ldy", C.c_int64 * 3), ("out_pair", C.c_int32 * 3),
-                ("pre_gamma", c_f32p), ("pre_beta", c_f32p), ("packed", c_f32p * 3), ("segs", C.POINTER(RowSegs))]
+                ("w", c_f32p * DWCONV_MAX_SETS), ("bias", c_f32p * DWCONV_MAX_SETS), ("gamma", c_f32p * DWCONV_MAX_SETS),
+                ("beta", c_f32p * DWCONV_MAX_SETS), ("relu", C.c_int32 * DWCONV_MAX_SETS), ("y", c_f32p * DWCONV_MAX_SETS),
+                ("ldy", C.c_int64 * DWCONV_MAX_SETS), ("out_pair", C.c_int32 * DWCONV_MAX_SETS),
+                ("pre_gamma", c_f32p), ("pre_beta", c_f32p), ("pre_ln_set", C.c_int32 * DWCONV_MAX_SETS),
+                ("packed", c_f32p * DWCONV_MAX_SETS), ("segs", C.POINTER(RowSegs))]
 
 
 class ConvLnArgs(C.Structure):
@@ -135,6 +140,7 @@
 
 _SIGNATURES = {
     "vrd_abi_version": (C.c_int, []),
+    "vrd_dwconv_max_sets": (C.c_int, []),
     "vrd_last_error": (C.c_char_p, []),
     "vrd_f16_range_flag": (C.c_int, [C.POINTER(C.c_void_p)]),
     "vrd_prof_enable": (C.c_int, [C.c_int]),
@@ -247,6 +253,8 @@
     got = lib.vrd_abi_version()
     if got != ABI_VERSION:
         raise HipLibraryError(f"libvrdone_hip.so ABI {got} != expected {ABI_VERSION}: rebuild it")
+    if lib.vrd_dwconv_max_sets() != DWCONV_MAX_SETS:
+        raise HipLibraryError(f"libvrdone_hip.so has {lib.vrd_dwconv_max_sets()} dwconv_ln sets, the binding {DWCONV_MAX_SETS}: rebuild it")
     return lib
 
 
diff --git a/vrdone_amd/csrc/vrd_rowops.hip b/vrdone_amd/csrc/vrd_rowops.hip
--- a/vrdone_amd/csrc/vrd_rowops.hip
+++ b/vrdone_amd/csrc/vrd_rowops.hip
@@ -373,22 +373,28 @@
 
 constexpr int DW_RW = 16;
 
-template <int NV, int KS, int GIN>
-__global__ __launch_bounds__(256) void dwconv_ln_kernel(vrd_dwconv_ln_args p, int Tout_u, int strips_per_seq, int strips_per_wave, int rw, unsigned* rflag,
+template <int NV, bool BOTH, int WAVES, int NS>
+constexpr int DW_MIN_WAVES = (BOTH && NV == 2) ? (WAVES == 8 ? 4 : (WAVES == 6 || NS == 3) ? 3 : 1) : 1;
+
+template <int NV, int KS, int GIN, bool BOTH = false, int WAVES = 4, int NS = 3>
+__global__ __launch_bounds__(64 * WAVES) __attribute__((amdgpu_waves_per_eu(DW_MIN_WAVES<NV, BOTH, WAVES, NS>))) void dwconv_ln_kernel(vrd_dwconv_ln_args p, int Tout_u, int strips_per_seq, int strips_per_wave, int rw, unsigned* rflag,
                                                         vrd::SegTable sg) {
     vrd::RangeTrack rt;
     constexpr int C = 256 * NV, NT = GIN * KS, SETF = (NT + 3) * C;
     constexpr bool WIDE = NV == 2 && GIN == 1;
+    constexpr int NTHR = 64 * WAVES;
+    static_assert(NS <= VRD_DWCONV_MAX_SETS, "more sets than the argument struct holds");
+    static_assert(!BOTH || GIN == 1, "an input LayerNorm needs group_in == 1");
     extern __shared__ __attribute__((aligned(16))) float dw_lds[];
     const int lane = threadIdx.x & 63, wave = __builtin_amdgcn_readfirstlane(threadIdx.x >> 6);
     for (int o = 0; o < p.n_out; ++o) {
         float* const ls = dw_lds + o * SETF;
         if (p.packed[o]) {
-            for (int idx = threadIdx.x * 4; idx < SETF; idx += 1024) st4(ls + idx, ld4(p.packed[o] + idx));
+            for (int idx = threadIdx.x * 4; idx < SETF; idx += 4 * NTHR) st4(ls + idx, ld4(p.packed[o] + idx));
             continue;
         }
-        for (int idx = threadIdx.x; idx < C * NT; idx += 256) ls[(idx % NT) * C + idx / NT] = p.w[o][idx];
-        for (int c = threadIdx.x; c < C; c += 256) {
+        for (int idx = threadIdx.x; idx < C * NT; idx += NTHR) ls[(idx % NT) * C + idx / NT] = p.w[o][idx];
+        for (int c = threadIdx.x; c < C; c += NTHR) {
             ls[NT * C + c] = p.bias[o] ? p.bias[o][c] : 0.f;
             ls[(NT + 1) * C + c] = p.gamma[o] ? p.gamma[o][c] : 1.f;
             ls[(NT + 2) * C + c] = p.gamma[o] ? p.beta[o][c] : 0.f;
@@ -396,7 +402,7 @@
     }
     const float* const pre = dw_lds + p.n_out * SETF;
     if (p.pre_gamma)
-        for (int c = threadIdx.x; c < C; c += 256) {
+        for (int c = threadIdx.x; c < C; c += NTHR) {
             dw_lds[p.n_out * SETF + c] = p.pre_gamma[c];
             dw_lds[p.n_out * SETF + C + c] = p.pre_beta[c];
         }
@@ -405,7 +411,7 @@
     const int xcd = bid & 7, qq = nwg >> 3, rem = nwg & 7;
     const int lid = (xcd < rem ? xcd * (qq + 1) : rem * (qq + 1) + (xcd - rem) * qq) + (bid >> 3);
     for (int si = 0; si < strips_per_wave; ++si) {
-    const int64_t ws = ((int64_t)lid * 4 + wave) * strips_per_wave + si;
+    const int64_t ws = ((int64_t)lid * WAVES + wave) * strips_per_wave + si;
     int Tin, Tout, to0;
     int64_t xrow0, urow0, orow0;
     if (sg.count) {
@@ -425,6 +431,7 @@
 
     struct Row {
         float4 v[NV][GIN];
+        float4 n[BOTH ? NV : 1];
     };
     auto load_row = [&](int ti) {
         Row r;
@@ -437,15 +444,29 @@
                 if (ok) {
                     const int64_t coff = (int64_t)GIN * lane_chan<NV, WIDE>(i, lane) + 4 * g;
                     v = ld4(p.x + (xrow0 + ti) * p.ldx + coff);
-                    if (p.x_up) v = f4add(v, ld4(p.x_up + (urow0 + (ti >> 1)) * p.ldx_up + coff));
+                    if (p.x_up && !(GIN == 1 && p.pre_gamma)) v = f4add(v, ld4(p.x_up + (urow0 + (ti >> 1)) * p.ldx_up + coff));
                 }
                 r.v[i][g] = v;
             }
-        if (GIN == 1 && p.pre_gamma && ok) {
+        if constexpr (BOTH) {
+            if (ok) {
+#pragma unroll
+                for (int i = 0; i < NV; ++i) r.n[i] = r.v[i][0];
+                ln_rows<NV, WIDE>(r.n, pre, pre + C, lane, false);
+            } else {
+#pragma unroll
+                for (int i = 0; i < NV; ++i) r.n[i] = make_float4(0.f, 0.f, 0.f, 0.f);
+            }
+        } else if (GIN == 1 && p.pre_gamma && ok) {
             float4 t[NV];
 #pragma unroll
             for (int i = 0; i < NV; ++i) t[i] = r.v[i][0];
             ln_rows<NV, WIDE>(t, pre, pre + C, lane, false);
+            if (p.x_up) {
+#pragma unroll
+                for (int i = 0; i < NV; ++i)
+                    t[i] = f4add(t[i], ld4(p.x_up + (urow0 + (ti >> 1)) * p.ldx_up + lane_chan<NV, WIDE>(i, lane)));
+            }
 #pragma unroll
             for (int i = 0; i < NV; ++i) r.v[i][0] = t[i];
         }
@@ -456,7 +477,7 @@
         const bool mine = lane < to1 - to0 && p.mask_out[r0 + lane] != 0;
         if (!__any(mine)) {
 #pragma unroll
-            for (int o = 0; o < 3; ++o) {
+            for (int o = 0; o < NS; ++o) {
                 if (o >= p.n_out) break;
                 const float* const lb = dw_lds + o * SETF + (NT + 2) * C;
                 float4 val[NV];
@@ -505,10 +526,25 @@
         const int64_t row = orow0 + to;
         const float mk = p.mask_out ? (float)p.mask_out[row] : 1.f;
 #pragma unroll
-        for (int o = 0; o < 3; ++o) {
+        for (int o = 0; o < NS; ++o) {
             if (o >= p.n_out) break;
             const float* const ls = dw_lds + o * SETF;
+            const bool nrm = BOTH && p.pre_ln_set[o] != 0;
             float4 acc[NV];
+            if (nrm) {
+#pragma unroll
+                for (int i = 0; i < NV; ++i) {
+                    const int c = lane_chan<NV, WIDE>(i, lane);
+                    float4 r = *reinterpret_cast<const float4*>(ls + NT * C + c);
+#pragma unroll
+                    for (int k = 0; k < KS; ++k) {
+                        const float4 w = *reinterpret_cast<const float4*>(ls + k * C + c);
+                        const float4 v = win[k].n[BOTH ? i : 0];
+                        r.x += w.x * v.x; r.y += w.y * v.y; r.z += w.z * v.z; r.w += w.w * v.w;
+                    }
+                    acc[i] = make_float4(r.x * mk, r.y * mk, r.z * mk, r.w * mk);
+                }
+            } else {
 #pragma unroll
             for (int i = 0; i < NV; ++i) {
                 const int c = lane_chan<NV, WIDE>(i, lane);
@@ -530,6 +566,7 @@
                     }
                 }
                 acc[i] = make_float4(r.x * mk, r.y * mk, r.z * mk, r.w * mk);
+            }
             }
             if (p.gamma[o]) {
                 ln_rows<NV, WIDE>(acc, ls + (NT + 1) * C, ls + (NT + 2) * C, lane, p.relu[o] != 0);
@@ -824,9 +861,20 @@
     VRD_CHECK_ARG(a->group_in == 1 || (a->group_in == 2 && a->C == 256 && a->ksize == 3),
                   "vrd_dwconv_ln: group_in=2 is only built for C=256, ksize=3");
     VRD_CHECK_ARG(a->segs || (a->B > 0 && a->Tin > 0 && a->Tin % a->stride == 0), "vrd_dwconv_ln: Tin %% stride != 0");
-    VRD_CHECK_ARG(a->n_out >= 1 && a->n_out <= 3, "vrd_dwconv_ln: n_out must be 1..3");
-    VRD_CHECK_ARG((a->pre_gamma == nullptr) == (a->pre_beta == nullptr) && (!a->pre_gamma || (a->group_in == 1 && !a->x_up)),
-                  "vrd_dwconv_ln: input LayerNorm needs gamma and beta, group_in == 1 and no x_up");
+    VRD_CHECK_ARG(a->n_out >= 1 && a->n_out <= VRD_DWCONV_MAX_SETS, "vrd_dwconv_ln: n_out must be 1..%d", VRD_DWCONV_MAX_SETS);
+    VRD_CHECK_ARG((a->pre_gamma == nullptr) == (a->pre_beta == nullptr) && (!a->pre_gamma || a->group_in == 1),
+                  "vrd_dwconv_ln: input LayerNorm needs gamma and beta, and group_in == 1");
+    int n_ln = 0;
+    for (int o = 0; o < a->n_out; ++o) n_ln += a->pre_gamma && a->pre_ln_set[o] ? 1 : 0;
+    const bool both = n_ln > 0 && n_ln < a->n_out;
+    VRD_CHECK_ARG(!(a->pre_gamma && a->x_up) || a->C == 256, "vrd_dwconv_ln: input LayerNorm with x_up is built for C = 256");
+    VRD_CHECK_ARG(!both || (!a->x_up && a->ksize == 3), "vrd_dwconv_ln: sets with and without the input LayerNorm need ksize 3 and no x_up");
+    vrd_dwconv_ln_args local;
+    if (a->pre_gamma && n_ln == 0) {
+        local = *a;
+        local.pre_gamma = local.pre_beta = nullptr;
+        a = &local;
+    }
     VRD_CHECK_ARG(a->ldx >= (int64_t)a->C * a->group_in && a->ldx % 4 == 0 && aligned16(a->x), "vrd_dwconv_ln: bad x layout");
     VRD_CHECK_ARG(!a->x_up || (a->Tin % 2 == 0 && a->ldx_up % 4 == 0 && aligned16(a->x_up)), "vrd_dwconv_ln: bad x_up layout");
     for (int o = 0; o < a->n_out; ++o) {
@@ -856,10 +904,30 @@
                         4.0 * ((double)rows_in * a->C * a->group_in * (a->x_up ? 1.5 : 1.0) + (double)rows * a->C * a->n_out));
     const size_t lds = ((size_t)a->n_out * (a->group_in * a->ksize + 3) + (a->pre_gamma ? 2 : 0)) * a->C * sizeof(float);
     static const int rw_env = [] { const char* e = getenv("VRD_DW_RW"); return e ? atoi(e) : 0; }();
+    static const int waves_env = [] { const char* e = getenv("VRD_DW_WAVES"); return e ? atoi(e) : 0; }();
+    const bool many = a->n_out > 3;
+    VRD_CHECK_ARG(!many || (a->ksize == 3 && a->group_in == 1), "vrd_dwconv_ln: more than three sets need ksize 3 and group_in 1");
+    const bool wide_wg = a->C == 512 && lds > 40 * 1024;
+    const int waves = !wide_wg ? 4 : (waves_env == 4 || waves_env == 6 || waves_env == 8) ? waves_env : both ? 6 : 8;
+    using kernel_t = void (*)(vrd_dwconv_ln_args, int, int, int, int, unsigned*, vrd::SegTable);
+    kernel_t kern;
+    if (wide_wg)
+        kern = both ? (waves == 8 ? dwconv_ln_kernel<2, 3, 1, true, 8, 6> : waves == 6 ? dwconv_ln_kernel<2, 3, 1, true, 6, 6>
+                                                                                       : dwconv_ln_kernel<2, 3, 1, true, 4, 6>)
+                    : (waves == 8 ? dwconv_ln_kernel<2, 3, 1, false, 8, 6> : waves == 6 ? dwconv_ln_kernel<2, 3, 1, false, 6, 6>
+                                                                                        : dwconv_ln_kernel<2, 3, 1, false, 4, 6>);
+    else if (many) kern = both ? dwconv_ln_kernel<1, 3, 1, true, 4, 6> : dwconv_ln_kernel<1, 3, 1, false, 4, 6>;
+    else if (both) kern = a->C == 512 ? dwconv_ln_kernel<2, 3, 1, true> : dwconv_ln_kernel<1, 3, 1, true>;
+    else if (a->group_in == 2) kern = dwconv_ln_kernel<1, 3, 2>;
+    else if (a->C == 256) kern = a->ksize == 3 ? dwconv_ln_kernel<1, 3, 1> : dwconv_ln_kernel<1, 1, 1>;
+    else kern = a->ksize == 3 ? dwconv_ln_kernel<2, 3, 1> : dwconv_ln_kernel<2, 1, 1>;
+    if (lds > 48 * 1024)
+        if (int rc = vrd::reserve_lds(reinterpret_cast<const void*>(kern), lds, "vrd_dwconv_ln")) return rc;
     int rw = DW_RW;
     {
         const int64_t wgs_per_cu = lds ? (int64_t)(160 * 1024 / lds) : 8;
-        const int64_t resident = 256 * (wgs_per_cu < 1 ? 1 : wgs_per_cu > 4 ? 4 : wgs_per_cu) * 4;
+        const int64_t wg_max = 16 / waves;
+        const int64_t resident = 256 * (wgs_per_cu < 1 ? 1 : wgs_per_cu > wg_max ? wg_max : wgs_per_cu) * waves;
         auto strips_at = [&](int r) -> int64_t {
             return a->segs ? vrd::seg_table(sg, a->segs, a->stride, r) : (int64_t)a->B * ((Tout + r - 1) / r);
         };
@@ -877,17 +945,11 @@
     static const int spw_env = [] { const char* e = getenv("VRD_DW_SPW"); return e ? atoi(e) : 0; }();
     const int64_t total_strips = a->segs ? vrd::seg_table(sg, a->segs, a->stride, rw) : (int64_t)a->B * strips;
     const int spw = spw_env > 0 ? spw_env : 1;
-    dim3 grid((unsigned)((total_strips + 4 * spw - 1) / (4 * spw))), block(256);
+    dim3 grid((unsigned)((total_strips + waves * spw - 1) / (waves * spw))), block(64 * waves);
     bool any_f16 = false;
     for (int o = 0; o < a->n_out; ++o) any_f16 |= a->out_pair[o] == VRD_PAIR_F16;
     unsigned* const rflag = any_f16 ? vrd::range_flag() : nullptr;
-#define VRD_DW(NV, KS, GIN) hipLaunchKernelGGL((dwconv_ln_kernel<NV, KS, GIN>), grid, block, lds, s, *a, Tout, strips, spw, rw, rflag, sg)
-    if (a->group_in == 2) VRD_DW(1, 3, 2);
-    else if (a->C == 256 && a->ksize == 3) VRD_DW(1, 3, 1);
-    else if (a->C == 256) VRD_DW(1, 1, 1);
-    else if (a->ksize == 3) VRD_DW(2, 3, 1);
-    else VRD_DW(2, 1, 1);
-#undef VRD_DW
+    hipLaunchKernelGGL(kern, grid, block, lds, s, *a, Tout, strips, spw, rw, rflag, sg);
     VRD_LAUNCH_CHECK();
     return 0;
 }
diff --git a/vrdone_amd/csrc/vrd_runtime.hip b/vrdone_amd/csrc/vrd_runtime.hip
--- a/vrdone_amd/csrc/vrd_runtime.hip
+++ b/vrdone_amd/csrc/vrd_runtime.hip
@@ -143,6 +143,7 @@
 extern "C" {
 
 int vrd_abi_version(void) { return VRD_ABI_VERSION; }
+int vrd_dwconv_max_sets(void) { return VRD_DWCONV_MAX_SETS; }
 const char* vrd_last_error(void) { return vrd::g_err; }
 
 int vrd_f16_range_flag(void** flag) {
diff --git a/vrdone_amd/models/backbones.py b/vrdone_amd/models/backbones.py
--- a/vrdone_amd/models/backbones.py
+++ b/vrdone_amd/models/backbones.py
@@ -2,7 +2,7 @@
 from torch import nn
 
 from .blocks import ConvMLP, LayerNorm, MaskedConv1D, TransformerBlock, _from_cl, _mask2d, _ops, get_sinusoid_encoding
-from .local_transformer import MaskedConvTransformerDecoderLayer
+from .local_transformer import MaskedConvTransformerDecoderLayer, sos_prepare
 
 
 class MaskConvTransformerBackbone(nn.Module):
@@ -167,8 +167,11 @@
                 so, _ = self.stem[i].cl(so, mask2)
             s, o = so[:B], so[B:]
             nxt = new(2 * B, T, D)
-            s2, _ = s_attn.cl(s, o, mask, mask, stream_add=s, out=nxt[:B])
-            o2, _ = o_attn.cl(o, s, mask, mask, stream_add=o, out=nxt[B:])
+            launch = lambda x, sets, pre_ln: ops.dwconv_ln(x, sets, mask_out=mask, pre_ln=pre_ln)
+            ps = sos_prepare(s_attn, o_attn, s, mask, mask, launch) or (None, None)
+            po = sos_prepare(o_attn, s_attn, o, mask, mask, launch) or (None, None)
+            s2, _ = s_attn.cl(s, o, mask, mask, stream_add=s, out=nxt[:B], have_self=ps[0], have_cross=po[1])
+            o2, _ = o_attn.cl(o, s, mask, mask, stream_add=o, out=nxt[B:], have_self=po[0], have_cross=ps[1])
             so = ops.join(nxt, (s2, o2), dim=0)
 
         so_in = new(B, T, 2 * D)
diff --git a/vrdone_amd/models/blocks.py b/vrdone_amd/models/blocks.py
--- a/vrdone_amd/models/blocks.py
+++ b/vrdone_amd/models/blocks.py
@@ -1,4 +1,5 @@
 import math
+import os
 
 import torch
 from torch import nn
@@ -165,6 +166,27 @@
 
     def forward(self, x):
         return x * self.scale
+
+
+MERGE_DWCONV = os.environ.get("VRDONE_MERGE_DWCONV", "0")
+
+
+def merge_ok(*tensors, part="sos"):
+    on = MERGE_DWCONV not in ("0", "") and MERGE_DWCONV in ("1", part)
+    return on and not (torch.is_grad_enabled() and any(t is not None and t.requires_grad for t in tensors))
+
+
+def shared_source_plan(branches):
+    from .. import _hip
+    convs = [getattr(mod, f"{name}_conv").conv for mod, name, _ in branches]
+    same = all(c.kernel_size == (3,) and c.stride == (1,) and c.groups == c.in_channels == convs[0].in_channels
+               and c.weight.shape == convs[0].weight.shape for c in convs)
+    return same and 1 <= len(branches) <= _hip.DWCONV_MAX_SETS
+
+
+def shared_source_launch(branches, x, pre_ln, launch):
+    sets = [dict(mod._branch_set(name), pre_ln=bool(use_ln)) for mod, name, use_ln in branches]
+    return launch(x, sets, pre_ln if any(u for _, _, u in branches) else None)
 
 
 class _ConvAttention(nn.Module):
@@ -188,26 +210,33 @@
         conv, norm = getattr(self, f"{name}_conv"), getattr(self, f"{name}_norm")
         return dict(weight=conv.conv.weight, gamma=norm.weight, beta=norm.bias, pair=_ops().pair_mode())
 
-    def _groups(self, q_in, k_in, v_in, q_mask, kv_mask, pre_ln=None, pre_ln_on="qkv"):
+    def _groups(self, q_in, k_in, v_in, q_mask, kv_mask, pre_ln=None, pre_ln_on="qkv", merge=False, have=()):
         specs = [("query", q_in, q_mask, "q"), ("key", k_in, kv_mask, "k"), ("value", v_in, kv_mask, "v")]
         groups = []
         for name, x, m, tag in specs:
+            if name in have:
+                continue
             ks = getattr(self, f"{name}_conv").conv.kernel_size
             use_ln = pre_ln is not None and tag in pre_ln_on
-            for g in groups:
-                if g[0] is x and g[1] is m and g[2] == use_ln and g[3] == ks:
+            for i, g in enumerate(groups):
+                if g[0] is x and g[1] is m and g[3] == ks and (g[2] == use_ln or (merge and ks == (3,))):
                     g[4].append(name)
+                    g[5].append(use_ln)
+                    groups[i] = (g[0], g[1], g[2] or use_ln, g[3], g[4], g[5])
                     break
             else:
-                groups.append((x, m, use_ln, ks, [name]))
+                groups.append((x, m, use_ln, ks, [name], [use_ln]))
         return groups
 
-    def _prep(self, q_in, k_in, v_in, q_mask, kv_mask, stride=1, pre_ln=None, pre_ln_on="qkv"):
-        ops = _ops()
-        outs = {}
-        for x, m, use_ln, _, names in self._groups(q_in, k_in, v_in, q_mask, kv_mask, pre_ln, pre_ln_on):
-            res = ops.dwconv_ln(x, [self._branch_set(n) for n in names], mask_out=m, stride=stride,
-                                pre_ln=pre_ln if use_ln else None)
+    def _branch_sets(self, names, flags):
+        return [dict(self._branch_set(n), pre_ln=f) for n, f in zip(names, flags)]
+
+    def _prep(self, q_in, k_in, v_in, q_mask, kv_mask, stride=1, pre_ln=None, pre_ln_on="qkv", have=None):
+        ops = _ops()
+        outs = dict(have or {})
+        merge = merge_ok(q_in, k_in, v_in, self.query_conv.conv.weight)
+        for x, m, use_ln, _, names, flags in self._groups(q_in, k_in, v_in, q_mask, kv_mask, pre_ln, pre_ln_on, merge, outs):
+            res = ops.dwconv_ln(x, self._branch_sets(names, flags), mask_out=m, stride=stride, pre_ln=pre_ln if use_ln else None)
             outs.update(zip(names, res))
         return outs["query"], outs["key"], outs["value"]
 
diff --git a/vrdone_amd/models/fpns.py b/vrdone_amd/models/fpns.py
--- a/vrdone_amd/models/fpns.py
+++ b/vrdone_amd/models/fpns.py
@@ -1,6 +1,6 @@
 from torch import nn
 
-from .blocks import LayerNorm, MaskedConv1D, _from_cl, _mask2d, _ops, _to_cl
+from .blocks import LayerNorm, MaskedConv1D, _from_cl, _mask2d, _ops, _to_cl, merge_ok
 
 
 class FPN1D_Fuse(nn.Module):
@@ -40,8 +40,11 @@
                 y, = ops.dwconv_ln(x, [fpn], mask_out=masks[l])
             else:
                 c = ops.conv_gemm(x, self.lateral_convs[l].conv.weight, None, row_mask=masks[l])
-                c = self.lateral_norms[l].cl(c)
-                y, = ops.dwconv_ln(c, [fpn], mask_out=masks[l], x_up=y)
+                ln = self.lateral_norms[l]
+                if c.shape[-1] == 256 and merge_ok(c, ln.weight, part="fpn"):
+                    y, = ops.dwconv_ln(c, [fpn], mask_out=masks[l], x_up=y, pre_ln=(ln.weight, ln.bias))
+                else:
+                    y, = ops.dwconv_ln(ln.cl(c), [fpn], mask_out=masks[l], x_up=y)
         mf = self.mask_features.conv
         out, = ops.dwconv_ln(y, [dict(weight=mf.weight, bias=mf.bias)], mask_out=masks[0])
         return out, masks[0]
diff --git a/vrdone_amd/models/local_transformer.py b/vrdone_amd/models/local_transformer.py
--- a/vrdone_amd/models/local_transformer.py
+++ b/vrdone_amd/models/local_transformer.py
@@ -4,7 +4,7 @@
 from torch import nn, Tensor
 
 from .blocks import (make_rel_pe, AffineDropPath, LayerNorm, MaskedMHA, _ConvAttention, _from_cl, _mask2d, _ops,
-                     _to_cl)
+                     _to_cl, merge_ok, shared_source_launch, shared_source_plan)
 from .transformer import _get_clones
 
 
@@ -29,9 +29,9 @@
         self.n_qx_stride, self.n_kv_stride = n_qx_stride, n_kv_stride
         self._build(n_embd, n_head, _qkv_kernel(n_qx_stride), _qkv_kernel(n_kv_stride), 1)
 
-    def cl_qkv(self, q_in, k_in, v_in, q_mask, kv_mask, pre_ln=None, pre_ln_on="", **epilogue):
+    def cl_qkv(self, q_in, k_in, v_in, q_mask, kv_mask, pre_ln=None, pre_ln_on="", have=None, **epilogue):
         ops = _ops()
-        q, k, v = self._prep(q_in, k_in, v_in, q_mask, kv_mask, pre_ln=pre_ln, pre_ln_on=pre_ln_on)
+        q, k, v = self._prep(q_in, k_in, v_in, q_mask, kv_mask, pre_ln=pre_ln, pre_ln_on=pre_ln_on, have=have)
         qkv_pair = self._half_win is None and ops.flash_pair_ok(self.n_head, self.n_embd, q.shape[1])
         q, k, v = self._project(q, k, v, out_pair=qkv_pair, q_mask=q_mask, kv_mask=kv_mask)
         if self._half_win is None:
@@ -63,6 +63,24 @@
         self.use_rel_pe = use_rel_pe
         self._half_win = self.window_overlap
         self.rel_pe = make_rel_pe(n_embd, n_head, window_size) if use_rel_pe else None
+
+
+def sos_source_branches(layer, other):
+    if not (isinstance(layer.self_attn, MaskedMHCA_QKV) and isinstance(other.multihead_attn, MaskedMHCA_QKV)):
+        return None
+    sa, ca = layer.self_attn, other.multihead_attn
+    branches = [(sa, "query", True), (sa, "key", True), (sa, "value", False), (ca, "key", False), (ca, "value", False)]
+    return branches if shared_source_plan(branches) else None
+
+
+def sos_prepare(layer, other, x, mask, other_mask, launch):
+    if mask is not other_mask or not merge_ok(x, layer.ln1.weight):
+        return None
+    branches = sos_source_branches(layer, other)
+    if branches is None:
+        return None
+    q, k, v, ck, cv = shared_source_launch(branches, x, (layer.ln1.weight, layer.ln1.bias), launch)
+    return dict(query=q, key=k, value=v), dict(key=ck, value=cv)
 
 
 class MaskedConvTransformerDecoderLayer(nn.Module):
@@ -113,14 +131,15 @@
     def _drop(dp, tgt):
         return dp.row_factors(tgt.shape[0], tgt.shape[1], tgt.device) if isinstance(dp, AffineDropPath) else None
 
-    def cl(self, tgt, memory, tgt_mask, memory_mask, query_pos=None, stream_add=None, out=None):
+    def cl(self, tgt, memory, tgt_mask, memory_mask, query_pos=None, stream_add=None, out=None, have_self=None, have_cross=None):
+        assert (have_self is None and have_cross is None) or query_pos is None
         ops = _ops()
         fuse1 = query_pos is None and isinstance(self.self_attn, MaskedMHCA_QKV)
         fuse2 = query_pos is None and isinstance(self.multihead_attn, MaskedMHCA_QKV)
         last = not self.with_ffn
         if fuse1:
             tgt, _ = self.self_attn.cl_qkv(tgt, tgt, tgt, tgt_mask, tgt_mask, pre_ln=(self.ln1.weight, self.ln1.bias),
-                                           pre_ln_on="qk", scale=self._scale(self.drop_path_attn1),
+                                           pre_ln_on="qk", have=have_self, scale=self._scale(self.drop_path_attn1),
                                            row_scale=self._drop(self.drop_path_attn1, tgt), res=tgt, res_masked=True)
         else:
             t2 = self.ln1.cl(tgt, post_add=query_pos)
@@ -130,7 +149,7 @@
                   res_masked=True, res2=stream_add if last else None, out=out if last else None)
         if fuse2:
             tgt, _ = self.multihead_attn.cl_qkv(tgt, memory, memory, tgt_mask, memory_mask,
-                                                pre_ln=(self.ln2.weight, self.ln2.bias), pre_ln_on="q", **kw)
+                                                pre_ln=(self.ln2.weight, self.ln2.bias), pre_ln_on="q", have=have_cross, **kw)
         else:
             t2 = self.ln2.cl(tgt, post_add=query_pos)
             tgt, _ = self.multihead_attn.cl_qkv(t2, memory, memory, tgt_mask, memory_mask, **kw)
diff --git a/vrdone_amd/models/ragged.py b/vrdone_amd/models/ragged.py
--- a/vrdone_amd/models/ragged.py
+++ b/vrdone_amd/models/ragged.py
@@ -1,6 +1,7 @@
 import torch
 
-from .blocks import _ConvAttention, _ops
+from .blocks import _ConvAttention, _ops, merge_ok
+from .local_transformer import sos_prepare
 
 
 _MAX_SEGS = 32
@@ -143,16 +144,17 @@
     return _side_streams[key]
 
 
-def _attn_rows(mod, q_in, k_in, v_in, q_mask, kv_mask, qsegs, ksegs, *, stride=1, pre_ln=None, pre_ln_on="", **epilogue):
+def _attn_rows(mod, q_in, k_in, v_in, q_mask, kv_mask, qsegs, ksegs, *, stride=1, pre_ln=None, pre_ln_on="", have=None, **epilogue):
     ops = _ops()
     if stride > 1:
         qsegs_o = ksegs_o = [(off // stride, n, T // stride) for off, n, T in qsegs]
     else:
         qsegs_o, ksegs_o = qsegs, ksegs
     if isinstance(mod, _ConvAttention):
-        outs = {}
-        for x, m, use_ln, _, names in mod._groups(q_in, k_in, v_in, q_mask, kv_mask, pre_ln, pre_ln_on):
-            res = _dwconv_rows(x, [mod._branch_set(nm) for nm in names], m, qsegs if x is q_in else ksegs, stride=stride,
+        outs = dict(have or {})
+        merge = merge_ok(q_in, k_in, v_in, mod.query_conv.conv.weight)
+        for x, m, use_ln, _, names, flags in mod._groups(q_in, k_in, v_in, q_mask, kv_mask, pre_ln, pre_ln_on, merge, outs):
+            res = _dwconv_rows(x, mod._branch_sets(names, flags), m, qsegs if x is q_in else ksegs, stride=stride,
                                pre_ln=pre_ln if use_ln else None)
             outs.update(zip(names, res))
         q, k, v = outs["query"], outs["key"], outs["value"]
@@ -192,7 +194,8 @@
     return y, m_out, segs_o
 
 
-def _decoder_layer(layer, tgt, memory, tgt_mask, memory_mask, qsegs, ksegs, *, query_pos=None, stream_add=None, out=None):
+def _decoder_layer(layer, tgt, memory, tgt_mask, memory_mask, qsegs, ksegs, *, query_pos=None, stream_add=None, out=None,
+                   have_self=None, have_cross=None):
     ops = _ops()
     from .local_transformer import MaskedMHCA_QKV
     fuse1 = query_pos is None and isinstance(layer.self_attn, MaskedMHCA_QKV)
@@ -201,7 +204,7 @@
     kw1 = dict(scale=layer._scale(layer.drop_path_attn1), res=tgt, res_masked=True)
     if fuse1:
         tgt = _attn_rows(layer.self_attn, tgt, tgt, tgt, tgt_mask, tgt_mask, qsegs, qsegs, pre_ln=(layer.ln1.weight, layer.ln1.bias),
-                         pre_ln_on="qk", **kw1)
+                         pre_ln_on="qk", have=have_self, **kw1)
     else:
         t2 = layer.ln1.cl(tgt, post_add=query_pos)
         tgt = _attn_rows(layer.self_attn, t2, t2, tgt, tgt_mask, tgt_mask, qsegs, qsegs, **kw1)
@@ -209,7 +212,7 @@
               out=out if last else None)
     if fuse2:
         tgt = _attn_rows(layer.multihead_attn, tgt, memory, memory, tgt_mask, memory_mask, qsegs, ksegs,
-                         pre_ln=(layer.ln2.weight, layer.ln2.bias), pre_ln_on="q", **kw)
+                         pre_ln=(layer.ln2.weight, layer.ln2.bias), pre_ln_on="q", have=have_cross, **kw)
     else:
         t2 = layer.ln2.cl(tgt, post_add=query_pos)
         tgt = _attn_rows(layer.multihead_attn, t2, memory, memory, tgt_mask, memory_mask, qsegs, ksegs, **kw)
@@ -327,8 +330,11 @@
             so, _, _ = _block(bb.stem[i], so, mask2, segs2)
         s, o = so[:, :R], so[:, R:]
         nxt = new(2 * R, D)
-        _decoder_layer(s_attn, s, o, mask, mask, segs, segs, stream_add=s, out=nxt[:, :R])
-        _decoder_layer(o_attn, o, s, mask, mask, segs, segs, stream_add=o, out=nxt[:, R:])
+        launch = lambda x, sets, pre_ln: _dwconv_rows(x, sets, mask, segs, pre_ln=pre_ln)
+        ps = sos_prepare(s_attn, o_attn, s, mask, mask, launch) or (None, None)
+        po = sos_prepare(o_attn, s_attn, o, mask, mask, launch) or (None, None)
+        _decoder_layer(s_attn, s, o, mask, mask, segs, segs, stream_add=s, out=nxt[:, :R], have_self=ps[0], have_cross=po[1])
+        _decoder_layer(o_attn, o, s, mask, mask, segs, segs, stream_add=o, out=nxt[:, R:], have_self=po[0], have_cross=ps[1])
         so = nxt
     so_in = new(R, 2 * D)
     bb.s_fuse_norm.cl(so[:, :R], out=so_in[..., :D], pair=pair)
@@ -363,8 +369,11 @@
             y, = _dwconv_rows(x, [fpn], masks[l], lays[l])
         else:
             c = ops.conv_gemm(x, neck.lateral_convs[l].conv.weight, None, row_mask=masks[l])
-            c = neck.lateral_norms[l].cl(c)
-            y, = _dwconv_rows(c, [fpn], masks[l], lays[l], x_up=y)
+            ln = neck.lateral_norms[l]
+            if c.shape[-1] == 256 and merge_ok(c, ln.weight, part="fpn"):
+                y, = _dwconv_rows(c, [fpn], masks[l], lays[l], x_up=y, pre_ln=(ln.weight, ln.bias))
+            else:
+                y, = _dwconv_rows(ln.cl(c), [fpn], masks[l], lays[l], x_up=y)
     mf = neck.mask_features.conv
     out, = _dwconv_rows(y, [dict(weight=mf.weight, bias=mf.bias)], masks[0], lays[0])
     return out
diff --git a/vrdone_amd/ops.py b/vrdone_amd/ops.py
--- a/vrdone_amd/ops.py
+++ b/vrdone_amd/ops.py
@@ -716,7 +716,10 @@
     if recording(x, x_up, *(t for st in sets for t in (st["weight"], st.get("bias"), st.get("gamma"), st.get("beta"))),
                  *(pre_ln or ())):
         from . import autograd
+        if len(sets) > 3 or (pre_ln is not None and (x_up is not None or not all(st.get("pre_ln", True) for st in sets))):
+            raise ValueError("dwconv_ln under autograd recording: up to three sets of one kind, no input LayerNorm with x_up")
         return autograd.dwconv_ln(x, sets, mask_out=mask_out, stride=stride, x_up=x_up, pre_ln=pre_ln)
+    assert 1 <= len(sets) <= _hip.DWCONV_MAX_SETS
     B, Tin, Cx = x.shape
     w0 = sets[0]["weight"]
     Cout, g, k = w0.shape
@@ -736,7 +739,7 @@
         a.x_up, a.ldx_up = pu, ldu
     a.B, a.Tin, a.C, a.ksize, a.stride, a.group_in = B, Tin, Cout, k, stride, g
     if pre_ln is not None:
-        assert g == 1 and x_up is None
+        assert g == 1
         a.pre_gamma, a.pre_beta = _param_ptr(pre_ln[0], x, "LayerNorm weight"), _param_ptr(pre_ln[1], x, "LayerNorm bias")
     a.mask_out = _mask_ptr(mask_out, B * Tout)
     a.n_out = len(sets)
@@ -753,6 +756,7 @@
                                  _param_ptr(s.get("beta"), x, "LayerNorm bias"))
         a.packed[i] = _dwconv_block(s["weight"], s.get("bias"), s.get("gamma"), s.get("beta")).data_ptr()
         a.relu[i] = 1 if s.get("relu") else 0
+        a.pre_ln_set[i] = 1 if pre_ln is not None and s.get("pre_ln", True) else 0
         a.y[i], a.ldy[i] = po, ldo
         a.out_pair[i] = _fmt(s.get("pair"))
         outs.append(Pair(o, Cout) if _fmt(s.get("pair")) else o)
```

Result: no change. 15800 (-0.0%).
